# jopohl/urh

Measured on AMD Instinct MI355X. Metric: Msamples/s IQ->bits (1 GiB complex64 2-FSK per GPU, qad materialised, compact outputs copied to the host), higher is better.
Workload: dtype f32

## Files before the change

include/urhgpu.h:

```cpp
#ifndef URHGPU_H
#define URHGPU_H

#include <stdint.h>

#ifdef __cplusplus
extern "C" {
#endif

#define URHGPU_VERSION 100

#define URHGPU_OK 0
#define URHGPU_ERR_HIP (-1)
#define URHGPU_ERR_DTYPE (-2)
#define URHGPU_ERR_ARG (-3)
#define URHGPU_ERR_CAPACITY (-4)
#define URHGPU_ERR_UNSUPPORTED (-5)
#define URHGPU_ERR_NO_DEVICE (-6)

#define URHGPU_DT_I8 0
#define URHGPU_DT_U8 1
#define URHGPU_DT_I16 2
#define URHGPU_DT_U16 3
#define URHGPU_DT_F32 4

// ... 190 lines not shown

int urhgpu_segment_runs_dev(urhgpu_ctx *ctx, const void *d_iq, int dtype, int64_t n, float noise_threshold,
                            int64_t *d_rows, int64_t cap_rows, int64_t *d_n_rows);
int urhgpu_message_ranges_dev(urhgpu_ctx *ctx, const void *d_iq, int dtype, int64_t n, float noise_threshold, int64_t *seg_out, int64_t cap_seg_out,
                              int64_t *n_seg_out, int64_t *merged_out, int64_t cap_merged_out, int64_t *n_merged_out, int *merge_ambiguous);
int urhgpu_message_ranges_demod_dev(urhgpu_ctx *ctx, const void *d_iq, int dtype, int64_t n, float noise_threshold, int64_t *seg_out,
                                    int64_t cap_seg_out, int64_t *n_seg_out, int64_t *merged_out, int64_t cap_merged_out,
                                    int64_t *n_merged_out, int *merge_ambiguous, float *d_qad_ask);
int urhgpu_compact_gt_dev(urhgpu_ctx *ctx, const float *d_x, int64_t n, float thr, float *d_out, int64_t *d_count);
int urhgpu_edges_le_dev(urhgpu_ctx *ctx, const float *d_x, int64_t n, float center, int64_t *d_idx, int64_t cap, int64_t *d_count);
int urhgpu_minmax_f32_dev(urhgpu_ctx *ctx, const float *d_x, int64_t n, float *d_out2);
int urhgpu_pairwise_sum_f32_dev(urhgpu_ctx *ctx, const float *d_x, int64_t n, int mode, float mean, float *sum_out);
int urhgpu_histogram_f32_dev(urhgpu_ctx *ctx, const float *d_x, int64_t n, const double *d_edges, int64_t n_edges, int64_t *d_counts);

int urhgpu_msg_center_stats(urhgpu_ctx *ctx, const float *d_x, int64_t n, const int64_t *ranges, int n_msgs, int64_t max_bins,
                            double *out_stats, int64_t *out_hist, double *out_center, int32_t *out_flag);
int urhgpu_msg_plateaus(urhgpu_ctx *ctx, const float *d_x, int64_t n, const int64_t *ranges, const double *centers, int n_msgs,
                        int percentage, int64_t extra_window, int64_t *out_off, uint64_t *out_len, int64_t cap_total);

int urhgpu_merge_plateaus(const uint64_t *plateaus, int64_t n, uint64_t tolerance, uint64_t max_count, uint64_t *out, int64_t *n_out);

int urhgpu_detect_modulation_dev(urhgpu_ctx *ctx, const float *d_iq, int64_t n, const int64_t *ranges, int n_msgs, int wavelet_scale,
                                 int median_filter_order, int *labels_out, double *vars_out);

int urhgpu_msg_bit_lengths(const uint64_t *lens, const int64_t *off, int n_msgs, int64_t *tol_out, int64_t *bitlen_out);
int urhgpu_msg_plateau_decisions(urhgpu_ctx *ctx, const float *d_x, int64_t n, const int64_t *ranges, const double *centers, int n_msgs,
                                 int percentage, int64_t extra_window, int64_t *tol_out, int64_t *bitlen_out);
int urhgpu_msg_estimate(urhgpu_ctx *ctx, const float *d_x, int64_t n, const int64_t *ranges, int n_msgs, int64_t max_bins, int percentage,
                        int64_t extra_window, double *out_stats, double *out_center, int32_t *out_flag, int64_t *tol_out, int64_t *bitlen_out);
int urhgpu_test_bit_length_from_counts(const uint64_t *lens, int64_t n, int64_t *tol_out, int64_t *bitlen_out);
int urhgpu_msg_divisor_histogram(const uint64_t *lens, int64_t n, uint64_t *hist_out, int64_t cap, int64_t *hist_len, int64_t *tol_out);
int urhgpu_bit_length_from_order(const uint64_t *hist, const int64_t *order_desc, int64_t len, int64_t *bitlen_out);

int urhgpu_minmax(urhgpu_ctx *ctx, const void *arr, int dtype, int64_t n, void *out2);
int urhgpu_segment_messages(urhgpu_ctx *ctx, const void *magnitudes, int is_f64, int64_t n, float noise_threshold, int64_t *seg_out,
                            int64_t cap_seg, int64_t *n_seg);
int urhgpu_get_plateau_lengths(urhgpu_ctx *ctx, const float *rect_data, int64_t n, float center, int percentage, uint64_t *out, int64_t cap,
                               int64_t *n_out);
int urhgpu_threshold_divisor_histogram(const uint64_t *lens, int64_t n, float threshold, uint64_t *hist_out, int64_t cap, int64_t *hist_len);
int urhgpu_median_filter(urhgpu_ctx *ctx, const double *data, int64_t n, unsigned int k, float *out);

int urhgpu_test_fast_division_dev(urhgpu_ctx *ctx, uint64_t seed, int reps, uint64_t *n_mismatch);
int urhgpu_test_sincosf_fast_dev(urhgpu_ctx *ctx, uint64_t *n_mismatch);
int urhgpu_test_force_merge_ambiguous(int on);

int urhgpu_modulate_dev(urhgpu_ctx *ctx, const uint8_t *bits, const int64_t *bit_off, const uint32_t *pause, const uint32_t *start,
                        int n_msgs, uint32_t samples_per_symbol, int mod, const float *parameters, int bits_per_symbol,
                        float carrier_amplitude, float carrier_frequency, float carrier_phase, float sample_rate, int dtype,
                        void *d_out, int64_t cap_samples, int64_t *total_samples);
int urhgpu_modulate(urhgpu_ctx *ctx, const uint8_t *bits, int64_t num_bits, uint32_t samples_per_symbol, int mod,
                    const float *parameters, int bits_per_symbol, float carrier_amplitude, float carrier_frequency,
                    float carrier_phase, float sample_rate, uint32_t pause, uint32_t start, int dtype, void *out);

int urhgpu_modulate_gfsk_dev(urhgpu_ctx *ctx, const uint8_t *bits, const int64_t *bit_off, const uint32_t *pause, const uint32_t *start,
                             int n_msgs, uint32_t samples_per_symbol, const float *parameters, int bits_per_symbol,
                             float carrier_amplitude, float carrier_phase, float sample_rate, int dtype, const float *gauss_fir,
                             int n_taps, const float *frequencies, void *d_out, int64_t cap_samples, int64_t *total_samples);
int urhgpu_modulate_gfsk(urhgpu_ctx *ctx, const uint8_t *bits, int64_t num_bits, uint32_t samples_per_symbol, const float *parameters,
                         int bits_per_symbol, float carrier_amplitude, float carrier_phase, float sample_rate, uint32_t pause,
                         uint32_t start, int dtype, const float *gauss_fir, int n_taps, const float *frequencies, void *out);

int urhgpu_convert_dev(urhgpu_ctx *ctx, const void *d_src, int src_dtype, void *d_dst, int dst_dtype, int64_t n);
int urhgpu_pcm_to_iq_dev(urhgpu_ctx *ctx, const void *d_raw, int64_t n_frames, int channels, int sample_width, float *d_out);
int urhgpu_fft_peak_dev(urhgpu_ctx *ctx, const float *d_x, int64_t n, int64_t *peak_index);
int urhgpu_sub_encode_runs(const uint8_t *values, int64_t n, int64_t stride, int64_t *runs_out, int64_t cap, int64_t *n_runs);
int urhgpu_astype_dev(urhgpu_ctx *ctx, const void *d_src, int src_dtype, void *d_dst, int dst_dtype, int64_t n);

int urhgpu_path_minmax_dev(urhgpu_ctx *ctx, const void *d_samples, int dtype, int64_t start, int64_t end,
                           int64_t samples_per_pixel, void *d_values);
int urhgpu_path_minmax(urhgpu_ctx *ctx, const void *samples, int dtype, int64_t n, int64_t start, int64_t end,
                       int64_t samples_per_pixel, void *values);

int urhgpu_spectrogram_dev(urhgpu_ctx *ctx, const float *d_x, int64_t n, int window_size, int64_t hop, int64_t frames,
                           const double *d_window, const double *d_twiddles, double *d_stft, float *d_db);
int urhgpu_bgra_lookup_dev(urhgpu_ctx *ctx, const float *d_db, int64_t frames, int window_size, const uint32_t *d_colormap,
                           int n_colors, float data_min, float data_max, uint32_t *d_image);

int urhgpu_bench_copy_ceiling_dev(urhgpu_ctx *ctx, const float *d_in, float *d_out, int64_t n_samples, int shape, int reps, float *ms_per_copy);
int urhgpu_test_hot_probe(urhgpu_ctx *ctx, const void *d_iq, int64_t n, const urhgpu_params *p, float *d_qad, int stream_kind, int event_mode,
                          int graded, int launches, int keep, void *d_chunks_out, int64_t *n_chunks_out, float *dur_ms, float *gap_ms, int bubble_us,
                          int load_kind);
int urhgpu_test_hot_stamps(int on);
int urhgpu_test_tail_skip(int mask);
int urhgpu_test_fetch_chunk_tables(urhgpu_ctx *ctx, void *host_dst, int64_t n_chunks);
int urhgpu_memcpy_to_host(urhgpu_ctx *ctx, const void *d_src, void *host_dst, int64_t bytes);
int urhgpu_memcpy_dtod(urhgpu_ctx *ctx, void *d_dst, const void *d_src, int64_t bytes);

int urhgpu_test_force_state_bytes(int on);

int urhgpu_test_force_generic_tail(int on);

int urhgpu_test_force_tiles_per_chunk(int tiles);

int64_t urhgpu_test_wide_int_launches(void);

int64_t urhgpu_test_costas_host_syncs(void);
int64_t urhgpu_test_center_host_syncs(void);
int urhgpu_test_costas_scratch(int64_t n, int loop_order, int64_t *out3);

int urhgpu_test_atan2f_dev(urhgpu_ctx *ctx, const float *d_y, const float *d_x, int64_t n, float *d_out);

int urhgpu_chunk_power_stats_dev(urhgpu_ctx *ctx, const void *d_src, int dtype, int64_t n_rows, void *d_dst, int64_t n_store, double *sum_out,
                                 double *max_out);
int urhgpu_chunk_stats_launches(urhgpu_ctx *ctx, int64_t *n_launches);

int urhgpu_magnitude_chunk_partials_dev(urhgpu_ctx *ctx, const void *d_iq, int dtype, int64_t n_local, int64_t pos_base, int64_t n_total,
                                        int64_t chunk, int64_t n_chunks, double *d_sum, double *d_max);
#define URHGPU_PW_REC_HEAD 8
#define URHGPU_PW_REC_FIRST 136
#define URHGPU_PW_REC_LAST 264
#define URHGPU_PW_REC_TAIL 392
#define URHGPU_PW_REC_PIECES 520
int urhgpu_pairwise_partial_f32_dev(urhgpu_ctx *ctx, const float *d_x, int64_t m_local, int64_t g_off, int64_t m_total, int mode, float mean,
                                    float *d_out, int64_t cap, int64_t *n_out);

typedef struct urhgpu_noise_result {
    double noise;
    float noise_f32;
    float noise_sqrd;
    int64_t flag;
    int64_t chunk, n_chunks;
    int64_t n_candidates;
    double min_mean, max_mean;
} urhgpu_noise_result;
double urhgpu_noise_max_magnitude(int dtype);
int urhgpu_detect_noise_level_dev(urhgpu_ctx *ctx, const void *d_iq, int dtype, int64_t n, void *d_result);
int urhgpu_iq_to_bits_auto_dev(urhgpu_ctx *ctx, const void *d_iq, int64_t n, const urhgpu_params *p, int auto_noise, int auto_center,
                               int64_t center_max_size, const urhgpu_outputs *out, void *d_noise_result, void *h_noise_result,
                               void *d_center_result, void *h_center_result, int64_t hist_cap);
int urhgpu_stream_set_auto_noise(urhgpu_stream *st, int enable);
int urhgpu_stream_noise(urhgpu_stream *st, int64_t seq, double *noise, int64_t *flag);
int64_t urhgpu_test_noise_host_syncs(void);

typedef struct urhgpu_msg_record {
    double rssi;
    int64_t first_pos;
    int64_t mid_pos;
    int32_t n_pad;
    int32_t flag;
} urhgpu_msg_record;
int urhgpu_msg_records_dev(urhgpu_ctx *ctx, const void *d_iq, int64_t n, const urhgpu_params *p, const urhgpu_outputs *out,
                           int64_t message_length_divisor, void *d_rec, int64_t cap_msg, void *h_rec);
int urhgpu_stream_set_msg_records(urhgpu_stream *st, int enable, int64_t message_length_divisor);
int urhgpu_stream_msg_records(urhgpu_stream *st, int64_t seq, const urhgpu_msg_record **rec, int64_t *n_msg);
int64_t urhgpu_test_records_host_syncs(void);

int urhgpu_dc_correct_dev(urhgpu_ctx *ctx, const void *d_in, int64_t n, int dtype, void *d_out, void *d_mean);
int urhgpu_dc_correct(urhgpu_ctx *ctx, const void *h_in, int64_t n, int dtype, void *h_out, void *h_mean);
int64_t urhgpu_test_dc_host_syncs(void);
int urhgpu_test_dc_stats(urhgpu_ctx *ctx, int64_t *stats);

int urhgpu_shard_dc_sums_dev(urhgpu_ctx *ctx, const void *d_in, int64_t n, int dtype, void *d_words);
#define URHGPU_DC_RECORD_BYTES 64
int urhgpu_shard_dc_spec_dev(urhgpu_ctx *ctx, const void *d_in, int64_t n, const double *base, void *d_records);
int urhgpu_shard_dc_resolve_dev(urhgpu_ctx *ctx, const void *d_in, int64_t n, const uint32_t *entry, void *d_exit);
int urhgpu_shard_dc_apply_dev(urhgpu_ctx *ctx, const void *d_in, int64_t n, int dtype, const void *mean, void *d_out);
int urhgpu_shard_dc_stats(urhgpu_ctx *ctx, int64_t *stats);

#define URHGPU_SHARD_REC_SUMMARY_WORDS 10
#define URHGPU_SHARD_REC_FIRST_WORDS 8
int urhgpu_shard_records_summary_dev(urhgpu_ctx *ctx, int64_t n_local, int64_t pos_base, const urhgpu_outputs *out, void *d_words);
int urhgpu_shard_records_lookup_dev(urhgpu_ctx *ctx, const urhgpu_outputs *out, const void *d_index, int64_t n, void *d_values);
int urhgpu_shard_msg_records_dev(urhgpu_ctx *ctx, const void *d_iq, int64_t n_local, int64_t pos_base, int64_t n_total, const urhgpu_params *p,
                                 const urhgpu_outputs *out, int64_t message_length_divisor, const int64_t *first, const void *d_window,
                                 int64_t window_len, void *d_rec, int64_t cap_msg, void *h_rec);

// ... 87 lines not shown
```

urh_amd/_lib.py:

```python
import ctypes as C
import os
import threading

HERE = os.path.dirname(os.path.abspath(__file__))
LIB_PATH = os.path.join(HERE, "liburhgpu.so")

OK = 0
ERR_HIP, ERR_DTYPE, ERR_ARG, ERR_CAPACITY, ERR_UNSUPPORTED, ERR_NO_DEVICE = -1, -2, -3, -4, -5, -6
BLOB_LEN16 = 2
BLOB_ROW16 = 4

DT_I8, DT_U8, DT_I16, DT_U16, DT_F32 = 0, 1, 2, 3, 4
MOD_ASK, MOD_FSK, MOD_PSK, MOD_OTHER = 0, 1, 2, 3
ROW_ABSORBED = -(1 << 62)
BLOB_MAGIC = 0x55524842424C4F42
BLOB_HEADER_BYTES = 128


class UrhGpuError(RuntimeError):
    def __init__(self, status, msg):
        super().__init__(msg)
        self.status = status


# ... 80 lines not shown
                                    C.POINTER(_i64)]),
    "urhgpu_ppseq_to_bits": (_i, [_vp, _vp, _i64, _i64, _i, _i, _i64, _vp, _i64, _vp, _vp, _i64, _vp, _i64, _vp, _vp]),
    "urhgpu_fir_filter": (_i, [_vp, _vp, _i64, _vp, _i64, _vp]),
    "urhgpu_fir_filter_dev": (_i, [_vp, _vp, _i64, _vp, _i64, _vp, _vp]),
    "urhgpu_fir_filter_stats_dev": (_i, [_vp, _vp, _i64, _vp, _i64, _vp, _vp, _i64, _i64, _vp, _vp]),
    "urhgpu_bandpass": (_i, [_vp, _vp, _i64, _vp, _i64, _i64, _i64, _vp]),
    "urhgpu_bandpass_dev": (_i, [_vp, _vp, _i64, _vp, _i64, _i64, _i64, _vp, _i64, _vp, _i64, _vp, _i]),
    "urhgpu_iir_filter": (_i, [_vp, _vp, _i64, _vp, _i64, _vp, _i64, _vp]),
    "urhgpu_afp_demod_dev": (_i, [_vp, _vp, _i64, C.POINTER(Params), _vp]),
    "urhgpu_grab_pulse_lens_dev": (_i, [_vp, _vp, _i64, C.POINTER(Params), _vp, _i64, _vp]),
    "urhgpu_ppseq_to_bits_dev": (_i, [_vp, _vp, _vp, _i64, C.POINTER(Params), C.POINTER(Outputs)]),
    "urhgpu_iq_to_bits_dev": (_i, [_vp, _vp, _i64, C.POINTER(Params), C.POINTER(Outputs)]),
    "urhgpu_detect_center_dev": (_i, [_vp, _vp, _i64, _i64, _vp, _i64]),
    "urhgpu_iq_to_bits_auto_center_dev": (_i, [_vp, _vp, _i64, C.POINTER(Params), _i64, C.POINTER(Outputs), _vp, _vp, _i64]),
    "urhgpu_center_hist_cap": (_i64, [_vp]),
    "urhgpu_stream_set_auto_center": (_i, [_vp, _i, _i64]),
    "urhgpu_stream_center": (_i, [_vp, _i64, C.POINTER(C.c_double), C.POINTER(_i64), C.POINTER(_vp), C.POINTER(_i64), C.POINTER(C.c_double),
                                  C.POINTER(C.c_double)]),
    "urhgpu_test_center_host_syncs": (_i64, []),
    "urhgpu_noise_max_magnitude": (C.c_double, [_i]),
    "urhgpu_detect_noise_level_dev": (_i, [_vp, _vp, _i, _i64, _vp]),
    "urhgpu_iq_to_bits_auto_dev": (_i, [_vp, _vp, _i64, C.POINTER(Params), _i, _i, _i64, C.POINTER(Outputs), _vp, _vp, _vp, _vp, _i64]),
    "urhgpu_stream_set_auto_noise": (_i, [_vp, _i]),
    "urhgpu_stream_noise": (_i, [_vp, _i64, C.POINTER(C.c_double), C.POINTER(_i64)]),
    "urhgpu_test_noise_host_syncs": (_i64, []),
    "urhgpu_msg_records_dev": (_i, [_vp, _vp, _i64, C.POINTER(Params), C.POINTER(Outputs), _i64, _vp, _i64, _vp]),
    "urhgpu_stream_set_msg_records": (_i, [_vp, _i, _i64]),
    "urhgpu_stream_msg_records": (_i, [_vp, _i64, C.POINTER(_vp), C.POINTER(_i64)]),
    "urhgpu_test_records_host_syncs": (_i64, []),
    "urhgpu_shard_records_summary_dev": (_i, [_vp, _i64, _i64, C.POINTER(Outputs), _vp]),
    "urhgpu_shard_records_lookup_dev": (_i, [_vp, C.POINTER(Outputs), _vp, _i64, _vp]),
    "urhgpu_shard_msg_records_dev": (_i, [_vp, _vp, _i64, _i64, _i64, C.POINTER(Params), C.POINTER(Outputs), _i64, C.POINTER(_i64), _vp, _i64, _vp, _i64,
                                          _vp]),
    "urhgpu_blob_capacity": (_i64, [_i64, _i64, _i64, _i64, _i]),
    "urhgpu_outputs_to_host": (_i, [_vp, C.POINTER(Outputs), _i, _vp, _i64, C.POINTER(_i64)]),
    "urhgpu_host_libm_check": (_i, [C.POINTER(_i64)]),
    "urhgpu_stream_capacities": (_i, [_i64, C.POINTER(Params), C.POINTER(_i64), C.POINTER(_i64), C.POINTER(_i64), C.POINTER(_i64)]),
    "urhgpu_stream_create": (_i, [_vp, _i64, C.POINTER(Params), _i, _i, _i64, C.POINTER(_vp)]),
    "urhgpu_stream_destroy": (_i, [_vp]),
    "urhgpu_stream_push": (_i, [_vp, _vp, _i64, C.POINTER(HostResult)]),
    "urhgpu_stream_push_upload": (_i, [_vp, _vp, _vp, _i64, C.POINTER(HostResult)]),
    "urhgpu_stream_flush": (_i, [_vp, C.POINTER(HostResult), C.POINTER(_i)]),
    "urhgpu_stream_stats": (_i, [_vp, C.POINTER(_i64)]),
    "urhgpu_stream_wide_passes": (_i, [_vp, C.POINTER(_i64)]),
    "urhgpu_stream_costas_stats": (_i, [_vp, C.POINTER(_i64)]),
    "urhgpu_shard_runs_dev": (_i, [_vp, _vp, _i64, _i64, _i64, _i, _i, _vp, C.POINTER(Params), C.POINTER(Outputs), _vp]),
    "urhgpu_shard_prelaunch_dev": (_i, [_vp, _vp, _i64, _i64, _i64, _i, _i, C.POINTER(Params), C.POINTER(Outputs)]),
    "urhgpu_shard_launch_dev": (_i, [_vp, _vp, _i64, _i64, _i64, _i, _i, _vp, C.POINTER(Params), C.POINTER(Outputs)]),
    "urhgpu_shard_rows_dev": (_i, [_vp, _vp, _vp]),
    "urhgpu_shard_bits_prepare_dev": (_i, [_vp, _vp, _vp]),
    "urhgpu_shard_bits_finish_dev": (_i, [_vp, _vp]),
    "urhgpu_costas_halo_samples": (_i64, [C.POINTER(Params)]),
    "urhgpu_shard_costas_spec_dev": (_i, [_vp, _vp, _i64, _i64, _i64, _i, _i, _vp, _i64, C.POINTER(Params), C.POINTER(Outputs), _vp]),
    "urhgpu_shard_costas_resolve_dev": (_i, [_vp, C.POINTER(C.c_uint32), _vp]),
    "urhgpu_shard_demod_dev": (_i, [_vp, _vp, _i64, _i64, _i64, _i, _i, _vp, C.POINTER(Params), C.POINTER(Outputs)]),
    "urhgpu_shard_seam_value": (_i, [_vp, C.POINTER(C.c_float)]),
    "urhgpu_magnitude_chunk_stats_dev": (_i, [_vp, _vp, _i, _i64, _i64, _i64, _vp, _vp]),
    "urhgpu_segment_runs_dev": (_i, [_vp, _vp, _i, _i64, _f, _vp, _i64, _vp]),
    "urhgpu_message_ranges_dev": (_i, [_vp, _vp, _i, _i64, _f, _vp, _i64, C.POINTER(_i64), _vp, _i64, C.POINTER(_i64), C.POINTER(_i)]),
    "urhgpu_message_ranges_demod_dev": (_i, [_vp, _vp, _i, _i64, _f, _vp, _i64, C.POINTER(_i64), _vp, _i64, C.POINTER(_i64), C.POINTER(_i), _vp]),
    "urhgpu_compact_gt_dev": (_i, [_vp, _vp, _i64, _f, _vp, _vp]),
    "urhgpu_edges_le_dev": (_i, [_vp, _vp, _i64, _f, _vp, _i64, _vp]),
    "urhgpu_minmax_f32_dev": (_i, [_vp, _vp, _i64, _vp]),
    "urhgpu_pairwise_sum_f32_dev": (_i, [_vp, _vp, _i64, _i, _f, C.POINTER(_f)]),
    "urhgpu_histogram_f32_dev": (_i, [_vp, _vp, _i64, _vp, _i64, _vp]),
    "urhgpu_msg_center_stats": (_i, [_vp, _vp, _i64, _vp, _i, _i64, _vp, _vp, _vp, _vp]),
    "urhgpu_msg_plateaus": (_i, [_vp, _vp, _i64, _vp, _vp, _i, _i, _i64, _vp, _vp, _i64]),
    "urhgpu_detect_modulation_dev": (_i, [_vp, _vp, _i64, _vp, _i, _i, _i, _vp, _vp]),
    "urhgpu_msg_bit_lengths": (_i, [_vp, _vp, _i, _vp, _vp]),
    "urhgpu_msg_plateau_decisions": (_i, [_vp, _vp, _i64, _vp, _vp, _i, _i, _i64, _vp, _vp]),
    "urhgpu_msg_estimate": (_i, [_vp, _vp, _i64, _vp, _i, _i64, _i, _i64, _vp, _vp, _vp, _vp, _vp]),
    "urhgpu_test_bit_length_from_counts": (_i, [_vp, _i64, C.POINTER(_i64), C.POINTER(_i64)]),
    "urhgpu_msg_divisor_histogram": (_i, [_vp, _i64, _vp, _i64, C.POINTER(_i64), C.POINTER(_i64)]),
    "urhgpu_bit_length_from_order": (_i, [_vp, _vp, _i64, C.POINTER(_i64)]),
    "urhgpu_merge_plateaus": (_i, [_vp, _i64, C.c_uint64, C.c_uint64, _vp, C.POINTER(_i64)]),
    "urhgpu_minmax": (_i, [_vp, _vp, _i, _i64, _vp]),
    "urhgpu_segment_messages": (_i, [_vp, _vp, _i, _i64, _f, _vp, _i64, C.POINTER(_i64)]),
    "urhgpu_get_plateau_lengths": (_i, [_vp, _vp, _i64, _f, _i, _vp, _i64, C.POINTER(_i64)]),
    "urhgpu_threshold_divisor_histogram": (_i, [_vp, _i64, _f, _vp, _i64, C.POINTER(_i64)]),
    "urhgpu_median_filter": (_i, [_vp, _vp, _i64, C.c_uint, _vp]),
    "urhgpu_test_hot_probe": (_i, [_vp, _vp, _i64, C.POINTER(Params), _vp, _i, _i, _i, _i, _i, _vp, C.POINTER(_i64), _vp, _vp, _i, _i]),
    "urhgpu_test_hot_stamps": (_i, [_i]),
    "urhgpu_test_tail_skip": (_i, [_i]),
    "urhgpu_test_fetch_chunk_tables": (_i, [_vp, _vp, _i64]),
    "urhgpu_test_fast_division_dev": (_i, [_vp, C.c_uint64, _i, C.POINTER(C.c_uint64)]),
    "urhgpu_test_sincosf_fast_dev": (_i, [_vp, C.POINTER(C.c_uint64)]),
    "urhgpu_test_force_merge_ambiguous": (_i, [_i]),
    "urhgpu_modulate_dev": (_i, [_vp, _vp, _vp, _vp, _vp, _i, C.c_uint32, _i, _vp, _i, _f, _f, _f, _f, _i, _vp, _i64, C.POINTER(_i64)]),
    "urhgpu_modulate": (_i, [_vp, _vp, _i64, C.c_uint32, _i, _vp, _i, _f, _f, _f, _f, C.c_uint32, C.c_uint32, _i, _vp]),
    "urhgpu_modulate_gfsk_dev": (_i, [_vp, _vp, _vp, _vp, _vp, _i, C.c_uint32, _vp, _i, _f, _f, _f, _i, _vp, _i, _vp, _vp, _i64, C.POINTER(_i64)]),
    "urhgpu_modulate_gfsk": (_i, [_vp, _vp, _i64, C.c_uint32, _vp, _i, _f, _f, _f, C.c_uint32, C.c_uint32, _i, _vp, _i, _vp, _vp]),
    "urhgpu_spectrogram_dev": (_i, [_vp, _vp, _i64, _i, _i64, _i64, _vp, _vp, _vp, _vp]),
    "urhgpu_bgra_lookup_dev": (_i, [_vp, _vp, _i64, _i, _vp, _i, _f, _f, _vp]),
    "urhgpu_convert_dev": (_i, [_vp, _vp, _i, _vp, _i, _i64]),
    "urhgpu_pcm_to_iq_dev": (_i, [_vp, _vp, _i64, _i, _i, _vp]),
    "urhgpu_sub_encode_runs": (_i, [_vp, _i64, _i64, _vp, _i64, _vp]),
    "urhgpu_fft_peak_dev": (_i, [_vp, _vp, _i64, _vp]),
    "urhgpu_astype_dev": (_i, [_vp, _vp, _i, _vp, _i, _i64]),
    "urhgpu_path_minmax_dev": (_i, [_vp, _vp, _i, _i64, _i64, _i64, _vp]),
    "urhgpu_path_minmax": (_i, [_vp, _vp, _i, _i64, _i64, _i64, _i64, _vp]),
    "urhgpu_bench_copy_ceiling_dev": (_i, [_vp, _vp, _vp, _i64, _i, _i, C.POINTER(_f)]),
    "urhgpu_memcpy_to_host": (_i, [_vp, _vp, _vp, _i64]),
    "urhgpu_memcpy_dtod": (_i, [_vp, _vp, _vp, _i64]),
    "urhgpu_test_force_state_bytes": (_i, [_i]),
    "urhgpu_test_force_tiles_per_chunk": (_i, [_i]),
    "urhgpu_test_wide_int_launches": (_i64, []),
    "urhgpu_test_costas_host_syncs": (_i64, []),
    "urhgpu_test_costas_scratch": (_i, [_i64, _i, C.POINTER(_i64)]),
    "urhgpu_test_force_generic_tail": (_i, [_i]),
    "urhgpu_test_atan2f_dev": (_i, [_vp, _vp, _vp, _i64, _vp]),
    "urhgpu_chunk_power_stats_dev": (_i, [_vp, _vp, _i, _i64, _vp, _i64, C.POINTER(C.c_double), C.POINTER(C.c_double)]),
    "urhgpu_chunk_stats_launches": (_i, [_vp, C.POINTER(_i64)]),
    "urhgpu_magnitude_chunk_partials_dev": (_i, [_vp, _vp, _i, _i64, _i64, _i64, _i64, _i64, _vp, _vp]),
    "urhgpu_pairwise_partial_f32_dev": (_i, [_vp, _vp, _i64, _i64, _i64, _i, _f, _vp, _i64, C.POINTER(_i64)]),
    "urhgpu_dc_correct_dev": (_i, [_vp, _vp, _i64, _i, _vp, _vp]),
    "urhgpu_dc_correct": (_i, [_vp, _vp, _i64, _i, _vp, _vp]),
    "urhgpu_test_dc_host_syncs": (_i64, []),
    "urhgpu_test_dc_stats": (_i, [_vp, C.POINTER(_i64)]),
    "urhgpu_shard_dc_sums_dev": (_i, [_vp, _vp, _i64, _i, _vp]),
    "urhgpu_shard_dc_spec_dev": (_i, [_vp, _vp, _i64, C.POINTER(C.c_double), _vp]),
    "urhgpu_shard_dc_resolve_dev": (_i, [_vp, _vp, _i64, C.POINTER(C.c_uint32), _vp]),
    "urhgpu_shard_dc_apply_dev": (_i, [_vp, _vp, _i64, _i, _vp, _vp]),
    "urhgpu_shard_dc_stats": (_i, [_vp, C.POINTER(_i64)]),
    "urhgpu_batch_step": (_i, []),
    "urhgpu_batch_plan": (_i, [_vp, _i64, C.POINTER(Params), _i, _i64, _vp, C.POINTER(_i64), C.POINTER(_i64)]),
    "urhgpu_iq_to_bits_batch_dev": (_i, [_vp, _vp, _i64, _vp, _vp, _i64, C.POINTER(Params), _vp, _vp, _i64, _vp, _vp, _vp, _i64]),
    "urhgpu_batch_fetch": (_i, [_vp, _vp, _i64, _vp, _vp, _vp, _i64, C.POINTER(_i64)]),
    "urhgpu_batch_launches": (_i, [_vp, C.POINTER(_i64)]),
    "urhgpu_batch_noise_dev": (_i, [_vp, _vp, _i64, _vp, _vp, _i64, C.POINTER(Params), _vp]),
    "urhgpu_iq_to_bits_batch_auto_dev": (_i, [_vp, _vp, _i64, _vp, _vp, _i64, C.POINTER(Params), _vp, _vp, _i64, _vp, _vp, _vp, _i64, _vp]),
    "urhgpu_batch_noise_fetch": (_i, [_vp, _vp, _i64, _vp]),
    "urhgpu_batch_center_plan": (_i, [_vp, _i64, _i64, _i64, C.POINTER(_i64), C.POINTER(_i64), C.POINTER(_i64)]),
    "urhgpu_batch_center_dev": (_i, [_vp, _vp, _i64, _vp, _i64, C.POINTER(Params), _i64, _vp, _vp, _i64, _vp, _i64, _vp, _i64, _vp, _i64]),
    "urhgpu_qad_to_bits_batch_dev": (_i, [_vp, _vp, _i64, _vp, _vp, _i64, C.POINTER(Params), _vp, _i64, _vp, _vp, _i64, _vp, _vp, _vp, _i64]),
    "urhgpu_iq_to_bits_batch_center_dev": (_i, [_vp, _vp, _i64, _vp, _vp, _i64, C.POINTER(Params), _i, _i64, _vp, _vp, _i64, _vp, _vp, _vp, _i64, _vp,
                                                _vp, _i64, _vp, _i64, _vp, _i64, _vp, _i64]),
    "urhgpu_batch_center_fetch": (_i, [_vp, _vp, _i64, _vp, _i64, _vp, _vp, _i64, C.POINTER(_i64)]),
    "urhgpu_batch_msg_records_dev": (_i, [_vp, _vp, _i64, _vp, _i64, _vp, _vp, _i64, C.POINTER(Params), _vp, _i64, _vp, _i64, _vp, _vp, _vp, _i64, _vp]),
    "urhgpu_batch_records_fetch": (_i, [_vp, _vp, _i64, _i64, _vp]),
    "urhgpu_batch_segments_capacity": (_i64, [_i64]),
    "urhgpu_batch_segments_dev": (_i, [_vp, _vp, _i, _i64, _vp, _vp, _i64, _vp, _vp, _vp, _i64, _vp, _vp, _vp, _i64]),
    "urhgpu_batch_segments_fetch": (_i, [_vp, _vp, _i64, _vp, _vp, _vp, _i64, C.POINTER(_i64)]),
    "urhgpu_batch_demod_dev": (_i, [_vp, _vp, _i64, _vp, _vp, _i64, C.POINTER(Params), _vp, _vp]),
    "urhgpu_batch_costas_dev": (_i, [_vp, _vp, _i64, _vp, _vp, _i64, C.POINTER(Params), _vp, _vp]),
    "urhgpu_iq_to_bits_batch_psk_dev": (_i, [_vp, _vp, _i64, _vp, _vp, _i64, C.POINTER(Params), _i, _i, _i64, _vp, _vp, _i64, _vp, _vp, _vp, _i64, _vp,
                                             _vp, _i64, _vp, _i64, _vp, _i64, _vp, _i64]),
    "urhgpu_batch_dc_correct_dev": (_i, [_vp, _vp, _i64, _i, _vp, _vp, _i64, _vp, _vp]),
    "urhgpu_batch_plan_each": (_i, [_vp, _i64, _vp, _i, _i64, _vp, C.POINTER(_i64), C.POINTER(_i64)]),
    "urhgpu_iq_to_bits_batch_each_dev": (_i, [_vp, _vp, _i64, _i, _vp, _vp, _i64, _vp, _vp, _i64, _i64, _i, _vp, _vp, _i64, _vp, _vp, _vp, _i64, _vp]),
    "urhgpu_batch_msg_records_each_dev": (_i, [_vp, _vp, _i64, _i, _vp, _vp, _i64, _vp, _i64, _vp, _i64, _vp, _vp, _vp, _i64, _vp]),
}

_lib = None
_lock = threading.Lock()


def _share_torch_hip_runtime():
    import importlib.util
    try:
        spec = importlib.util.find_spec("torch")
    except (ImportError, ValueError):
        spec = None
    if spec is None or not spec.origin:
        return
    cand = os.path.join(os.path.dirname(spec.origin), "lib", "libamdhip64.so")
    if os.path.exists(cand):
# ... 139 lines not shown
```

urh_amd/csrc/common.hpp:

```cpp
#pragma once
#include <hip/hip_runtime.h>
#include <stdint.h>
#include <stdio.h>
#include <string.h>

#include <atomic>
#include <vector>

#include "../../include/urhgpu.h"

#ifndef URH_TAIL_PRIO_LEVEL
#define URH_TAIL_PRIO_LEVEL 3
#endif
#ifndef URH_TAIL_PAD
#define URH_TAIL_PAD 0
#endif
#if URH_TAIL_PAD
#define URH_TAIL_PRIO() do { __builtin_amdgcn_s_setprio(URH_TAIL_PRIO_LEVEL); __asm__ volatile("v_mov_b32 v95, 0" ::: "v95"); } while (0)
#else
#define URH_TAIL_PRIO() __builtin_amdgcn_s_setprio(URH_TAIL_PRIO_LEVEL)
#endif

namespace urh {

// ... 25 lines not shown
    void *take(size_t bytes) {
        size_t off = (used + 255) & ~size_t(255);
        if (off + bytes > cap) return nullptr;
        used = off + bytes;
        return (char *)base + off;
    }
    void release();
};
inline size_t align256(size_t x) { return (x + 255) & ~size_t(255); }

extern std::atomic<long long> g_center_host_syncs;
extern thread_local int g_center_scope;
extern std::atomic<long long> g_noise_host_syncs;
extern thread_local int g_noise_scope;
extern std::atomic<long long> g_records_host_syncs;
extern thread_local int g_records_scope;
inline void center_note_wait() {
    if (g_center_scope > 0) ++g_center_host_syncs;
    if (g_noise_scope > 0) ++g_noise_host_syncs;
    if (g_records_scope > 0) ++g_records_host_syncs;
}
struct CenterScope { CenterScope() { ++g_center_scope; } ~CenterScope() { --g_center_scope; } };
struct NoiseScope { bool on; explicit NoiseScope(bool enable = true) : on(enable) { if (on) ++g_noise_scope; } ~NoiseScope() { if (on) --g_noise_scope; } };
struct RecordsScope { bool on; explicit RecordsScope(bool enable = true) : on(enable) { if (on) ++g_records_scope; } ~RecordsScope() { if (on) --g_records_scope; } };

}

constexpr size_t kSmallPinned = size_t(1) << 20;
constexpr int kNoiseMaxChunks = 199;
constexpr size_t kNoiseWorkBytes = 128 * 1024;
struct urhgpu_ctx {
    int device = 0;
    hipStream_t own_stream = nullptr;
    hipStream_t stream = nullptr;
    hipDeviceProp_t prop;
    urh::Arena arena;
    urh::Arena staging;
    urh::Arena aux;
    urh::Arena fir_work;
    hipEvent_t ev_fir = nullptr;
    hipStream_t fir_stream = nullptr;
    int64_t *d_counts = nullptr;
    int64_t *h_counts = nullptr;
    bool tune_spin_wait = true;
    bool tune_wide_int = false;
    bool tune_shard_summary_generic = false;
    int tune_costas_dev_rounds = -1;
    int32_t *costas_stats_next = nullptr;
    hipStream_t last_tail = nullptr;
    int wide_int_next = 0;
    char *h_small = nullptr;
    int32_t *d_tickets = nullptr;
    void *d_desc = nullptr;
    size_t desc_cap = 0;
    void *d_rdesc = nullptr;
    size_t rdesc_cap = 0;
    unsigned long long scan_epoch = 0x0ACE0FBA5E000000ull;
    std::vector<hipEvent_t> prof_events;
    std::vector<bool> prof_dispatch;
    int prof_used = 0;
    bool prof_on = false;
    bool prof_bracket = false;
    void *shard = nullptr;
    bool pipelined = false;
    int hot_lds_pad_sharded = 33 * 1024;
    int tune_hot_cus_removed = 4;
    hipStream_t hot_masked = nullptr;
    hipEvent_t ev_in = nullptr;
    int hot_lds_pad = 0;
    hipStream_t tail_stream = nullptr;
    bool own_tail_stream = false;
    urh::Arena arena_alt, arena_alt2;
    hipEvent_t ev_hot = nullptr;
    hipEvent_t ev_tail[3] = {nullptr, nullptr, nullptr};
    int flip = 0;
    bool tail_pending = false;
    int tile_parity = 0;
    void *d_seg = nullptr;
    bool seg_dirty[3] = {false, false, false};
    int tune_stream_segments = 7;
    int tune_stream_policy = 5;
    long long passes_begun = 0;
    bool tune_stream_latency = false;
    bool tune_stream_pos_direct = true;
    int tune_upload_pieces = 4;
    hipEvent_t ev_piece[16] = {};
    hipEvent_t ev_hot_done[3] = {nullptr, nullptr, nullptr};
    hipStream_t bits_stream = nullptr;
    hipEvent_t ev_rows[3][16] = {};
    hipEvent_t ev_bits[3] = {nullptr, nullptr, nullptr};
    urh::Arena chunk_work;
    double *h_chunk = nullptr;
    long long chunk_launches = 0;
    long long batch_launches = 0, batch_copies = 0;
    urh::Arena center_work;
    int tune_center_max_bins = 4096;
    hipEvent_t ev_center = nullptr;
    void *d_noise_work = nullptr;
    int wide_int_auto = 0;
    urh::Arena dc_work;
    hipEvent_t ev_dc = nullptr;
    hipStream_t dc_stream = nullptr;
    const void *dc_shard_in = nullptr;
    int64_t dc_shard_n = -1;
    urh::Arena batch_dc_mean;
};
constexpr size_t kSegBlockBytes = 4096;

namespace urh {
int iq_to_bits_streamed(urhgpu_ctx *ctx, const void *d_iq, int64_t n, const urhgpu_params *p, const urhgpu_outputs *out, void *host_blob,
                        int64_t cap_host, hipEvent_t ev_ready, bool *streamed, const void *h_iq, void *stage_blob = nullptr, bool *staged = nullptr,
                        hipEvent_t ev_rows = nullptr, int len16 = 0);
hipError_t wait_stream(const urhgpu_ctx *ctx, hipStream_t s);
int reserve_psk_pass(urhgpu_ctx *ctx, int64_t n_max, int tolerance, bool want_qad);
int join_tail(urhgpu_ctx *ctx);
inline int stage_in(urhgpu_ctx *ctx, const void *host, size_t bytes, void **dev) {
    void *d = ctx->staging.take(bytes ? bytes : 16);
    if (!d) return URHGPU_ERR_ARG;
    if (bytes) URH_HIP(hipMemcpyAsync(d, host, bytes, hipMemcpyHostToDevice, ctx->stream));
    *dev = d;
    return URHGPU_OK;
}
inline int fetch_out(urhgpu_ctx *ctx, void *host, const void *dev, size_t bytes) {
    URH_HIP(hipMemcpyAsync(host, dev, bytes, hipMemcpyDeviceToHost, ctx->stream));
    URH_HIP(hipStreamSynchronize(ctx->stream));
    return URHGPU_OK;
}
}
```

urh_amd/csrc/ctx.hip:

```cpp
#include <chrono>

#include "pass.hpp"
#include "fdlibm_atan2f.h"
#include "glibc_sincosf.h"

namespace urh {

thread_local char g_hip_err[256] = "";
std::atomic<long long> g_center_host_syncs{0};
thread_local int g_center_scope = 0;
std::atomic<long long> g_noise_host_syncs{0};
thread_local int g_noise_scope = 0;
std::atomic<long long> g_records_host_syncs{0};
thread_local int g_records_scope = 0;

int Arena::reserve(size_t bytes) {
    if (bytes <= cap) return URHGPU_OK;
    if (base) { center_note_wait(); URH_HIP(hipFree(base)); base = nullptr; cap = 0; }
    const size_t want = (bytes + (size_t(1) << 20)) & ~((size_t(1) << 20) - 1);
    URH_HIP(hipMalloc(&base, want));
    cap = want;
    used = 0;
    return URHGPU_OK;
}
// ... 118 lines not shown
            if (ctx->ev_bits[k]) (void)hipEventDestroy(ctx->ev_bits[k]);
            for (hipEvent_t e : ctx->ev_rows[k]) if (e) (void)hipEventDestroy(e);
        }
    }
    if (ctx->ev_hot) { (void)hipEventDestroy(ctx->ev_hot); (void)hipEventDestroy(ctx->ev_tail[0]); (void)hipEventDestroy(ctx->ev_tail[1]); (void)hipEventDestroy(ctx->ev_tail[2]); }
    free_shard_session(ctx);
    for (hipEvent_t e : ctx->prof_events) (void)hipEventDestroy(e);
    if (ctx->d_counts) (void)hipFree(ctx->d_counts);
    if (ctx->d_tickets) (void)hipFree(ctx->d_tickets);
    if (ctx->d_noise_work) (void)hipFree(ctx->d_noise_work);
    if (ctx->d_desc) (void)hipFree(ctx->d_desc);
    if (ctx->d_rdesc) (void)hipFree(ctx->d_rdesc);
    if (ctx->h_counts) (void)hipHostFree(ctx->h_counts);
    if (ctx->h_small) (void)hipHostFree(ctx->h_small);
    if (ctx->own_stream) (void)hipStreamDestroy(ctx->own_stream);
    delete ctx;
    return URHGPU_OK;
}

int urhgpu_ctx_set_stream(urhgpu_ctx *ctx, void *hip_stream) {
    if (!ctx) return URHGPU_ERR_ARG;
    ctx->stream = (hipStream_t)hip_stream;
    return URHGPU_OK;
}

int urhgpu_ctx_use_private_stream(urhgpu_ctx *ctx) {
    if (!ctx) return URHGPU_ERR_ARG;
    ctx->stream = ctx->own_stream;
    return URHGPU_OK;
}

int urhgpu_ctx_sync(urhgpu_ctx *ctx) {
    if (!ctx) return URHGPU_ERR_ARG;
    if (ctx->hot_masked) URH_HIP(hipStreamSynchronize(ctx->hot_masked));
    if (ctx->bits_stream) URH_HIP(hipStreamSynchronize(ctx->bits_stream));
    if (ctx->tail_stream) URH_HIP(hipStreamSynchronize(ctx->tail_stream));
    URH_HIP(hipStreamSynchronize(ctx->stream));
    ctx->tail_pending = false;
    return URHGPU_OK;
}

int urhgpu_ctx_set_pipelined(urhgpu_ctx *ctx, int enable, void *tail_stream) {
    if (!ctx) return URHGPU_ERR_ARG;
    URH_HIP(hipSetDevice(ctx->device));
    URH_TRY(urhgpu_ctx_sync(ctx));
    if (ctx->own_tail_stream && ctx->tail_stream) { (void)hipStreamDestroy(ctx->tail_stream); }
    ctx->tail_stream = nullptr; ctx->own_tail_stream = false; ctx->pipelined = false;
    if (ctx->hot_masked) { (void)hipStreamSynchronize(ctx->hot_masked); (void)hipStreamDestroy(ctx->hot_masked); ctx->hot_masked = nullptr; }
    if (!enable) return URHGPU_OK;
    if (tail_stream) ctx->tail_stream = (hipStream_t)tail_stream;
    else {
        URH_HIP(hipStreamCreateWithFlags(&ctx->tail_stream, hipStreamNonBlocking));
        ctx->own_tail_stream = true;
    }
    if (!ctx->ev_hot) {
        URH_HIP(hipEventCreateWithFlags(&ctx->ev_hot, hipEventDisableTiming));
        for (hipEvent_t &e : ctx->ev_tail) URH_HIP(hipEventCreateWithFlags(&e, hipEventDisableTiming));
    }
    if (ctx->tune_hot_cus_removed > 0 && ctx->prop.multiProcessorCount == 256) {
        const int words = 8;
        uint32_t mask[8];
        hot_cu_mask(ctx->tune_hot_cus_removed, mask);
        if (hipExtStreamCreateWithCUMask(&ctx->hot_masked, (uint32_t)words, mask) != hipSuccess) { (void)hipGetLastError(); ctx->hot_masked = nullptr; }
        if (ctx->hot_masked && !ctx->ev_in && hipEventCreateWithFlags(&ctx->ev_in, hipEventDisableTiming) != hipSuccess) {
            (void)hipGetLastError();
            (void)hipStreamDestroy(ctx->hot_masked);
            ctx->hot_masked = nullptr;
        }
    }
    ctx->pipelined = true;
    return URHGPU_OK;
}

int urhgpu_ctx_set_tuning(urhgpu_ctx *ctx, const char *key, int value) {
    if (!ctx || !key) return URHGPU_ERR_ARG;
    if (!strcmp(key, "hot_lds_kb")) { if (value < 0 || value > 150) return URHGPU_ERR_ARG; ctx->hot_lds_pad = value * 1024; }
    else if (!strcmp(key, "hot_lds_kb_sharded")) { if (value < 0 || value > 150) return URHGPU_ERR_ARG; ctx->hot_lds_pad_sharded = value * 1024; }
    else if (!strcmp(key, "profile_bracket")) ctx->prof_bracket = value != 0;
    else if (!strcmp(key, "hot_cus_removed_per_xcd")) { if (value < 0 || value > 16) return URHGPU_ERR_ARG; ctx->tune_hot_cus_removed = value; }
    else if (!strcmp(key, "stream_segments")) { if (value < 1 || value > kMaxSegments) return URHGPU_ERR_ARG; ctx->tune_stream_segments = value; }
    else if (!strcmp(key, "stream_policy")) { if (value < 0 || value > 6) return URHGPU_ERR_ARG; ctx->tune_stream_policy = value; }
    else if (!strcmp(key, "stream_latency")) { ctx->tune_stream_latency = value != 0; }
    else if (!strcmp(key, "stream_pos_direct")) { ctx->tune_stream_pos_direct = value != 0; }
    else if (!strcmp(key, "spin_wait")) { ctx->tune_spin_wait = value != 0; }
    else if (!strcmp(key, "shard_summary_generic")) { ctx->tune_shard_summary_generic = value != 0; }
    else if (!strcmp(key, "wide_int")) { ctx->tune_wide_int = value != 0; }
    else if (!strcmp(key, "costas_dev_rounds")) { if (value < -1 || value > 24) return URHGPU_ERR_ARG; ctx->tune_costas_dev_rounds = value; }
    else if (!strcmp(key, "upload_pieces")) { if (value < 2 || value > kMaxSegments) return URHGPU_ERR_ARG; ctx->tune_upload_pieces = value; }
    else if (!strcmp(key, "auto_center_max_bins")) { if (value < 1 || value > (1 << 20)) return URHGPU_ERR_ARG; ctx->tune_center_max_bins = value; }
    else return URHGPU_ERR_ARG;
    return URHGPU_OK;
}

int urhgpu_ctx_join(urhgpu_ctx *ctx) {
    if (!ctx) return URHGPU_ERR_ARG;
    URH_HIP(hipSetDevice(ctx->device));
    return join_tail(ctx);
}

int urhgpu_host_libm_check(int64_t *out4) {
    if (!out4) return URHGPU_ERR_ARG;
    static const uint32_t kDiscriminating[17] = {0x418a3adbu, 0x418a3adcu, 0x418a3addu, 0x418a3adeu, 0x41bc76d9u, 0x4202eb4bu, 0x4255b0a9u, 0x4280ce28u,
                                                 0x42687a55u, 0x42a35c07u, 0x42a35d44u, 0x42870e40u, 0x42a97360u, 0x42c55faau, 0x42d8d23eu, 0x42e87a55u,
                                                 0x42cf5854u};
    int64_t n_sc = 0, bad_sc = 0, n_at = 0, bad_at = 0;
    auto same = [](float a, float b) { uint32_t x, y; memcpy(&x, &a, 4); memcpy(&y, &b, 4); return x == y || (a != a && b != b); };
    auto check_sc = [&](float x) {
        volatile float vx = x;
        n_sc += 2;
        if (!same(sinf(vx), urh_sinf(x))) ++bad_sc;
        if (!same(cosf(vx), urh_cosf(x))) ++bad_sc;
    };
    for (uint32_t u : kDiscriminating) {
        float x; memcpy(&x, &u, 4);
        check_sc(x); check_sc(-x);
    }
    uint64_t s = 0x243f6a8885a308d3ull;
    auto next = [&]() { s += 0x9e3779b97f4a7c15ull; uint64_t z = s; z = (z ^ (z >> 30)) * 0xbf58476d1ce4e5b9ull; z = (z ^ (z >> 27)) * 0x94d049bb133111ebull; return z ^ (z >> 31); };
    for (int i = 0; i < 4096; ++i) {
        const uint64_t z = next();
        check_sc((float)((double)(int64_t)(z >> 11) * (1.0 / 9007199254740992.0) * 240.0 - 120.0));
        const uint32_t a = (uint32_t)z, b = (uint32_t)(z >> 32);
        float y, x;
        const uint32_t uy = (a & 0x807fffffu) | (((a >> 23) % 41u + 107u) << 23), ux = (b & 0x807fffffu) | (((b >> 23) % 41u + 107u) << 23);
        memcpy(&y, &uy, 4); memcpy(&x, &ux, 4);
        volatile float vy = y, vx = x;
        ++n_at;
        if (!same(atan2f(vy, vx), urh_atan2f(y, x))) ++bad_at;
    }
    out4[0] = n_sc; out4[1] = bad_sc; out4[2] = n_at; out4[3] = bad_at;
    return URHGPU_OK;
}

int urhgpu_ctx_info(urhgpu_ctx *ctx, int *compute_units, int *wavefront, int64_t *hbm_bytes, char *name, int name_cap) {
    if (!ctx) return URHGPU_ERR_ARG;
    if (compute_units) *compute_units = ctx->prop.multiProcessorCount;
    if (wavefront) *wavefront = ctx->prop.warpSize;
    if (hbm_bytes) *hbm_bytes = (int64_t)ctx->prop.totalGlobalMem;
    if (name && name_cap > 0) { strncpy(name, ctx->prop.name, (size_t)name_cap - 1); name[name_cap - 1] = 0; }
    return URHGPU_OK;
}

int urhgpu_ctx_reserve(urhgpu_ctx *ctx, int64_t n_samples, int tolerance) {
    if (!ctx || n_samples < 0 || tolerance < 0) return URHGPU_ERR_ARG;
    URH_HIP(hipSetDevice(ctx->device));
    const Plan pl = make_plan(ctx, n_samples, tolerance);
    const int64_t cap_rows = n_samples / ((int64_t)tolerance + 1) + 2;
    URH_TRY(ctx->arena.reserve(digitize_scratch_bytes(pl, cap_rows, true, true)));
    if (ctx->pipelined) {
        URH_TRY(ctx->arena_alt.reserve(digitize_scratch_bytes(pl, cap_rows, true, true)));
        URH_TRY(ctx->arena_alt2.reserve(digitize_scratch_bytes(pl, cap_rows, true, true)));
    }
    return URHGPU_OK;
}

int urhgpu_ctx_profile_begin(urhgpu_ctx *ctx, int max_records) {
    if (!ctx || max_records < 0) return URHGPU_ERR_ARG;
    URH_HIP(hipSetDevice(ctx->device));
    while ((int)ctx->prof_events.size() < 4 * max_records) {
        hipEvent_t e;
        URH_HIP(hipEventCreate(&e));
        ctx->prof_events.push_back(e);
    }
    ctx->prof_used = 0;
    ctx->prof_on = max_records > 0;
    return URHGPU_OK;
// ... 53 lines not shown
```

urh_amd/csrc/launchers.hpp:

```cpp
#pragma once
#include <atomic>
#include <hip/hip_runtime.h>
#include <stdint.h>

#include "common.hpp"
#include "runs.hpp"

namespace urh {

struct RunArgs {
    const void *in;
    float *qad;
    const void *left_halo;
    int64_t n;
    int64_t range_begin;
    int64_t range_end;
    int64_t chunk_base;
    int64_t pos_base;
    int64_t chunk_len;
    uint64_t *slab;
    int64_t slab_stride;
    ChunkInfo *chunks;
    float noise_sqrd;
    float noise_val;
// ... 155 lines not shown
size_t merge_scratch_bytes(int64_t cap);
int launch_merge_rows_ask(const int64_t *rows_in, const int64_t *d_n_in, int64_t cap, int64_t *rows_out,
                          int64_t cap_out, int64_t *d_n_out, void *scratch, int32_t *tickets, hipStream_t s);
size_t bits_scratch_bytes(int64_t cap_rows);
struct ScanState {
    int32_t *tickets;
    void *desc;
    size_t desc_bytes;
    unsigned long long *epoch;
};
size_t bits_desc_bytes(int64_t cap_rows);
int launch_ppseq_to_bits(const int64_t *rows, const int64_t *d_n_rows, int64_t cap_rows, const BitsParams &bp,
                         const BitsOut &o, void *scratch, const ScanState &ss, hipStream_t s);
int launch_bits_prepare(const int64_t *rows, const int64_t *d_n_rows, int64_t cap_rows, const BitsParams &bp,
                        void *scratch, int64_t *d_flags, const ScanState &ss, hipStream_t s);
int launch_bits_finish(const int64_t *rows, const int64_t *d_n_rows, int64_t cap_rows, const BitsParams &bp,
                       const BitsOut &o, void *scratch, const ScanState &ss, hipStream_t s);
struct SegState {
    int64_t rows_at[kMaxSegments];
    int64_t rows_needed;
    int64_t n_acc;
    int64_t n_groups;
    int64_t n_groups_local;
    int64_t end_bits, end_pos, end_msgs;
    int64_t err;
    struct In {
        int64_t g0;
        int64_t carry[3];
        int64_t ship_bits, ship_pos, ship_msgs, pad;
    } in[2];
};
static_assert(sizeof(SegState) == 128 + 64 + 128, "SegState");
constexpr int64_t kSegAlign = 256;
struct SegGate {
    const uint32_t *progress;
    int k;
    uint32_t target;
    int init;
    SegState *seg;
    long long max_ticks;
    int fused;
};
struct RowsSegment {
    int index;
    int final;
    int64_t c0, c1;
    SegGate gate;
    int8_t *h_state;
    int32_t *h_len;
    int fuse_gate;
    int len16;
    int64_t *esc;
    int64_t esc_cap;
};
struct BitsSegment {
    int index;
    int final;
    int64_t c0, c1;
    int rows_index;
    SegState *state;
    int64_t scan_b0;
};
struct SegPackDst {
    void *host;
    int64_t cap_host;
    uint32_t *progress_reset;
    int blocks;
    int pos_direct;
    int split;
    void *host_head;
    const int64_t *esc;
    int64_t esc_cap;
    int64_t row16_esc_off;
};

struct TileTailMem {
    void *mem;
    int64_t n_chunks;
    int32_t *huge_count;
    int parity;
    void *rdesc;
    unsigned long long epoch;
    int64_t *d_row_base = nullptr;
};
size_t tile_rdesc_bytes(int64_t n_chunks);
size_t tile_tail_bytes(int64_t n_chunks);
int64_t tile_desc_cap(int64_t cap_rows, int64_t n_chunks);
int64_t tile_scan_blocks(int64_t c0, int64_t c1, int final);
int launch_tile_rows(const ResolveArgs &r, const EmitArgs &e, const TileTailMem &m, const BitsParams *bp, hipStream_t s);
int launch_tile_bits(const TileTailMem &m, const int64_t *rows, const int64_t *d_n_rows, int64_t cap_rows, const BitsParams &bp,
                     const BitsOut &o, void *scratch, const ScanState &ss, hipStream_t s);
int launch_tile_bits_prepare(const TileTailMem &m, const int64_t *rows, const int64_t *d_n_rows, int64_t cap_rows, const BitsParams &bp,
                             void *scratch, int64_t *d_flags, const ScanState &ss, hipStream_t s);
int launch_tile_bits_finish(const TileTailMem &m, const int64_t *rows, const int64_t *d_n_rows, int64_t cap_rows, const BitsParams &bp,
                            const BitsOut &o, void *scratch, const ScanState &ss, hipStream_t s);
int launch_rows_segment(const ResolveArgs &r, const EmitArgs &e, const TileTailMem &m, const BitsParams &bp, SegState *state, const RowsSegment &sg,
                        hipStream_t s);
int launch_bits_segment(const TileTailMem &m, const BitsParams &bp, const BitsOut &o, void *scratch, const ScanState &ss, int64_t *rows,
                        int64_t cap_rows, const BitsSegment &sg, const SegPackDst *dst, hipStream_t s);
void launch_merge_summary(const int64_t *rows, const int64_t *d_n_rows, int64_t *d_out5, hipStream_t s);
void launch_merge_fix(int64_t *rows, const int64_t *d_n_rows, const int64_t *d_all, int rank, int world,
                      int64_t *d_absorbed, hipStream_t s);
void launch_bits_extra(const int64_t *d_all, int rank, int world, int32_t *d_extra, hipStream_t s);

size_t fir_stats_scratch_bytes(int64_t n);
size_t fir_work_bytes(int64_t n, int m);
int launch_fir(const float2 *x, int64_t n, const float2 *taps, int m, const float2 *halo, float2 *out, hipStream_t s, void *work = nullptr,
               int64_t chunk = 0, int64_t n_chunks = 0, double *d_sum = nullptr, double *d_max = nullptr, void *tile_scratch = nullptr);
int launch_iir(const double *a, int64_t M, const double *b, int64_t N, const float2 *x, int64_t n, float2 *y, hipStream_t s);
int launch_magnitudes(const void *iq, int dtype, int64_t n, double *out, hipStream_t s);
size_t mag_chunk_scratch_bytes(int64_t n_chunks);
int launch_mag_chunk_stats(const void *iq, int dtype, int64_t n, int64_t chunk, int64_t n_chunks, double *d_sum, double *d_max,
                           void *scratch, hipStream_t s);
int launch_noise_chain(const void *iq, int dtype, int64_t n, double max_mag, float cfg_noise, int use_cfg, void *work, void *d_result, void *h_result,
                       hipStream_t s);
size_t compact_scratch_bytes(int64_t n);
int launch_compact_gt(const float *x, int64_t n, const int64_t *d_n, float thr, float *out, int64_t *d_count, void *scratch,
                      int32_t *tickets, hipStream_t s);
int launch_compact_edges(const float *x, int64_t n, const int64_t *d_n, float center, int64_t *out, int64_t cap, int64_t *d_count,
                         void *scratch, int32_t *tickets, hipStream_t s);
size_t minmax_scratch_bytes();
int launch_minmax(const float *x, int64_t n, float *d_out2, void *scratch, hipStream_t s);
int launch_minmax_any(const void *x, int dtype, int64_t n, void *d_out2, void *scratch, hipStream_t s);
int launch_above_flags(const void *mag, int is_f64, int64_t n, float thr, float *flags, hipStream_t s);
int launch_median_filter(const double *data, int64_t n, int k, float *out, hipStream_t s);
constexpr int kDtAboveFlags = 100;
int pairwise_sum_f32(urhgpu_ctx *ctx, const float *d_x, int64_t n, int mode, float mean, float *out);
int launch_hist_edges(const float *x, int64_t n, const double *d_edges, int n_edges, int64_t *d_counts, hipStream_t s);
size_t sp_mag_scratch_bytes(int64_t n_chunks);
int launch_mag_chunk_partials(const void *iq, int dtype, int64_t n_local, int64_t pos_base, int64_t n_total, int64_t chunk, int64_t n_chunks,
                              double *d_sum, double *d_max, void *scratch, hipStream_t s);
int64_t pairwise_partial_words(int64_t m_local, int64_t g_off, int64_t m_total);
size_t pairwise_partial_scratch_bytes(int64_t m_local);
int launch_pairwise_partial(const float *x, int64_t m_local, int64_t g_off, int64_t m_total, int mode, float mean, float *rec, void *scratch,
                            hipStream_t s);
size_t chunk_stats_scratch_bytes(int dtype, int64_t n_rows);
int launch_chunk_stats(const void *d_src, int dtype, int64_t n_rows, void *d_dst, int64_t store_rows, void *scratch, double *h_out, hipStream_t s);
struct SegCtl;
extern bool g_force_merge_ambiguous;
int launch_message_ranges(const int64_t *d_rows, const int64_t *d_n_rows, int64_t cap_rows, const void *d_iq, int dtype, int64_t n, float thr,
                          int ook_merge, int64_t *d_seg, int64_t *d_msgs, int64_t cap, SegCtl *d_ctl, void *scratch, hipStream_t s);
size_t seg_scratch_bytes(int64_t cap_rows, int64_t cap);
size_t seg_ctl_bytes();
void seg_ctl_read(const void *host_copy, int64_t *n_seg, int64_t *n_msgs, int *ambiguous);
int launch_pack_blob(const urhgpu_outputs *o, int write_pos, hipStream_t s);
void launch_copy_shape(const float *in, float *out, int64_t n_samples, int shape, hipStream_t s);
int launch_msg_records(const void *d_iq, int64_t n, const urhgpu_params *p, const urhgpu_outputs *out, int64_t divisor, void *d_rec, int64_t cap_rec,
                       void *h_rec, hipStream_t s);
size_t costas_scratch_bytes(int64_t n);
int launch_costas(urhgpu_ctx *ctx, const void *d_iq, int64_t n, const urhgpu_params *p, float *d_qad, void *scratch, const float *d_noise = nullptr);
extern std::atomic<long long> g_costas_host_syncs;
void costas_scratch_layout(int64_t n, int K, int64_t out3[3]);
constexpr int kCostasSummaryBytes = 160;
struct CostasShard {
    const void *iq;
    const void *halo_end;
    float *out;
    int64_t n, origin, lo, start1;
    urhgpu_params p;
    void *scratch;
};
int64_t costas_halo_samples(const urhgpu_params *p);
int launch_costas_shard_spec(urhgpu_ctx *ctx, const CostasShard &cs, void *d_summary);
int launch_costas_shard_resolve(urhgpu_ctx *ctx, const CostasShard &cs, uint32_t freq_bits, uint32_t phase_bits, void *d_end);

}
```

urh_amd/csrc/probes.hip:

```cpp
#include "pass.hpp"

using namespace urh;

#define URH_PROBE_WPB 4

namespace urh {
bool g_tile_tail = true;
int g_force_tiles_per_chunk = 0;
}

extern "C" {

int urhgpu_test_fast_division_dev(urhgpu_ctx *ctx, uint64_t seed, int reps, uint64_t *n_mismatch) {
    if (!ctx || !n_mismatch || reps < 0) return URHGPU_ERR_ARG;
    URH_HIP(hipSetDevice(ctx->device));
    URH_HIP(hipMemsetAsync(ctx->d_counts, 0, 8, ctx->stream));
    launch_test_div(seed, reps, (unsigned long long *)ctx->d_counts, ctx->stream);
    URH_HIP(hipGetLastError());
    URH_TRY(fetch_out(ctx, ctx->h_counts, ctx->d_counts, 8));
    *n_mismatch = (uint64_t)ctx->h_counts[0];
    return URHGPU_OK;
}

int urhgpu_test_force_merge_ambiguous(int on) {
    const int was = urh::g_force_merge_ambiguous ? 1 : 0;
    urh::g_force_merge_ambiguous = on != 0;
    return was;
}

int urhgpu_test_sincosf_fast_dev(urhgpu_ctx *ctx, uint64_t *n_mismatch) {
    if (!ctx || !n_mismatch) return URHGPU_ERR_ARG;
    URH_HIP(hipSetDevice(ctx->device));
    URH_HIP(hipMemsetAsync(ctx->d_counts, 0, 8, ctx->stream));
    launch_test_sincosf_fast((unsigned long long *)ctx->d_counts, ctx->stream);
    URH_HIP(hipGetLastError());
    URH_TRY(fetch_out(ctx, ctx->h_counts, ctx->d_counts, 8));
    *n_mismatch = (uint64_t)ctx->h_counts[0];
    return URHGPU_OK;
}

int urhgpu_bench_copy_ceiling_dev(urhgpu_ctx *ctx, const float *d_in, float *d_out, int64_t n_samples, int shape, int reps, float *ms_per_copy) {
    if (!ctx || !d_in || !d_out || !ms_per_copy || n_samples < 8192 || n_samples % 8192 || reps < 1 || shape < 0 || shape > 2) return URHGPU_ERR_ARG;
    if (((uintptr_t)d_in & 15) || ((uintptr_t)d_out & 15)) return URHGPU_ERR_ARG;
    URH_HIP(hipSetDevice(ctx->device));
    URH_TRY(urhgpu_ctx_sync(ctx));
    hipStream_t cs = ctx->stream;
    if (shape == 2) {
        if (!ctx->hot_masked) return URHGPU_ERR_UNSUPPORTED;
        cs = ctx->hot_masked; shape = 0;
    }
    hipEvent_t e0, e1;
    URH_HIP(hipEventCreate(&e0));
    URH_HIP(hipEventCreate(&e1));
    for (int k = 0; k < 3; ++k) launch_copy_shape(d_in, d_out, n_samples, shape, cs);
    URH_HIP(hipEventRecord(e0, cs));
    for (int k = 0; k < reps; ++k) launch_copy_shape(d_in, d_out, n_samples, shape, cs);
    URH_HIP(hipEventRecord(e1, cs));
    URH_HIP(hipEventSynchronize(e1));
    float ms = 0.f;
    URH_HIP(hipEventElapsedTime(&ms, e0, e1));
    (void)hipEventDestroy(e0); (void)hipEventDestroy(e1);
    *ms_per_copy = ms / (float)reps;
    return URHGPU_OK;
}

__global__ void k_probe_valu(long long ticks, int prio, float *sink) {
    if (prio) __builtin_amdgcn_s_setprio(3);
    const long long t0 = (long long)wall_clock64();
    float x = (float)threadIdx.x, y = 1.0f;
    unsigned long long z = threadIdx.x;
    do {
#pragma unroll
        for (int k = 0; k < 64; ++k) { x = x * 1.0001f + y; y = y * 0.9999f + x; z = z * 6364136223846793005ull + 1442695040888963407ull; }
    } while ((long long)wall_clock64() - t0 < ticks);
    if (x == 12345.678f && z == 42) *sink = y;
}
__global__ void k_probe_latency(long long ticks, const unsigned long long *mem, unsigned long long lines, unsigned long long *sink) {
    const long long t0 = (long long)wall_clock64();
    unsigned long long at = (blockIdx.x * 256ull + threadIdx.x) * 0x9e3779b97f4a7c15ull, acc = 0;
    do {
#pragma unroll 1
        for (int k = 0; k < 8; ++k) { const unsigned long long v = mem[(at % lines) * 8]; acc += v; at = at * 6364136223846793005ull + v + 1442695040888963407ull; }
    } while ((long long)wall_clock64() - t0 < ticks);
    if (acc == 0x1234567ull) *sink = acc;
}

__global__ void k_probe_spin(long long ticks) {
    const long long t0 = (long long)wall_clock64();
    while ((long long)wall_clock64() - t0 < ticks) __builtin_amdgcn_s_sleep(16);
}

int urhgpu_test_hot_stamps(int on) { urh::g_stamp_probe = (on != 0); return URHGPU_OK; }
int urhgpu_test_tail_skip(int mask) { urh::g_tail_skip = mask; return URHGPU_OK; }

int urhgpu_test_fetch_chunk_tables(urhgpu_ctx *ctx, void *host_dst, int64_t n_chunks) {
    if (!ctx || !host_dst || n_chunks < 1) return URHGPU_ERR_ARG;
    URH_HIP(hipSetDevice(ctx->device));
    URH_TRY(urhgpu_ctx_sync(ctx));
    const size_t bytes = (size_t)n_chunks * sizeof(ChunkInfo);
    const urh::Arena *order[3] = {&ctx->arena, &ctx->arena_alt2, &ctx->arena_alt};
    for (int k = 0; k < 3; ++k) {
        if (!order[k]->base || order[k]->cap < bytes) { memset((char *)host_dst + k * bytes, 0, bytes); continue; }
        URH_HIP(hipMemcpy((char *)host_dst + k * bytes, order[k]->base, bytes, hipMemcpyDeviceToHost));
    }
    return URHGPU_OK;
}

int urhgpu_test_hot_probe(urhgpu_ctx *ctx, const void *d_iq, int64_t n, const urhgpu_params *p, float *d_qad, int stream_kind, int event_mode,
                          int graded, int launches, int keep, void *d_chunks_out, int64_t *n_chunks_out, float *dur_ms, float *gap_ms, int bubble_us,
                          int load_kind) {
    if (!ctx || !d_iq || !p || !d_qad || !d_chunks_out || !n_chunks_out || launches < 1 || keep < 1 || keep > launches || n < kTile || n % kTile) return URHGPU_ERR_ARG;
    if (p->dtype != URHGPU_DT_F32 || p->mod != URHGPU_MOD_FSK || p->bits_per_symbol != 1) return URHGPU_ERR_UNSUPPORTED;
    URH_HIP(hipSetDevice(ctx->device));
    URH_TRY(join_tail(ctx));
    URH_TRY(urhgpu_ctx_sync(ctx));
    const Plan pl = make_plan(ctx, n, p->tolerance);
    const int64_t g = std::min<int64_t>(std::max(graded, 0), pl.n_chunks);
    const int64_t short_len = pl.chunk_len / 4;
    if (g > 0 && ((short_len % (URH_PROBE_WPB * kRowSamples)) != 0 || n % pl.chunk_len != 0)) return URHGPU_ERR_UNSUPPORTED;
    const int64_t n_launch = pl.n_chunks + 3 * g;
    URH_TRY(ctx->arena.reserve((size_t)n_launch * sizeof(ChunkInfo) + (size_t)n_launch * pl.slab_stride * 8 + 4096));
    ctx->arena.reset();
    ChunkInfo *chunks = (ChunkInfo *)ctx->arena.take((size_t)n_launch * sizeof(ChunkInfo));
    uint64_t *slab = (uint64_t *)ctx->arena.take((size_t)n_launch * pl.slab_stride * 8);
    if (!chunks || !slab) return URHGPU_ERR_ARG;
    RunArgs a;
    URH_TRY(hot_run_args(ctx, p, pl, n, 0, true, &a));
    a.in = d_iq; a.qad = d_qad; a.wide_int = 0;
    a.chunks = chunks; a.slab = slab; a.stamp_probe = 1;
    if (g > 0) { a.graded_from = pl.n_chunks - g; a.graded_len = short_len; }
    hipStream_t s = ctx->stream;
    if (stream_kind == 1) { if (!ctx->hot_masked) return URHGPU_ERR_UNSUPPORTED; s = ctx->hot_masked; }
    std::vector<hipEvent_t> ev((size_t)launches * 2, nullptr);
    if (event_mode != 0) {
        const unsigned fl = event_mode == 1 ? hipEventDisableTiming : event_mode == 2 ? (hipEventDisableTiming | hipEventDisableSystemFence | hipEventReleaseToDevice) : hipEventDefault;
        for (auto &e : ev) URH_HIP(hipEventCreateWithFlags(&e, fl));
    }
    hipStream_t s2 = nullptr;
    void *load_mem = nullptr;
    if (load_kind != 0) {
        if (event_mode == 0 || event_mode == 3) return URHGPU_ERR_ARG;
        if (load_kind == 3 || load_kind == 5) URH_HIP(hipStreamCreateWithFlags(&s2, hipStreamNonBlocking));
        else {
            uint32_t m[8], inv[8];
            hot_cu_mask(ctx->tune_hot_cus_removed, m);
            for (int w = 0; w < 8; ++w) inv[w] = ~m[w];
            URH_HIP(hipExtStreamCreateWithCUMask(&s2, 8, inv));
        }
        URH_HIP(hipMalloc(&load_mem, size_t(256) << 20));
        URH_HIP(hipMemset(load_mem, 1, size_t(256) << 20));
        URH_HIP(hipDeviceSynchronize());
    }
    for (int j = 0; j < launches; ++j) {
        a.chunks = (j >= launches - keep) ? (ChunkInfo *)d_chunks_out + (size_t)(j - (launches - keep)) * n_launch : chunks;
        HotEvents he;
        if (event_mode != 0) { he.start = event_mode == 3 ? ev[2 * j] : nullptr; he.stop = ev[2 * j + 1]; }
        URH_TRY(launch_demod_runs_iq(a, p->dtype, p->mod, true, s, &he));
        if (bubble_us > 0) hipLaunchKernelGGL(k_probe_spin, dim3(1), dim3(64), 0, s, (long long)bubble_us * 100);
        if (load_kind != 0) {
            URH_HIP(hipStreamWaitEvent(s2, ev[2 * j + 1], 0));
            if (load_kind == 1 || load_kind == 2) hipLaunchKernelGGL(k_probe_valu, dim3(64), dim3(256), 0, s2, 20000ll, load_kind == 2 ? 1 : 0, (float *)load_mem);
            else if (load_kind == 3) hipLaunchKernelGGL(k_probe_valu, dim3(4096), dim3(256), 0, s2, 400ll, 1, (float *)load_mem);
            else if (load_kind == 4) hipLaunchKernelGGL(k_probe_latency, dim3(64), dim3(256), 0, s2, 20000ll, (const unsigned long long *)load_mem, (unsigned long long)((size_t(256) << 20) / 64), (unsigned long long *)load_mem);
            else for (int k = 0; k < 6; ++k) hipLaunchKernelGGL(k_probe_spin, dim3(1), dim3(64), 0, s2, 100ll);
        }
    }
    URH_HIP(hipStreamSynchronize(s));
    if (s2) { URH_HIP(hipStreamSynchronize(s2)); (void)hipStreamDestroy(s2); (void)hipFree(load_mem); }
    if (event_mode == 3 && dur_ms && gap_ms) {
        for (int j = 0; j < launches; ++j) {
            URH_HIP(hipEventElapsedTime(&dur_ms[j], ev[2 * j], ev[2 * j + 1]));
            if (j + 1 < launches) URH_HIP(hipEventElapsedTime(&gap_ms[j], ev[2 * j + 1], ev[2 * j + 2]));
        }
    }
    for (auto e : ev) if (e) (void)hipEventDestroy(e);
    *n_chunks_out = n_launch;
// ... 29 lines not shown
```

urh_amd/csrc/pulse_table.hip:

```cpp
#include <hip/hip_runtime.h>

#include <algorithm>

#include "common.hpp"
#include "compact.hpp"
#include "launchers.hpp"
#include "runs.hpp"
#include "scan.hpp"

namespace urh {

#ifndef URH_RESOLVE_BLOCK
#define URH_RESOLVE_BLOCK 256
#endif
#ifndef URH_RESOLVE_ITEMS
#define URH_RESOLVE_ITEMS 4
#endif
constexpr int kResolveBlock = URH_RESOLVE_BLOCK;

__host__ __device__ static inline int64_t resolve_blocks(int64_t n_chunks) { return (n_chunks + kResolveBlock - 1) / kResolveBlock; }

size_t resolve_scratch_bytes(int64_t n_chunks) {
    return (size_t)n_chunks * (4 * 4 + 2 * 8) + (size_t)(resolve_blocks(n_chunks) + 1) * (4 + 4 + 8) + 10 * 256;
}
// ... 568 lines not shown
    __device__ __forceinline__ bool has() const { return (meta >> 48) & 1; }
    __device__ __forceinline__ bool la_valid() const { return (meta >> 49) & 1; }
    __device__ __forceinline__ uint32_t first_state() const { return (uint32_t)(meta & 0xFFFF); }
    __device__ __forceinline__ uint32_t last_state() const { return (uint32_t)((meta >> 16) & 0xFFFF); }
    __device__ __forceinline__ uint32_t la_state() const { return (uint32_t)((meta >> 32) & 0xFFFF); }
};
__device__ __forceinline__ ResElem res_identity() { ResElem e; e.cnt = 0; e.first_pos = -1; e.la_pos = -1; e.meta = 0; return e; }
__device__ __forceinline__ ResElem res_make(uint32_t first_state, int64_t first_pos, uint32_t last_state, int64_t cnt, bool la_valid,
                                            int64_t la_pos, uint32_t la_state) {
    ResElem e;
    e.cnt = cnt; e.first_pos = first_pos; e.la_pos = la_pos;
    e.meta = (uint64_t)(first_state & 0xFFFF) | ((uint64_t)(last_state & 0xFFFF) << 16) | ((uint64_t)(la_state & 0xFFFF) << 32) |
             (1ull << 48) | ((uint64_t)(la_valid ? 1 : 0) << 49);
    return e;
}
__device__ __forceinline__ ResElem res_combine(const ResElem &a, const ResElem &b) {
    const bool ah = a.has(), bh = b.has();
    const bool acc = b.first_state() != a.last_state();
    const bool blv = b.la_valid();
    const int64_t both_cnt = a.cnt + b.cnt + (acc ? 1 : 0);
    const int64_t both_la_pos = blv ? b.la_pos : (acc ? b.first_pos : a.la_pos);
    const uint64_t both_la_state = blv ? b.la_state() : (acc ? b.first_state() : a.la_state());
    const uint64_t both_lav = (blv || acc || a.la_valid()) ? 1 : 0;
    const uint64_t both_meta = (uint64_t)a.first_state() | ((uint64_t)b.last_state() << 16) | (both_la_state << 32) | (1ull << 48) | (both_lav << 49);
    ResElem r;
    r.cnt = !ah ? b.cnt : (!bh ? a.cnt : both_cnt);
    r.first_pos = !ah ? b.first_pos : a.first_pos;
    r.la_pos = !ah ? b.la_pos : (!bh ? a.la_pos : both_la_pos);
    r.meta = !ah ? b.meta : (!bh ? a.meta : both_meta);
    return r;
}
__device__ __forceinline__ ResElem res_shfl_up(const ResElem &x, int o) {
    ResElem r;
    r.cnt = __shfl_up(x.cnt, o); r.first_pos = __shfl_up(x.first_pos, o); r.la_pos = __shfl_up(x.la_pos, o);
    r.meta = (uint64_t)__shfl_up((long long)x.meta, o);
    return r;
}
__device__ __forceinline__ ResElem res_shfl_down(const ResElem &x, int o) {
    ResElem r;
    r.cnt = __shfl_down(x.cnt, o); r.first_pos = __shfl_down(x.first_pos, o); r.la_pos = __shfl_down(x.la_pos, o);
    r.meta = (uint64_t)__shfl_down((long long)x.meta, o);
    return r;
}
__device__ __forceinline__ ResElem res_shfl(const ResElem &x, int src) {
    ResElem r;
    r.cnt = __shfl(x.cnt, src); r.first_pos = __shfl(x.first_pos, src); r.la_pos = __shfl(x.la_pos, src);
    r.meta = (uint64_t)__shfl((long long)x.meta, src);
    return r;
}
__device__ __forceinline__ ResElem res_wave_incl_scan(ResElem x, int lane) {
#pragma unroll
    for (int o = 1; o < 64; o <<= 1) {
        const ResElem u = res_shfl_up(x, o);
        if (lane >= o) x = res_combine(u, x);
    }
    return x;
}
__device__ __forceinline__ ResElem res_of_chunk(int cnt, uint32_t c_first_state, uint32_t c_last_state, uint32_t c_pend_state, int64_t c_last_pos,
                                                int64_t c_pend_pos, int pend_stable) {
    const bool pend_in = pend_stable && (cnt == 0 || c_pend_state != c_last_state);
    const int k = cnt + (pend_in ? 1 : 0);
    if (k == 0) return res_identity();
    const uint32_t first_state = cnt > 0 ? c_first_state : c_pend_state;
    const int64_t last_pos = pend_in ? c_pend_pos : c_last_pos;
    const uint32_t last_state = pend_in ? c_pend_state : c_last_state;
    return res_make(first_state, k == 1 ? last_pos : -1, last_state, k - 1, k >= 2, last_pos, last_state);
}

struct TileTail {
    ResElem *ploc;
    ResElem *btot;
    VecK<4> *agg;
    VecK<4> *excl;
    int64_t *tile_off;
    int32_t *tile_cnt;
    int64_t *d_n_tiles;
    int32_t *huge_count;
    int parity;
    int want_bits;
    GranDesc *rdesc;
    unsigned long long epoch;
    int64_t *d_row_base;
    int64_t *esc;
};

__global__ __launch_bounds__(kResolveBlock) void k_resolve_one(const ResolveArgs a, const TileTail ft, const int64_t blk0, const SegGate gate) {
    URH_TAIL_PRIO();
    __shared__ ResElem s_w[kResolveBlock / 64];
    const int64_t blk = blk0 + blockIdx.x;
    const int64_t c = blk * kResolveBlock + threadIdx.x;
    const int t = threadIdx.x, lane = t & 63, wave = t >> 6;
    if (gate.fused) {
        if (t == 0) {
            const uint32_t *ctr = gate.progress + gate.k * kProgressStride;
            const long long t0 = (long long)wall_clock64();
            while (__hip_atomic_load(ctr, __ATOMIC_RELAXED, __HIP_MEMORY_SCOPE_AGENT) < gate.target) {
                __builtin_amdgcn_s_sleep(8);
                if ((long long)wall_clock64() - t0 > gate.max_ticks) { gate.seg->err = 1 + gate.k; break; }
            }
        }
        __syncthreads();
        __builtin_amdgcn_fence(__ATOMIC_ACQUIRE, "agent");
    }
    if (gate.seg && gate.init && blockIdx.x == 0 && t == 0) {
        if (!gate.progress) gate.seg->err = 0;
        int64_t *w = (int64_t *)&gate.seg->in[0];
        for (int i = 0; i < (int)(2 * sizeof(SegState::In) / 8); ++i) w[i] = 0;
    }
    if (blockIdx.x == 0 && t == 0 && ft.want_bits) ft.huge_count[ft.parity] = 0;
    if (blockIdx.x == 0 && t == 0 && ft.esc) ft.esc[0] = 0;
    ResElem e = res_identity();
    if (c < a.n_chunks) {
        ChunkInfo *ch = a.chunks + c;
        const int64_t pend_pos = ch->pend_pos, start = ch->start, len = ch->len, last_pos = ch->last_pos;
        const int cnt = ch->cnt;
        const uint32_t first_state = ch->first_state, last_state = ch->last_state, pend_state = ch->pend_state;
        const bool has_next = c + 1 < a.n_chunks;
        int64_t lead = has_next ? ch[1].lead : 0, nlen = has_next ? ch[1].len : 1;
        int ps = 0;
        if (pend_pos >= 0) {
            int64_t run = start + len - pend_pos;
            for (int64_t u = c + 1; run <= a.tol && u < a.n_chunks; ++u) {
                if (u > c + 1) { lead = a.chunks[u].lead; nlen = a.chunks[u].len; }
                run += lead;
                if (lead < nlen) break;
            }
            ps = run > a.tol;
        }
        ch->pend_stable = ps;
        e = res_of_chunk(cnt, first_state, last_state, pend_state, last_pos, pend_pos, ps);
    }
    const ResElem incl = res_wave_incl_scan(e, lane);
    if (lane == 63) s_w[wave] = incl;
    __syncthreads();
    ResElem base = res_identity(), tot = res_identity();
#pragma unroll
    for (int w = 0; w < kResolveBlock / 64; ++w) {
        if (w < wave) base = res_combine(base, s_w[w]);
        tot = res_combine(tot, s_w[w]);
    }
    ResElem ex = res_shfl_up(incl, 1);
    if (lane == 0) ex = res_identity();
    ex = res_combine(base, ex);
    if (c < a.n_chunks) ft.ploc[c] = ex;
    if (t == 0) ft.btot[blk] = tot;
}

__device__ __forceinline__ ResElem res_fold_blocks(const ResElem *btot, int64_t count, int lane, ResElem first) {
    ResElem carry = res_identity();
    for (int64_t u0 = 0; u0 < count; u0 += 64) {
        ResElem x = first;
        if (u0 > 0) { x = res_identity(); if (u0 + lane < count) x = btot[u0 + lane]; }
        x = res_wave_incl_scan(x, lane);
        carry = res_combine(carry, res_shfl(x, 63));
    }
    return carry;
}

__device__ __forceinline__ ResElem res_before_entry(const TileTail &ft, const ResElem &init, int64_t c, int64_t n_chunks, int lane) {
    const int64_t nb = (c >= n_chunks) ? resolve_blocks(n_chunks) : c / kResolveBlock;
    ResElem first = res_identity();
    if (lane < nb) first = ft.btot[lane];
    ResElem pre = res_combine(init, res_fold_blocks(ft.btot, nb, lane, first));
    if (c < n_chunks) pre = res_combine(pre, ft.ploc[c]);
    return pre;
}

struct ShardPart { ResElem tot; int32_t first_nonlead, open_chunk; };
__global__ __launch_bounds__(kResolveBlock) void k_shard_summary(const ResolveArgs a, ShardPart *part, int32_t *ticket) {
    URH_TAIL_PRIO();
    __shared__ ResElem s_w[kResolveBlock / 64];
    __shared__ int32_t s_fn[kResolveBlock / 64], s_oc[kResolveBlock / 64];
    __shared__ bool s_last;
    const int64_t c = (int64_t)blockIdx.x * kResolveBlock + threadIdx.x;
    const int t = threadIdx.x, lane = t & 63, wave = t >> 6;
    ResElem e = res_identity();
    int32_t fn = kAuxNone, oc = kAuxNone;
    if (c < a.n_chunks) {
        const ChunkInfo *ch = a.chunks + c;
        const int64_t pend_pos = ch->pend_pos, start = ch->start, len = ch->len, last_pos = ch->last_pos, own_lead = ch->lead;
        const int cnt = ch->cnt;
        const uint32_t first_state = ch->first_state, last_state = ch->last_state, pend_state = ch->pend_state;
        const bool has_next = c + 1 < a.n_chunks;
        int64_t lead = has_next ? ch[1].lead : 0, nlen = has_next ? ch[1].len : 1;
        int ps = 0;
        if (pend_pos >= 0) {
            int64_t run = start + len - pend_pos;
            bool hit = false;
            for (int64_t u = c + 1; run <= a.tol && u < a.n_chunks; ++u) {
                if (u > c + 1) { lead = a.chunks[u].lead; nlen = a.chunks[u].len; }
                run += lead;
                if (lead < nlen) { hit = true; break; }
            }
// ... 86 lines not shown
constexpr int kEmitWaves = 4;
#ifndef URH_TAIL_CPW
#define URH_TAIL_CPW 4
#endif
constexpr int kTailCPW = URH_TAIL_CPW;
#ifndef URH_TILE_CHUNKS
#define URH_TILE_CHUNKS URH_TAIL_CPW
#endif
constexpr int kTileChunks = URH_TILE_CHUNKS;
static_assert(kTileChunks >= 1 && kTailCPW % kTileChunks == 0, "a wavefront's chunks are a whole number of tiles");
#ifndef URH_EXPAND_PREFETCH
#define URH_EXPAND_PREFETCH 1
#endif
#ifndef URH_PACK_WORDS
#define URH_PACK_WORDS 1
#endif
#ifndef URH_EXPAND_EARLY_EXIT
#define URH_EXPAND_EARLY_EXIT 1
#endif
#ifdef URH_TAIL_CAP80
#define URH_TAIL_OCC __attribute__((amdgpu_waves_per_eu(URH_TAIL_CAP80)))
#else
#define URH_TAIL_OCC
#endif
#ifdef URH_OCC_EMIT
#define URH_EMIT_OCC __attribute__((amdgpu_waves_per_eu(URH_OCC_EMIT)))
#else
#define URH_EMIT_OCC
#endif
#ifdef URH_OCC_EXPAND
#define URH_EXPAND_OCC __attribute__((amdgpu_waves_per_eu(URH_OCC_EXPAND)))
#else
#define URH_EXPAND_OCC URH_TAIL_OCC
#endif
static_assert(kResolveBlock % kTailCPW == 0 && kTailCPW <= 64, "the chunks of one wavefront share their resolve workgroup");

__device__ __forceinline__ int64_t lane_bcast(int64_t v, int src) {
    const int lo = __builtin_amdgcn_readlane((int)(uint32_t)(uint64_t)v, src), hi = __builtin_amdgcn_readlane((int)(uint32_t)((uint64_t)v >> 32), src);
    return (int64_t)(((uint64_t)(uint32_t)hi << 32) | (uint32_t)lo);
}
__device__ __forceinline__ int lane_bcast(int v, int src) { return __builtin_amdgcn_readlane(v, src); }

struct EmitTileArgs {
    EmitArgs e;
    ResolveArgs r;
    TileTail ft;
    BitsParams bp;
    HugeRef *huge;
    int32_t huge_cap;
    int64_t w0, w_end;
    int final_seg;
    SegState *seg;
    int seg_k;
    int8_t *h_state;
    int32_t *h_len;
    int len16;
    int64_t *esc;
    int64_t esc_cap;
};

__host__ __device__ static inline int64_t tail_waves(int64_t n_items) { return (n_items + kTailCPW - 1) / kTailCPW; }
__host__ __device__ static inline int64_t chunk_tiles(int64_t n_chunks, int tc) { return (n_chunks + tc - 1) / tc; }

__device__ __forceinline__ void ship_row(const EmitTileArgs &g, int64_t idx, int64_t state, int64_t len) {
    if (g.len16 == 2) {
        const bool fits = len >= 0 && len < 0x1FFF;
        ((uint16_t *)g.h_len)[idx] = (uint16_t)((((uint32_t)(state + 1) & 7u) << 13) | (fits ? (uint32_t)len : 0x1FFFu));
        if (!fits) {
            const unsigned long long slot = atomicAdd((unsigned long long *)g.esc, 1ull);
            if ((int64_t)slot < g.esc_cap) g.esc[1 + slot] = (int64_t)(((uint64_t)(uint32_t)(int32_t)len << 32) | (uint64_t)(uint32_t)idx);
        }
        return;
    }
    g.h_state[idx] = (int8_t)state;
    if (!g.len16) { g.h_len[idx] = (int32_t)len; return; }
    const bool fits = len >= 0 && len < 0xFFFF;
    ((uint16_t *)g.h_len)[idx] = fits ? (uint16_t)len : (uint16_t)0xFFFF;
    if (!fits) {
        const unsigned long long slot = atomicAdd((unsigned long long *)g.esc, 1ull);
        if ((int64_t)slot < g.esc_cap) g.esc[1 + slot] = (int64_t)(((uint64_t)(uint32_t)(int32_t)len << 32) | (uint64_t)(uint32_t)idx);
    }
}

template <int TC>
__global__ __launch_bounds__(64 * kEmitWaves) URH_EMIT_OCC void k_emit_rows_tiles(const EmitTileArgs g) {
    URH_TAIL_PRIO();
    const EmitArgs &a = g.e;
    const ResolveArgs &r = g.r;
    const int lane = threadIdx.x & 63;
    const int64_t w = g.w0 + (int64_t)blockIdx.x * kEmitWaves + __builtin_amdgcn_readfirstlane((int)(threadIdx.x >> 6));
    const int64_t n_cw = g.w_end;
    if (w > n_cw) return;
    const bool totals = (w == n_cw);
    const bool table = (r.n_local != r.n_chunks);
    const int64_t lc0 = a.chunk_first, lc1 = a.chunk_first + r.n_local;
    const int64_t c0 = totals ? (g.final_seg ? r.n_chunks : n_cw * kTailCPW) : w * kTailCPW;
    const int64_t n_before = (totals && g.final_seg) ? resolve_blocks(r.n_chunks) : c0 / kResolveBlock;
    const uint32_t init_state = a.chunks[0].init_state;
    ResElem first = res_identity();
    if (lane < n_before) first = g.ft.btot[lane];
    const int n_mine = totals ? 0 : (int)((r.n_chunks - c0 < kTailCPW) ? r.n_chunks - c0 : kTailCPW);
    ResElem pl_l = res_identity();
    int cnt_l = 0, fl_l = 0, pp_l = 0;
    int64_t pend_pos_l = -1, last_pos_l = 0;
    if (lane < n_mine) {
        pl_l = g.ft.ploc[c0 + lane];
        const ChunkInfo *ch = a.chunks + c0 + lane;
        cnt_l = ch->cnt; pend_pos_l = ch->pend_pos;
        if (table) last_pos_l = ch->last_pos;
        fl_l = (int)((uint32_t)ch->first_state | ((uint32_t)ch->last_state << 16));
        pp_l = (int)((uint32_t)ch->pend_state | ((uint32_t)(ch->pend_stable ? 1 : 0) << 16));
    }
    uint64_t rec = 0;
    if (n_mine > 0 && c0 >= lc0 && c0 < lc1 && lane < a.slab_stride)
        rec = (a.slab + (c0 - lc0) * a.slab_stride)[lane];
    const ResElem init = res_make(init_state, -1, init_state, 0, false, -1, 0);
    const ResElem base = res_combine(init, res_fold_blocks(g.ft.btot, n_before, lane, first));
    int64_t row_base = 0;
    if (table) row_base = res_before_entry(g.ft, init, lc0, r.n_chunks, lane).cnt;
    if (totals) {
        const ResElem pre = base;
        if (!g.final_seg) {
            if (lane == 0) g.seg->rows_at[g.seg_k] = (r.rows != nullptr && pre.cnt > r.cap_rows) ? r.cap_rows : pre.cnt;
            return;
        }
        const int64_t c = chunk_tiles(r.n_chunks, TC);
        int64_t row_end = pre.cnt;
        if (table && lc1 < r.n_chunks) row_end = res_before_entry(g.ft, init, lc1, r.n_chunks, lane).cnt;
        if (lane == 0) {
            const int64_t P = pre.cnt;
            *r.d_n_acc = P;
            int64_t n_rows = row_end - row_base;
            int64_t o = n_rows;
            VecK<4> v; v.zero();
            int32_t tcnt = 0;
            if (P < r.n_total && r.write_last_row) {
                o = P - row_base;
                n_rows = o + 1;
                tcnt = 1;
                const int64_t fpos = pre.la_valid() ? pre.la_pos : -1;
                const uint32_t fstate = pre.la_valid() ? pre.la_state() : init_state;
                const int64_t len = (P == 0) ? (r.n_total - r.tol) : (r.n_total - 1 - fpos - r.tol);
                if (r.rows != nullptr && o < r.cap_rows) {
                    r.rows[2 * o] = (int64_t)fstate - 1; r.rows[2 * o + 1] = len;
                    if (g.h_state) ship_row(g, o, (int64_t)fstate - 1, len);
                }
                if (g.ft.want_bits) {
                    v = row_value((int64_t)fstate - 1, len, P == 0, g.bp);
                    if (v.v[0] > kHugeBits) {
                        const int slot = atomicAdd(g.ft.huge_count + g.ft.parity, 1);
                        if (slot < g.huge_cap) { g.huge[slot].tile = c; g.huge[slot].row = o; }
                    }
                }
            }
            *r.d_n_rows_needed = n_rows;
            *r.d_n_rows = (r.rows != nullptr && n_rows > r.cap_rows) ? r.cap_rows : n_rows;
            if (g.ft.d_row_base) *g.ft.d_row_base = row_base;
            g.ft.agg[c] = v; g.ft.tile_off[c] = o; g.ft.tile_cnt[c] = tcnt;
        }
        return;
    }
    int64_t acc_bits = 0;
    uint64_t acc_ld = 0;
    int64_t my_last_pos = 0;
    int64_t t_samples = 0, t_off = 0, t_total = 0;
    for (int jc = 0; jc < n_mine; ++jc) {
        const int64_t c = c0 + jc;
        const bool local = (TC > 1) || (c >= lc0 && c < lc1);
        const uint64_t *slab = a.slab + (c - lc0) * a.slab_stride;
        uint64_t rec_next = 0;
        if (jc + 1 < n_mine && c + 1 >= lc0 && c + 1 < lc1 && lane < a.slab_stride) rec_next = (a.slab + (c + 1 - lc0) * a.slab_stride)[lane];
        ResElem pl;
        pl.cnt = lane_bcast(pl_l.cnt, jc); pl.first_pos = lane_bcast(pl_l.first_pos, jc); pl.la_pos = lane_bcast(pl_l.la_pos, jc);
        pl.meta = (uint64_t)lane_bcast((int64_t)pl_l.meta, jc);
        const int cnt = lane_bcast(cnt_l, jc);
        const uint32_t fl = (uint32_t)lane_bcast(fl_l, jc), pp = (uint32_t)lane_bcast(pp_l, jc);
        const int64_t pend_pos = lane_bcast(pend_pos_l, jc);
        const uint32_t c_first = fl & 0xFFFFu, c_last = fl >> 16, c_pend = pp & 0xFFFFu;
        const int pend_stable = (int)(pp >> 16);
        const ResElem pre = res_combine(base, pl);
        const uint32_t prev_state = pre.last_state();
        const int first_acc = (cnt > 0) && (c_first != prev_state);
        const uint32_t before_pend = (cnt > 0) ? c_last : prev_state;
        const int pend_acc = pend_stable && (c_pend != before_pend);
        const int skip = (cnt > 0 && !first_acc) ? 1 : 0;
        const int64_t from_slab = (cnt > 0) ? cnt - skip : 0;
        const int64_t total = from_slab + pend_acc;
        const int64_t out_off = pre.cnt;
        const int64_t prev_pos = pre.la_valid() ? pre.la_pos : -1;
        const uint32_t prev_st = pre.la_valid() ? pre.la_state() : init_state;
        if (!local) {
            VecK<4> acc; acc.zero();
            if (g.ft.want_bits && total > 0) acc.v[2] = (pend_acc ? pend_pos : lane_bcast(last_pos_l, jc)) - prev_pos;
            if (lane == 0) { g.ft.agg[c] = acc; g.ft.tile_off[c] = 0; g.ft.tile_cnt[c] = 0; }
            rec = rec_next;
            continue;
        }
        if (jc % TC == 0) { acc_bits = 0; acc_ld = 0; t_samples = 0; t_total = 0; t_off = out_off - row_base; }
        const bool in_regs = cnt <= 64;
        const uint64_t rec_j = skip ? (uint64_t)__shfl_down((long long)rec, 1) : rec;
        const uint64_t rec_p = (uint64_t)__shfl_up((long long)rec_j, 1);
        for (int64_t j = lane; j < total; j += 64) {
            int64_t pos, ppos; uint32_t pst;
            if (in_regs && j < 64) {
                pos = (j < from_slab) ? rec_pos(rec_j) : pend_pos;
                if (j == 0) { ppos = prev_pos; pst = prev_st; }
                else { ppos = rec_pos(rec_p); pst = rec_state(rec_p); }
            } else {
                pos = (j < from_slab) ? rec_pos(slab[j + skip]) : pend_pos;
                if (j == 0) { ppos = prev_pos; pst = prev_st; }
                else { const uint64_t rr = slab[j - 1 + skip]; ppos = rec_pos(rr); pst = rec_state(rr); }
            }
            my_last_pos = pos;
            const int64_t gi = out_off + j;
            const int64_t len = (gi == 0) ? pos + 1 : pos - ppos;
            const int64_t state = (int64_t)pst - 1;
            if (gi - row_base < a.cap_rows) {
                if (a.rows) *(longlong2 *)(a.rows + 2 * (gi - row_base)) = longlong2{(long long)state, (long long)len};
                if (g.h_state) ship_row(g, gi - row_base, state, len);
            }
            if (g.ft.want_bits) {
                const VecK<4> v = row_value(state, len, gi == 0, g.bp);
                acc_bits += v.v[0];
                acc_ld += (uint64_t)v.v[1] | ((uint64_t)v.v[3] << 32);
                if (v.v[0] > kHugeBits) {
                    const int slot = atomicAdd(g.ft.huge_count + g.ft.parity, 1);
                    if (slot < g.huge_cap) { g.huge[slot].tile = c / TC; g.huge[slot].row = gi - row_base; }
                }
            }
        }
        if (g.ft.want_bits && total > 0) t_samples += lane_bcast(my_last_pos, (int)((total - 1) & 63)) - prev_pos;
        t_total += total;
        if (jc % TC == TC - 1 || jc == n_mine - 1) {
            VecK<4> acc; acc.zero();
            if (g.ft.want_bits && t_total > 0) {
#pragma unroll
                for (int o = 32; o > 0; o >>= 1) { acc_bits += __shfl_xor(acc_bits, o); acc_ld += (uint64_t)__shfl_xor((long long)acc_ld, o); }
                acc.v[0] = acc_bits; acc.v[1] = (int64_t)(acc_ld & 0xFFFFFFFFull); acc.v[3] = (int64_t)(acc_ld >> 32);
                acc.v[2] = t_samples;
            }
            if (lane == 0) { g.ft.agg[c / TC] = acc; g.ft.tile_off[c / TC] = t_off; g.ft.tile_cnt[c / TC] = (int32_t)t_total; }
        }
        rec = rec_next;
    }
}

struct TileScanArgs {
    const int64_t *rows;
    const int64_t *d_n_rows;
    const VecK<4> *agg;
    const int64_t *tile_off;
    const int32_t *tile_cnt;
    VecK<4> *excl;
    GroupInfo *groups;
    int64_t cap_groups;
    int64_t *d_n_groups;
    int64_t n_tiles;
    BitsParams bp;
    GranDesc *desc;
    unsigned long long epoch;
    int64_t b0, t_base;
    SegState *seg;
    int seg_parity;
};
__global__ __launch_bounds__(kScanBlock) URH_TAIL_OCC void k_tile_scan(const TileScanArgs a) {
    URH_TAIL_PRIO();
    __shared__ VecK<4> s_wave[kScanBlock / 64];
    __shared__ VecK<4> s_prefix;
    __shared__ VecK<4> s_ex[kScanBlock];
    __shared__ int64_t s_off[kScanBlock], s_end[kScanBlock];
    __shared__ int s_count;
    const int64_t b = a.b0 + blockIdx.x, nb = a.b0 + gridDim.x;
    const int64_t t = a.t_base + (int64_t)blockIdx.x * kScanBlock + threadIdx.x;
    const int lane = threadIdx.x & 63, wave = threadIdx.x >> 6;
    const int64_t n = *a.d_n_rows;
    const bool row0g = !a.bp.d_row_base || *a.bp.d_row_base == 0;
    VecK<4> mine; mine.zero();
    int64_t off = 0; int32_t cnt = 0;
    if (t < a.n_tiles) { mine = a.agg[t]; off = a.tile_off[t]; cnt = a.tile_cnt[t]; }
    if (threadIdx.x == 0) s_count = 0;
    VecK<4> total;
    VecK<4> ex = block_excl_scan_vec<4>(mine, total, s_wave);
    if (threadIdx.x < 64) {
        const uint32_t tag = (uint32_t)a.epoch;
        if (threadIdx.x == 0) gran_store(a.desc[b].agg, total, tag);
        VecK<4> zero; zero.zero();
        bool ok;
        const VecK<4> prefix = gran_look_back<VecK<4>>(a.desc, b, tag, zero,
                                                         [](const VecK<4> &l, const VecK<4> &r) { VecK<4> x = l; x.add(r); return x; },
                                                         [](const VecK<4> &x, int o) { VecK<4> r; for (int k = 0; k < 4; ++k) r.v[k] = __shfl_down(x.v[k], o); return r; },
                                                         [](const VecK<4> &x) { VecK<4> r; for (int k = 0; k < 4; ++k) r.v[k] = __shfl(x.v[k], 0); return r; },
                                                         lane, ok);
        if (threadIdx.x == 0) {
            VecK<4> incl = prefix; incl.add(total);
            gran_store(a.desc[b].incl, incl, tag);
            s_prefix = prefix;
            if (b == nb - 1) {
                int64_t g = (n > 0) ? incl.v[1] + 1 : 0;
                if (g > a.cap_groups) g = a.cap_groups;
                *a.d_n_groups = g;
                if (a.seg) {
                    const int64_t g0 = a.seg->in[a.seg_parity].g0;
                    a.seg->n_groups_local = (g > g0) ? g - g0 : 0;
                }
            }
        }
    }
    __syncthreads();
    ex.add(s_prefix);
    int64_t end = off + cnt;
    if (end > n) end = n;
    if (t < a.n_tiles) {
        a.excl[t] = ex;
        if (end > off && (mine.v[1] > 0 || end == n)) {
            const int slot = atomicAdd(&s_count, 1);
            s_ex[slot] = ex; s_off[slot] = off; s_end[slot] = end;
        }
    }
    __syncthreads();
    const int n_list = s_count;
    for (int w = wave; w < n_list; w += kScanBlock / 64) {
        const int64_t o = s_off[w], e = s_end[w];
        VecK<4> run = s_ex[w];
        for (int64_t i0 = o; i0 < e; i0 += 64) {
            const int64_t i = i0 + lane;
            VecK<4> v; v.zero();
            int64_t type = 0, len = 0;
            if (i < e) {
                const longlong2 row = *(const longlong2 *)(a.rows + 2 * i);
                type = row.x; len = row.y;
                v = row_value(type, len, i == 0 && row0g, a.bp);
            }
            const VecK<4> incl = wave_incl_scan_vec<4>(v, lane);
            VecK<4> before = run;
#pragma unroll
            for (int k = 0; k < 4; ++k) before.v[k] += incl.v[k] - v.v[k];
            if (i < e && v.v[1] && before.v[1] < a.cap_groups) {
                GroupInfo gi;
                gi.bits_end = before.v[0]; gi.data_end = before.v[3]; gi.ts_close = before.v[2]; gi.pause = len; gi.closed = 1; gi.pad = 0;
                a.groups[before.v[1]] = gi;
            }
            if (i < e && i + 1 == n && before.v[1] + v.v[1] < a.cap_groups) {
                GroupInfo gi;
                gi.bits_end = before.v[0] + v.v[0]; gi.data_end = before.v[3] + v.v[3]; gi.ts_close = before.v[2] + v.v[2];
                gi.pause = (type == -1) ? len : 0;
                gi.closed = 0; gi.pad = 0;
                a.groups[before.v[1] + v.v[1]] = gi;
            }
#pragma unroll
            for (int k = 0; k < 4; ++k) run.v[k] += __shfl(incl.v[k], 63);
        }
    }
}

struct ExpandTileArgs {
    const int64_t *rows;
    const int64_t *d_n_rows;
    const VecK<4> *agg;
    const VecK<4> *excl;
    const int64_t *tile_off;
    const int32_t *tile_cnt;
    const GroupOut *gout;
    const int64_t *d_n_groups;
    uint8_t *bits; int64_t cap_bits;
    int64_t *pos; int64_t cap_pos;
    BitsParams bp;
    const HugeRef *huge;
    int32_t *huge_count;
    int32_t huge_cap;
    int parity;
    int64_t n_tiles;
    int64_t t_base;
    uint32_t *h_pos;
};
constexpr unsigned kHugeBlocksX = 16, kHugeBlocksY = 16;

__host__ __device__ static inline int64_t expand_tile_blocks(int64_t n_tiles, int tc) {
    const int64_t tpw = kTailCPW / tc;
    return ((n_tiles + tpw - 1) / tpw + kEmitWaves - 1) / kEmitWaves;
}

template <int TC>
__global__ __launch_bounds__(64 * kEmitWaves) URH_EXPAND_OCC void k_expand_tiles(const ExpandTileArgs a) {
    constexpr int kTPW = kTailCPW / TC;
    URH_TAIL_PRIO();
    const int lane = threadIdx.x & 63, wave = __builtin_amdgcn_readfirstlane((int)(threadIdx.x >> 6));
    const int bps = (int)a.bp.bps;
    const int64_t tile_blocks = expand_tile_blocks(a.n_tiles - a.t_base, TC);
    if ((int64_t)blockIdx.x >= tile_blocks) {
        const int64_t n = *a.d_n_rows;
        const bool row0g = !a.bp.d_row_base || *a.bp.d_row_base == 0;
        const int64_t hb = (int64_t)blockIdx.x - tile_blocks;
        const int hx = (int)(hb % kHugeBlocksX), hy = (int)(hb / kHugeBlocksX);
        if (hb == 0 && threadIdx.x == 0) a.huge_count[a.parity ^ 1] = 0;
        int cnt = a.huge_count[a.parity];
        if (cnt > a.huge_cap) cnt = 0;
        __shared__ int64_t s_h[5];
        for (int w = hy; w < cnt; w += kHugeBlocksY) {
            const HugeRef h = a.huge[w];
            __syncthreads();
            if (h.tile < a.t_base || h.tile >= a.n_tiles || h.row < a.tile_off[h.tile] || h.row >= a.tile_off[h.tile] + a.tile_cnt[h.tile]) continue;
            if (wave == 0) {
                VecK<4> run = a.excl[h.tile];
                const int64_t off = a.tile_off[h.tile];
                for (int64_t i0 = off; i0 <= h.row; i0 += 64) {
                    const int64_t i = i0 + lane;
                    VecK<4> v; v.zero();
                    if (i < h.row && i < n) v = row_value(a.rows[2 * i], a.rows[2 * i + 1], i == 0 && row0g, a.bp);
                    run.add(wave_sum_vec<4>(v));
                }
                if (lane == 0) {
                    int64_t kb = 0, ob = 0, op = 0, ty = 0;
                    if (h.row < n && run.v[1] < *a.d_n_groups) {
                        const GroupOut go = a.gout[run.v[1]];
                        if (go.is_msg) {
                            ty = a.rows[2 * h.row];
                            kb = row_value(ty, a.rows[2 * h.row + 1], h.row == 0 && row0g, a.bp).v[0];
                            ob = go.out_bits + (run.v[0] - go.bits_start);
                            op = go.out_pos + (run.v[0] - go.bits_start);
                        }
                    }
                    s_h[0] = kb; s_h[1] = ob; s_h[2] = op; s_h[3] = run.v[2]; s_h[4] = ty;
                }
            }
            __syncthreads();
            const int64_t kb = s_h[0], ob = s_h[1], op = s_h[2], ts = s_h[3], ty = s_h[4];
            for (int64_t k = (int64_t)hx * blockDim.x + threadIdx.x; k < kb; k += (int64_t)kHugeBlocksX * blockDim.x) {
                const int sh = (bps == 1) ? 0 : bps - 1 - (int)(k % bps);
                const uint8_t b = (ty < 0) ? 0 : (uint8_t)((ty >> sh) & 1);
                if (ob + k < a.cap_bits) a.bits[ob + k] = b;
                if (a.bp.write_pos && op + k < a.cap_pos) {
                    a.pos[op + k] = ts + k * a.bp.samples_per_bit;
                    if (a.h_pos) a.h_pos[op + k] = (uint32_t)(ts + k * a.bp.samples_per_bit);
                }
            }
        }
        return;
    }
    const int64_t t0 = a.t_base + ((int64_t)blockIdx.x * kEmitWaves + wave) * kTPW;
    if (t0 >= a.n_tiles) return;
    const int n_mine = (int)((a.n_tiles - t0 < kTPW) ? a.n_tiles - t0 : kTPW);
    const int64_t n = *a.d_n_rows;
    const int64_t n_groups = *a.d_n_groups;
    const bool row0g = !a.bp.d_row_base || *a.bp.d_row_base == 0;
    const int hc = a.huge_count[a.parity];
    int64_t off_l = 0; int32_t tcnt_l = 0;
    VecK<4> run_l; run_l.zero();
    int narrow_l = 0;
    if (lane < n_mine) {
        off_l = a.tile_off[t0 + lane]; tcnt_l = a.tile_cnt[t0 + lane]; run_l = a.excl[t0 + lane];
        const int64_t tb = a.agg[t0 + lane].v[0], tsm = a.agg[t0 + lane].v[2];
        narrow_l = (tb >= 0 && tb < (int64_t(1) << 31) && tsm >= 0 && tsm < (int64_t(1) << 31)) ? 1 : 0;
    }
    const int64_t own_limit = (hc > a.huge_cap) ? INT64_MAX : kHugeBits;
    GroupOut go_l; go_l.bits_start = 0; go_l.out_bits = 0; go_l.out_pos = 0; go_l.is_msg = 0; go_l.pad = 0;
    if (lane < n_mine && run_l.v[1] < n_groups) go_l = a.gout[run_l.v[1]];
    const int64_t off_first = lane_bcast(off_l, 0);
    int64_t end_first = off_first + lane_bcast((int)tcnt_l, 0);
    if (end_first > n) end_first = n;
    longlong2 row0 = longlong2{0, 0};
    if (off_first + lane < end_first) row0 = *(const longlong2 *)(a.rows + 2 * (off_first + lane));
    for (int jt = 0; jt < n_mine; ++jt) {
        const int64_t off = lane_bcast(off_l, jt);
        const int32_t tcnt = lane_bcast((int)tcnt_l, jt);
        const bool narrow = lane_bcast(narrow_l, jt) != 0;
        VecK<4> run;
        run.v[0] = lane_bcast(run_l.v[0], jt); run.v[1] = lane_bcast(run_l.v[1], jt); run.v[2] = lane_bcast(run_l.v[2], jt); run.v[3] = 0;
        GroupOut go0;
        go0.bits_start = lane_bcast(go_l.bits_start, jt); go0.out_bits = lane_bcast(go_l.out_bits, jt); go0.out_pos = lane_bcast(go_l.out_pos, jt);
        go0.is_msg = lane_bcast((int)go_l.is_msg, jt); go0.pad = 0;
        int64_t end = off + tcnt;
        if (end > n) end = n;
        longlong2 row_next = longlong2{0, 0};
        if (jt + 1 < n_mine) {
            const int64_t off_n = lane_bcast(off_l, jt + 1);
            int64_t end_n = off_n + lane_bcast((int)tcnt_l, jt + 1);
            if (end_n > n) end_n = n;
            if (off_n + lane < end_n) row_next = *(const longlong2 *)(a.rows + 2 * (off_n + lane));
        }
        const int64_t g0 = run.v[1];
        longlong2 row_cur = row0;
        for (int64_t i0 = off; i0 < end; i0 += 64) {
            const int64_t i = i0 + lane;
            VecK<4> v; v.zero();
            int64_t type = 0;
#if URH_EXPAND_PREFETCH
            longlong2 row_pf = longlong2{0, 0};
            if (i + 64 < end) row_pf = *(const longlong2 *)(a.rows + 2 * (i + 64));
            if (i < end) {
                type = row_cur.x;
                v = row_value(type, row_cur.y, i == 0 && row0g, a.bp);
            }
            row_cur = row_pf;
#else
            if (i < end) {
                const longlong2 row = (i0 == off) ? row0 : *(const longlong2 *)(a.rows + 2 * i);
                type = row.x;
                v = row_value(type, row.y, i == 0 && row0g, a.bp);
            }
#endif
            int64_t in_bits = v.v[0], in_ts = v.v[2];
            int in_l = (int)v.v[1];
#if URH_DPP_SCAN
            in_bits = wave_incl_sum_dpp(in_bits); in_ts = wave_incl_sum_dpp(in_ts); in_l = wave_incl_sum_dpp(in_l);
#else
            if (narrow) {
                uint32_t b32 = (uint32_t)v.v[0], t32 = (uint32_t)v.v[2];
#pragma unroll
                for (int o = 1; o < 64; o <<= 1) {
                    const uint32_t ub = (uint32_t)__shfl_up((int)b32, o), ut = (uint32_t)__shfl_up((int)t32, o);
                    const int ul = __shfl_up(in_l, o);
                    if (lane >= o) { b32 += ub; t32 += ut; in_l += ul; }
                }
                in_bits = (int64_t)b32; in_ts = (int64_t)t32;
            } else {
#pragma unroll
                for (int o = 1; o < 64; o <<= 1) {
                    const int64_t ub = __shfl_up(in_bits, o), ut = __shfl_up(in_ts, o);
                    const int ul = __shfl_up(in_l, o);
                    if (lane >= o) { in_bits += ub; in_ts += ut; in_l += ul; }
                }
            }
#endif
            int64_t kb = 0, ob = 0, op = 0, ts = 0;
            if (i < end && v.v[0] > 0 && v.v[0] <= own_limit) {
                const int64_t grp = run.v[1] + in_l - v.v[1];
                if (grp < n_groups) {
                    GroupOut go = go0;
                    if (grp != g0) go = a.gout[grp];
                    if (go.is_msg) {
                        const int64_t bit_prefix = run.v[0] + in_bits - v.v[0];
                        kb = v.v[0];
                        ob = go.out_bits + (bit_prefix - go.bits_start);
                        op = go.out_pos + (bit_prefix - go.bits_start);
                        ts = run.v[2] + in_ts - v.v[2];
                    }
                }
            }
            constexpr int kShort = 16;
#if URH_EXPAND_EARLY_EXIT
            {
                const int kbs = (kb > 0 && kb <= kShort) ? (int)kb : 0;
                const int nb = (ob + kbs <= a.cap_bits) ? kbs : (int)((a.cap_bits > ob) ? a.cap_bits - ob : 0);
                const int np = !a.bp.write_pos ? 0 : ((op + kbs <= a.cap_pos) ? kbs : (int)((a.cap_pos > op) ? a.cap_pos - op : 0));
                uint8_t *bp8 = a.bits + ob;
                int64_t *pp = a.pos + op;
                uint32_t *hp = a.h_pos ? a.h_pos + op : nullptr;
                int64_t tsk = ts;
                int sh = bps - 1;
#pragma unroll 1
                for (int k = 0; k < kShort; ++k) {
                    if (__ballot(k < kbs) == 0ull) break;
                    const uint8_t b = (type < 0) ? 0 : (uint8_t)((type >> sh) & 1);
                    sh = (sh == 0) ? bps - 1 : sh - 1;
                    if (k < nb) bp8[k] = b;
                    if (k < np) { pp[k] = tsk; if (hp) hp[k] = (uint32_t)tsk; }
                    tsk += a.bp.samples_per_bit;
                }
            }
#else
            if (kb > 0 && kb <= kShort) {
                const int nb = (ob + kb <= a.cap_bits) ? (int)kb : (int)((a.cap_bits > ob) ? a.cap_bits - ob : 0);
                const int np = !a.bp.write_pos ? 0 : ((op + kb <= a.cap_pos) ? (int)kb : (int)((a.cap_pos > op) ? a.cap_pos - op : 0));
                uint8_t *bp8 = a.bits + ob;
                int64_t *pp = a.pos + op;
                uint32_t *hp = a.h_pos ? a.h_pos + op : nullptr;
                int64_t tsk = ts;
                int sh = bps - 1;
                for (int k = 0; k < (int)kb; ++k) {
                    const uint8_t b = (type < 0) ? 0 : (uint8_t)((type >> sh) & 1);
                    sh = (sh == 0) ? bps - 1 : sh - 1;
                    if (k < nb) bp8[k] = b;
                    if (k < np) { pp[k] = tsk; if (hp) hp[k] = (uint32_t)tsk; }
                    tsk += a.bp.samples_per_bit;
                }
            }
#endif
            unsigned long long big = __ballot(kb > kShort);
            while (big) {
                const int src = __builtin_ctzll(big);
                big &= big - 1;
                const int64_t kb_s = __shfl(kb, src), ob_s = __shfl(ob, src), op_s = __shfl(op, src), ts_s = __shfl(ts, src),
                              ty_s = __shfl(type, src);
                for (int64_t k = lane; k < kb_s; k += 64) {
                    const uint8_t b = symbol_bit(ty_s, k, bps);
                    if (ob_s + k < a.cap_bits) a.bits[ob_s + k] = b;
                    if (a.bp.write_pos && op_s + k < a.cap_pos) {
                        a.pos[op_s + k] = ts_s + k * a.bp.samples_per_bit;
                        if (a.h_pos) a.h_pos[op_s + k] = (uint32_t)(ts_s + k * a.bp.samples_per_bit);
                    }
                }
            }
            run.v[0] += lane_bcast(in_bits, 63); run.v[1] += lane_bcast(in_l, 63); run.v[2] += lane_bcast(in_ts, 63);
        }
        row0 = row_next;
    }
}

int launch_resolve(const ResolveArgs &a, int32_t *tickets, hipStream_t s) {
    if (a.n_chunks <= 0) return URHGPU_ERR_ARG;
    const unsigned g = (unsigned)((a.n_chunks + kResolveBlock - 1) / kResolveBlock);
    (void)tickets;
    hipLaunchKernelGGL(k_resolve_a, dim3(g), dim3(kResolveBlock), 0, s, a);
    hipLaunchKernelGGL(k_resolve_b, dim3(g), dim3(kResolveBlock), 0, s, a);
    hipLaunchKernelGGL(k_resolve_c, dim3(g), dim3(kResolveBlock), 0, s, a);
    return URHGPU_OK;
}

int launch_shard_summary(const ResolveArgs &a, int32_t *ticket, hipStream_t s) {
    if (a.n_chunks <= 0 || !a.local_pass || !a.summary_out || a.n_chunks >= kAuxNone) return URHGPU_ERR_ARG;
    static_assert(sizeof(ShardPart) <= 256 && sizeof(ShardPart) <= (size_t)kResolveBlock * 8, "one partial per kResolveBlock chunks fits the out_cnt section (8 bytes per chunk, 256-byte granules)");
    const unsigned g = (unsigned)resolve_blocks(a.n_chunks);
    hipLaunchKernelGGL(k_shard_summary, dim3(g), dim3(kResolveBlock), 0, s, a, (ShardPart *)a.sc.out_cnt, ticket);
    return URHGPU_OK;
}

int launch_resolve_emit_single(const ResolveArgs &r, const EmitArgs &e, hipStream_t s) {
    if (r.n_chunks <= 0 || r.local_pass || r.chunk_first != 0 || r.n_local != r.n_chunks || e.chunk_first != 0) return URHGPU_ERR_ARG;
    const unsigned g = (unsigned)((r.n_chunks + kResolveBlock - 1) / kResolveBlock);
    hipLaunchKernelGGL(k_resolve_a, dim3(g), dim3(kResolveBlock), 0, s, r);
    hipLaunchKernelGGL(k_resolve_b, dim3(g), dim3(kResolveBlock), 0, s, r);
    hipLaunchKernelGGL(k_emit_rows_fused, dim3((unsigned)r.n_chunks), dim3(64), 0, s, e, r);
    return URHGPU_OK;
}

int launch_emit_rows(const EmitArgs &a, int64_t n_local_chunks, hipStream_t s) {
    if (n_local_chunks > 0) hipLaunchKernelGGL(k_emit_rows, dim3((unsigned)n_local_chunks), dim3(64), 0, s, a);
    return URHGPU_OK;
}

static inline int64_t scan_blocks(int64_t cap) { return (cap + kScanTile - 1) / kScanTile; }
constexpr int kGroupItems = 1;
static inline int64_t group_scan_blocks(int64_t cap) { return (cap + kScanBlock * kGroupItems - 1) / (kScanBlock * kGroupItems); }

size_t merge_scratch_bytes(int64_t cap) {
    return (size_t)(scan_blocks(cap) + 1) * sizeof(VecK<2>) + 256 + (size_t)cap * 16 + 512;
}

int launch_merge_rows_ask(const int64_t *rows_in, const int64_t *d_n_in, int64_t cap, int64_t *rows_out,
                          int64_t cap_out, int64_t *d_n_out, void *scratch, int32_t *tickets, hipStream_t s) {
    if (cap <= 0) return URHGPU_OK;
    const int64_t nb = scan_blocks(cap);
    char *p = (char *)scratch;
    VecK<2> *partials = (VecK<2> *)p; p += ((size_t)(nb + 1) * sizeof(VecK<2>) + 255) & ~size_t(255);
    int64_t *grp_state = (int64_t *)p; p += (size_t)cap * 8;
    int64_t *grp_end = (int64_t *)p;
    MergeLoad ld{rows_in};
    MergeStore st{rows_in, d_n_in, grp_state, grp_end};
    (void)tickets;
    hipLaunchKernelGGL((k_scan_reduce<2, MergeLoad>), dim3(scan_grid(nb)), dim3(kScanBlock), 0, s, d_n_in, ld, partials, nb);
    hipLaunchKernelGGL((k_scan_apply<2, MergeLoad, MergeStore>), dim3(scan_grid(nb)), dim3(kScanBlock), 0, s, d_n_in, ld, partials, nb, st,
                       kScanAlwaysDirect);
    hipLaunchKernelGGL((k_scan_finish<2, NoFinal>), dim3(1), dim3(kScanBlock), 0, s, d_n_in, partials, nb, NoFinal(), kScanAlwaysDirect);
    int64_t fin_blocks = (cap + 255) / 256; if (fin_blocks > 4096) fin_blocks = 4096;
    hipLaunchKernelGGL(k_merge_finish, dim3((unsigned)fin_blocks), dim3(256), 0, s, partials + nb, grp_state, grp_end,
                       rows_out, cap_out, d_n_out);
    return URHGPU_OK;
}

size_t bits_scratch_bytes(int64_t cap_rows) {
    const int64_t nb = scan_blocks(cap_rows);
    const int64_t cap_groups = cap_rows + 1;
    const int64_t nbg = group_scan_blocks(cap_groups);
    return (size_t)(nb + 1) * sizeof(VecK<4>) + (size_t)(nbg + 1) * sizeof(VecK<3>) + (size_t)cap_rows * sizeof(RowInfo) +
           (size_t)cap_groups * (sizeof(GroupInfo) + sizeof(GroupOut)) + 64 + 8 * 256 + 64 + 256 +
           (size_t)kHugeCap * sizeof(HugeRow) + 256;
}

namespace {
struct BitsScratch {
    VecK<4> *part4; VecK<3> *part3; RowInfo *info; GroupInfo *groups; GroupOut *gout; int64_t *d_n_groups;
    HugeRow *huge; int32_t *huge_count;
    int64_t nb, nbg;
};
BitsScratch carve_bits(void *scratch, int64_t cap_rows) {
    BitsScratch b;
    b.nb = scan_blocks(cap_rows);
    const int64_t cap_groups = cap_rows + 1;
// ... 21 lines not shown
        const int64_t n = *d_n_rows;
        const int64_t n_l = (n > 0) ? grand.v[1] : 0;
        *d_n_groups = (n > 0) ? n_l + 1 : 0;
        if (d_flags) {
            d_flags[0] = n_l > 0;
            d_flags[1] = (n > 0) && groups[0].data_end > 0;
            d_flags[2] = (n > 0) && (groups[n_l].data_end - (n_l ? groups[n_l - 1].data_end : 0) > 0);
        }
    }
};

size_t bits_desc_bytes(int64_t cap_rows) {
    if (cap_rows <= 0) cap_rows = 1;
    return (((size_t)(scan_blocks(cap_rows) + 1) * sizeof(ScanDesc<4>) + 255) & ~size_t(255)) + (size_t)(group_scan_blocks(cap_rows + 1) + 1) * sizeof(ScanDesc<3>) + 512;
}

int launch_bits_prepare(const int64_t *rows, const int64_t *d_n_rows, int64_t cap_rows, const BitsParams &bp,
                        void *scratch, int64_t *d_flags, const ScanState &ss, hipStream_t s) {
    if (cap_rows <= 0) cap_rows = 1;
    if (ss.desc_bytes < bits_desc_bytes(cap_rows)) return URHGPU_ERR_ARG;
    const BitsScratch b = carve_bits(scratch, cap_rows);
    const bool single = (d_flags == nullptr);
    BitsLoad ld{rows, d_n_rows, bp, single ? b.d_n_groups : nullptr};
    BitsStore st{rows, d_n_rows, b.info, b.groups, bp.d_ts_carry, bp.d_absorbed, single ? b.d_n_groups : nullptr};
    GroupCountFinal fin{d_n_rows, b.groups, b.d_n_groups, d_flags};
    hipLaunchKernelGGL((k_scan_reduce<4, BitsLoad>), dim3(scan_grid(b.nb)), dim3(kScanBlock), 0, s, d_n_rows, ld, b.part4, b.nb);
    hipLaunchKernelGGL((k_scan_apply<4, BitsLoad, BitsStore>), dim3(scan_grid(b.nb)), dim3(kScanBlock), 0, s, d_n_rows, ld, b.part4, b.nb, st,
                       kScanAlwaysDirect);
    if (!single)
        hipLaunchKernelGGL((k_scan_finish<4, GroupCountFinal>), dim3(1), dim3(kScanBlock), 0, s, d_n_rows, b.part4, b.nb, fin, kScanAlwaysDirect);
    return URHGPU_OK;
}

int launch_bits_finish(const int64_t *rows, const int64_t *d_n_rows, int64_t cap_rows, const BitsParams &bp,
                       const BitsOut &o, void *scratch, const ScanState &ss, hipStream_t s) {
    if (cap_rows <= 0) cap_rows = 1;
    if (ss.desc_bytes < bits_desc_bytes(cap_rows)) return URHGPU_ERR_ARG;
    const BitsScratch b = carve_bits(scratch, cap_rows);
    ScanDesc<3> *desc3 = (ScanDesc<3> *)((char *)ss.desc + (((size_t)(b.nb + 1) * sizeof(ScanDesc<4>) + 255) & ~size_t(255)));
    GroupLoad gl{b.groups, b.d_n_groups, bp.d_extra, bp.is_last_rank, bp.write_pos};
    GroupStore gs{gl, b.gout, o.msg_off, o.pauses, o.pos_off, o.pos, o.cap_msg, o.cap_pos};
    BitsCountsFinal fin{d_n_rows, o.msg_off, o.pos_off, o.counts, b.huge_count, bp.d_rows_needed, o.h_counts};
    if (!(g_tail_skip & 8))
        hipLaunchKernelGGL((k_scan_lookback<3, GroupLoad, GroupStore, BitsCountsFinal, kGroupItems>), dim3(scan_grid(b.nbg)), dim3(kScanBlock), 0, s,
                           b.d_n_groups, gl, desc3, b.nbg, gs, fin, ++*ss.epoch, ss.tickets + 2, 0);
    ExpandArgs ea{rows, d_n_rows, b.info, b.gout, o.bits, o.cap_bits, o.pos, o.cap_pos, bp, b.huge, b.huge_count, kHugeCap};
    const int64_t eb = std::min<int64_t>((cap_rows + 255) / 256, kExpandMaxBlocks);
    hipLaunchKernelGGL(k_expand_bits, dim3((unsigned)eb), dim3(256), 0, s, ea);
    hipLaunchKernelGGL(k_expand_huge, dim3(kHugeGridX, kHugeGridY), dim3(256), 0, s, ea);
    return URHGPU_OK;
}

int launch_ppseq_to_bits(const int64_t *rows, const int64_t *d_n_rows, int64_t cap_rows, const BitsParams &bp,
                         const BitsOut &o, void *scratch, const ScanState &ss, hipStream_t s) {
    URH_TRY(launch_bits_prepare(rows, d_n_rows, cap_rows, bp, scratch, nullptr, ss, s));
    return launch_bits_finish(rows, d_n_rows, cap_rows, bp, o, scratch, ss, s);
}


int g_tail_skip = 0;
namespace {
constexpr int kTileHugeCap = 8192;
struct TileCarve { TileTail ft; HugeRef *huge; };
TileCarve carve_tile(const TileTailMem &m) {
    TileCarve tc;
    char *p = (char *)m.mem;
    auto take = [&](size_t bytes) { char *r = p; p += (bytes + 255) & ~size_t(255); return r; };
    const int64_t nt = m.n_chunks + 1;
    tc.ft.ploc = (ResElem *)take((size_t)m.n_chunks * sizeof(ResElem));
    tc.ft.btot = (ResElem *)take((size_t)(resolve_blocks(m.n_chunks) + 1) * sizeof(ResElem));
    tc.ft.agg = (VecK<4> *)take((size_t)nt * sizeof(VecK<4>));
    tc.ft.excl = (VecK<4> *)take((size_t)nt * sizeof(VecK<4>));
    tc.ft.tile_off = (int64_t *)take((size_t)nt * 8);
    tc.ft.tile_cnt = (int32_t *)take((size_t)nt * 4);
    tc.ft.d_n_tiles = (int64_t *)take(64);
    tc.huge = (HugeRef *)take((size_t)kTileHugeCap * sizeof(HugeRef));
    tc.ft.huge_count = m.huge_count;
    tc.ft.parity = m.parity;
    tc.ft.want_bits = 0;
    tc.ft.rdesc = (GranDesc *)m.rdesc;
    tc.ft.epoch = m.epoch;
    tc.ft.d_row_base = m.d_row_base;
    tc.ft.esc = nullptr;
    return tc;
}
}

static inline int tile_chunks_of(const TileTailMem &m) { return m.d_row_base ? 1 : kTileChunks; }

int64_t tile_desc_cap(int64_t cap_rows, int64_t n_chunks) { return std::max<int64_t>(cap_rows, 8 * (n_chunks + 2) + kScanTile); }

static inline int64_t tile_scan_blocks_tc(int64_t c0, int64_t c1, int final, int tc) {
    const int64_t t1 = final ? chunk_tiles(c1, tc) + 1 : c1 / tc;
    return (t1 - c0 / tc + kScanBlock - 1) / kScanBlock;
}
int64_t tile_scan_blocks(int64_t c0, int64_t c1, int final) { return tile_scan_blocks_tc(c0, c1, final, kTileChunks); }

size_t tile_rdesc_bytes(int64_t n_chunks) {
    return (size_t)(resolve_blocks(n_chunks) + 2 + (n_chunks + 1 + kScanBlock - 1) / kScanBlock + kMaxSegments + 2) * sizeof(GranDesc);
}

size_t tile_tail_bytes(int64_t n_chunks) {
    const int64_t nt = n_chunks + 1;
    return (size_t)n_chunks * sizeof(ResElem) + (size_t)(resolve_blocks(n_chunks) + 1) * sizeof(ResElem) + (size_t)nt * (2 * sizeof(VecK<4>) + 12) +
           64 + (size_t)kTileHugeCap * sizeof(HugeRef) + 10 * 256;
}

int launch_tile_rows(const ResolveArgs &r, const EmitArgs &e, const TileTailMem &m, const BitsParams *bp, hipStream_t s) {
    if (r.n_chunks <= 0 || r.local_pass || r.chunk_first != e.chunk_first || r.chunk_first < 0 || r.chunk_first + r.n_local > r.n_chunks ||
        m.n_chunks != r.n_chunks || e.is_ask)
        return URHGPU_ERR_ARG;
    if ((r.n_local != r.n_chunks) != (m.d_row_base != nullptr)) return URHGPU_ERR_ARG;
    TileCarve tc = carve_tile(m);
    EmitTileArgs g;
    g.e = e; g.r = r; g.ft = tc.ft; g.huge = tc.huge; g.huge_cap = kTileHugeCap;
    memset(&g.bp, 0, sizeof(g.bp));
    if (bp) { g.bp = *bp; g.ft.want_bits = 1; }
    const unsigned gb = (unsigned)resolve_blocks(r.n_chunks);
    g.w0 = 0; g.w_end = tail_waves(r.n_chunks); g.final_seg = 1; g.seg = nullptr; g.seg_k = 0; g.h_state = nullptr; g.h_len = nullptr; g.len16 = 0; g.esc = nullptr; g.esc_cap = 0; g.ft.esc = nullptr;
    SegGate no_gate;
    memset(&no_gate, 0, sizeof(no_gate));
    if (!(g_tail_skip & 1)) hipLaunchKernelGGL(k_resolve_one, dim3(gb), dim3(kResolveBlock), 0, s, r, g.ft, (int64_t)0, no_gate);
    const dim3 grid((unsigned)((tail_waves(r.n_chunks) + 1 + kEmitWaves - 1) / kEmitWaves));
    if (!(g_tail_skip & 2)) {
        if (tile_chunks_of(m) == 1) hipLaunchKernelGGL(k_emit_rows_tiles<1>, grid, dim3(64 * kEmitWaves), 0, s, g);
        else hipLaunchKernelGGL(k_emit_rows_tiles<kTileChunks>, grid, dim3(64 * kEmitWaves), 0, s, g);
    }
    return URHGPU_OK;
}

namespace {
__global__ void k_tile_flags(const int64_t *d_n_rows, const GroupInfo *groups, const int64_t *d_n_groups, int64_t *d_flags) {
    const int64_t n = *d_n_rows, ng = *d_n_groups;
    const int64_t n_l = (n > 0 && ng > 0) ? ng - 1 : 0;
    d_flags[0] = n_l > 0;
    d_flags[1] = (n > 0) && groups[0].data_end > 0;
    d_flags[2] = (n > 0) && (groups[n_l].data_end - (n_l ? groups[n_l - 1].data_end : 0) > 0);
}
}

int launch_tile_bits_prepare(const TileTailMem &m, const int64_t *rows, const int64_t *d_n_rows, int64_t cap_rows, const BitsParams &bp,
                             void *scratch, int64_t *d_flags, const ScanState &ss, hipStream_t s) {
    if (cap_rows <= 0) cap_rows = 1;
    const int64_t nt = chunk_tiles(m.n_chunks, tile_chunks_of(m)) + 1;
    const int64_t cap_desc = tile_desc_cap(cap_rows, m.n_chunks);
    if (ss.desc_bytes < bits_desc_bytes(cap_desc)) return URHGPU_ERR_ARG;
    const TileCarve tc = carve_tile(m);
    const BitsScratch b = carve_bits(scratch, cap_rows);
    const int64_t cap_groups = cap_rows + 1;
    GranDesc *tdesc = (GranDesc *)m.rdesc + resolve_blocks(m.n_chunks) + 2;
    TileScanArgs ta{rows, d_n_rows, tc.ft.agg, tc.ft.tile_off, tc.ft.tile_cnt, tc.ft.excl, b.groups, cap_groups, b.d_n_groups, nt, bp, tdesc,
                    m.epoch, 0, 0, nullptr, 0};
    const unsigned nb_ts = (unsigned)((nt + kScanBlock - 1) / kScanBlock);
    if (!(g_tail_skip & 4)) hipLaunchKernelGGL(k_tile_scan, dim3(nb_ts), dim3(kScanBlock), 0, s, ta);
    if (d_flags) hipLaunchKernelGGL(k_tile_flags, dim3(1), dim3(1), 0, s, d_n_rows, b.groups, b.d_n_groups, d_flags);
    return URHGPU_OK;
}

int launch_tile_bits_finish(const TileTailMem &m, const int64_t *rows, const int64_t *d_n_rows, int64_t cap_rows, const BitsParams &bp,
                            const BitsOut &o, void *scratch, const ScanState &ss, hipStream_t s) {
    if (cap_rows <= 0) cap_rows = 1;
    const int tch = tile_chunks_of(m);
    const int64_t nt = chunk_tiles(m.n_chunks, tch) + 1;
    const int64_t cap_desc = tile_desc_cap(cap_rows, m.n_chunks);
    if (ss.desc_bytes < bits_desc_bytes(cap_desc)) return URHGPU_ERR_ARG;
    const TileCarve tc = carve_tile(m);
    const BitsScratch b = carve_bits(scratch, cap_rows);
    ScanDesc<3> *desc3 = (ScanDesc<3> *)((char *)ss.desc + (((size_t)(scan_blocks(cap_desc) + 1) * sizeof(ScanDesc<4>) + 255) & ~size_t(255)));
    GroupLoad gl{b.groups, b.d_n_groups, bp.d_extra, bp.is_last_rank, bp.write_pos};
    GroupStore gs{gl, b.gout, o.msg_off, o.pauses, o.pos_off, o.pos, o.cap_msg, o.cap_pos};
    BitsCountsFinal fin{d_n_rows, o.msg_off, o.pos_off, o.counts, b.huge_count, bp.d_rows_needed, o.h_counts};
    if (!(g_tail_skip & 8))
        hipLaunchKernelGGL((k_scan_lookback<3, GroupLoad, GroupStore, BitsCountsFinal, kGroupItems>), dim3(scan_grid(b.nbg)), dim3(kScanBlock), 0, s,
                           b.d_n_groups, gl, desc3, b.nbg, gs, fin, ++*ss.epoch, ss.tickets + 2, 0);
    ExpandTileArgs ea{rows, d_n_rows, tc.ft.agg, tc.ft.excl, tc.ft.tile_off, tc.ft.tile_cnt, b.gout, b.d_n_groups, o.bits, o.cap_bits, o.pos, o.cap_pos,
                      bp, tc.huge, m.huge_count, kTileHugeCap, m.parity, nt, 0, nullptr};
    const dim3 grid((unsigned)expand_tile_blocks(nt, tch) + kHugeBlocksX * kHugeBlocksY);
    if (!(g_tail_skip & 16)) {
        if (tch == 1) hipLaunchKernelGGL(k_expand_tiles<1>, grid, dim3(64 * kEmitWaves), 0, s, ea);
        else hipLaunchKernelGGL(k_expand_tiles<kTileChunks>, grid, dim3(64 * kEmitWaves), 0, s, ea);
    }
    return URHGPU_OK;
}

int launch_tile_bits(const TileTailMem &m, const int64_t *rows, const int64_t *d_n_rows, int64_t cap_rows, const BitsParams &bp,
                     const BitsOut &o, void *scratch, const ScanState &ss, hipStream_t s) {
    URH_TRY(launch_tile_bits_prepare(m, rows, d_n_rows, cap_rows, bp, scratch, nullptr, ss, s));
    return launch_tile_bits_finish(m, rows, d_n_rows, cap_rows, bp, o, scratch, ss, s);
}

__global__ void k_seg_gate(const SegGate gate) {
    if (threadIdx.x != 0) return;
    if (gate.init) gate.seg->err = 0;
    if (!gate.progress) return;
    const uint32_t *ctr = gate.progress + gate.k * kProgressStride;
    const long long t0 = (long long)wall_clock64();
    while (__hip_atomic_load(ctr, __ATOMIC_RELAXED, __HIP_MEMORY_SCOPE_AGENT) < gate.target) {
        __builtin_amdgcn_s_sleep(16);
        if ((long long)wall_clock64() - t0 > gate.max_ticks) { gate.seg->err = 1 + gate.k; break; }
    }
}

struct SegGroupLoad {
    GroupLoad ld;
    const SegState *seg;
    int parity;
    __device__ VecK<3> operator()(int64_t i) const { return ld(seg->in[parity].g0 + i); }
};
struct SegGroupStore {
// ... 62 lines not shown
    uint32_t *progress;
    int pos_shipped;
    int split;
    char *head;
    const int64_t *esc;
    int64_t esc_cap;
    int64_t row16_esc_off;
};
__global__ __launch_bounds__(256) void k_pack_seg(const SegPack a) {
    URH_TAIL_PRIO();
    const int64_t gtid = blockIdx.x * 256ll + threadIdx.x, stride = (int64_t)gridDim.x * 256;
    const SegState::In in = a.seg->in[a.parity];
    auto lim = [](int64_t x, int64_t cap) { return x < cap ? (x < 0 ? 0 : x) : cap; };
    const int64_t nbits = lim(a.seg->end_bits, a.cap_bits);
    const int64_t j0 = lim(in.ship_bits, a.cap_bits) / 8, j1 = a.final ? (nbits + 7) / 8 : nbits / 8;
    const int64_t p0 = a.has_pos ? lim(in.ship_pos, a.cap_pos) : 0, p1 = a.has_pos ? lim(a.seg->end_pos, a.cap_pos) : 0;
    const int64_t m0 = lim(in.ship_msgs, a.cap_msg), m1 = lim(a.seg->end_msgs, a.cap_msg);
    BlobLayout L = a.L;
    if (a.split) {
        const int64_t c5[5] = {0, m1, nbits, 0, 0};
        const BlobLayout T = blob_layout(c5, a.cap_rows, a.cap_bits, a.cap_msg, a.cap_pos, 0);
        L.off_pauses = T.off_pauses; L.off_msg_off = T.off_msg_off; L.off_pos_off = T.off_pos_off; L.off_bits = T.off_bits;
    }
    {
        uint8_t *out = (uint8_t *)(a.head + L.off_bits);
        const unsigned long long *in8 = (const unsigned long long *)a.bits;
        auto pack8 = [&](int64_t j) -> unsigned long long {
            unsigned long long w;
            if (8 * j + 8 <= nbits) w = in8[j];
            else { w = 0; for (int k = 0; k < 8 && 8 * j + k < nbits; ++k) w |= (unsigned long long)a.bits[8 * j + k] << (8 * k); }
            return ((w & 0x0101010101010101ull) * 0x8040201008040201ull) >> 56;
        };
#if URH_PACK_WORDS
        int64_t ja = j0 + (int64_t)((8 - ((uintptr_t)(out + j0) & 7)) & 7);
        if (ja > j1) ja = j1;
        int64_t nw = (j1 - ja) / 8;
        const int64_t full = nbits / 8;
        if (ja + 8 * nw > full) nw = full > ja ? (full - ja) / 8 : 0;
        for (int64_t k = gtid; k < nw; k += stride) {
            const int64_t j = ja + 8 * k;
            unsigned long long r = 0;
#pragma unroll
            for (int b = 0; b < 8; ++b) r |= (((in8[j + b] & 0x0101010101010101ull) * 0x8040201008040201ull) >> 56) << (8 * b);
            *(unsigned long long *)(out + j) = r;
        }
        for (int64_t j = j0 + gtid; j < ja; j += stride) out[j] = (uint8_t)pack8(j);
        for (int64_t j = ja + 8 * nw + gtid; j < j1; j += stride) out[j] = (uint8_t)pack8(j);
#else
        for (int64_t j = j0 + gtid; j < j1; j += stride) out[j] = (uint8_t)pack8(j);
#endif
    }
    if (a.has_pos && !a.pos_shipped) {
        uint32_t *p32 = (uint32_t *)(a.host + L.off_pos32);
        for (int64_t i = p0 + gtid; i < p1; i += stride) p32[i] = (uint32_t)a.pos[i];
    }
    {
        int64_t *pa = (int64_t *)(a.head + L.off_pauses), *mo = (int64_t *)(a.head + L.off_msg_off), *po = (int64_t *)(a.head + L.off_pos_off);
        if (gtid == 0 && m0 == 0) { mo[0] = 0; po[0] = 0; }
        for (int64_t i = m0 + gtid; i < m1; i += stride) { pa[i] = a.pauses[i]; mo[i + 1] = a.msg_off[i + 1]; po[i + 1] = a.pos_off[i + 1]; }
    }
    int64_t n_esc = 0;
    if (a.esc && a.final) {
        n_esc = a.esc[0];
        const bool over = n_esc > a.esc_cap;
        if (over) n_esc = a.esc_cap;
        int64_t *dst = (int64_t *)(a.head + (a.row16_esc_off > 0 ? a.row16_esc_off : ((L.off_bits + (nbits + 7) / 8 + 15) & ~int64_t(15))));
        if (gtid == 0) dst[0] = over ? -n_esc : n_esc;
        for (int64_t i = gtid; i < n_esc; i += stride) dst[1 + i] = a.esc[1 + i];
    }
    if (a.final && gtid == 0) {
        int64_t *hdr = (int64_t *)a.head;
        const int64_t *c = a.counts;
        const int64_t n_rows = lim(*a.d_n_rows, a.cap_rows);
        hdr[1] = n_rows; hdr[2] = m1; hdr[3] = nbits; hdr[4] = p1; hdr[5] = c[4];
        const bool row16 = a.esc && a.row16_esc_off > 0;
        hdr[6] = URHGPU_BLOB_HEADER_BYTES + n_rows * (row16 ? 2 : (a.esc ? 3 : 5)) + (a.esc ? 8 + n_esc * 8 : 0) + (nbits + 7) / 8 + p1 * 4 + m1 * 24 + 16;
        hdr[7] = a.has_pos | (row16 ? URHGPU_BLOB_ROW16 : (a.esc ? URHGPU_BLOB_LEN16 : 0));
        hdr[8] = L.off_pauses; hdr[9] = L.off_msg_off; hdr[10] = L.off_pos_off; hdr[11] = row16 ? a.row16_esc_off : L.off_row_state; hdr[12] = L.off_bits;
        hdr[13] = L.off_row_len; hdr[14] = L.off_pos32;
        hdr[15] = ((c[1] > a.cap_msg || c[2] > a.cap_bits || (a.has_pos && c[3] > a.cap_pos) || c[4] > a.cap_rows) ? 1 : 0) | (a.seg->err ? 2 : 0);
        hdr[0] = URHGPU_BLOB_MAGIC;
    }
    if (a.final && a.progress && gtid < kMaxSegments) a.progress[gtid * kProgressStride] = 0;
}

int launch_rows_segment(const ResolveArgs &r, const EmitArgs &e, const TileTailMem &m, const BitsParams &bp, SegState *state, const RowsSegment &sg,
                        hipStream_t s) {
    if (r.n_chunks <= 0 || r.local_pass || r.chunk_first != 0 || e.chunk_first != 0 || r.n_local != r.n_chunks || m.n_chunks != r.n_chunks ||
        e.is_ask || m.d_row_base != nullptr || !state || sg.index < 0 || sg.index >= kMaxSegments)
        return URHGPU_ERR_ARG;
    if (sg.c0 < 0 || sg.c0 % kSegAlign || sg.c1 <= sg.c0 || sg.c1 > r.n_chunks || (sg.final ? sg.c1 != r.n_chunks : (sg.c1 % kSegAlign != 0 || sg.c1 >= r.n_chunks)))
        return URHGPU_ERR_ARG;
    static_assert(kSegAlign % kResolveBlock == 0 && kSegAlign % kScanBlock == 0 && kSegAlign % (kTailCPW * kEmitWaves) == 0, "segment alignment");
    if (sg.final && (r.d_n_rows != &state->rows_at[sg.index] || r.d_n_rows_needed != &state->rows_needed)) return URHGPU_ERR_ARG;
    if ((sg.h_state == nullptr) != (sg.h_len == nullptr) || sg.gate.seg != state) return URHGPU_ERR_ARG;
    const TileCarve tc = carve_tile(m);
    EmitTileArgs g;
    g.e = e; g.r = r; g.ft = tc.ft; g.huge = tc.huge; g.huge_cap = kTileHugeCap;
    g.bp = bp; g.ft.want_bits = 1;
    g.w0 = sg.c0 / kTailCPW; g.w_end = sg.final ? tail_waves(r.n_chunks) : sg.c1 / kTailCPW; g.final_seg = sg.final; g.seg = state; g.seg_k = sg.index;
    g.h_state = sg.h_state; g.h_len = sg.h_len;
    g.len16 = (sg.len16 && sg.esc && sg.h_len) ? sg.len16 : 0; g.esc = g.len16 ? sg.esc : nullptr; g.esc_cap = sg.esc_cap;
    g.ft.esc = (g.len16 && sg.index == 0) ? sg.esc : nullptr;
    if (g_tail_skip & 64) { g.h_state = nullptr; g.h_len = nullptr; }
    if (g_tail_skip & 128) g.e.rows = nullptr;
    TileTail ft_resolve = g.ft;
    if (sg.index != 0) ft_resolve.want_bits = 0;
    SegGate gate = sg.gate;
    gate.fused = (sg.fuse_gate && gate.progress && !gate.init && resolve_blocks(sg.c1 - sg.c0) == 1) ? 1 : 0;
    if (!gate.fused && gate.progress) hipLaunchKernelGGL(k_seg_gate, dim3(1), dim3(64), 0, s, gate);
    if (!(g_tail_skip & 1)) hipLaunchKernelGGL(k_resolve_one, dim3((unsigned)resolve_blocks(sg.c1 - sg.c0)), dim3(kResolveBlock), 0, s, r, ft_resolve, sg.c0 / kResolveBlock, gate);
    if (!(g_tail_skip & 2)) hipLaunchKernelGGL(k_emit_rows_tiles<kTileChunks>, dim3((unsigned)((g.w_end - g.w0 + 1 + kEmitWaves - 1) / kEmitWaves)), dim3(64 * kEmitWaves), 0, s, g);
    return URHGPU_OK;
}

int launch_bits_segment(const TileTailMem &m, const BitsParams &bp, const BitsOut &o, void *scratch, const ScanState &ss, int64_t *rows,
                        int64_t cap_rows, const BitsSegment &sg, const SegPackDst *dst, hipStream_t s) {
    if (m.n_chunks <= 0 || m.d_row_base != nullptr || !sg.state || sg.rows_index < 0 || sg.rows_index >= kMaxSegments) return URHGPU_ERR_ARG;
    if (sg.c0 < 0 || sg.c0 % kSegAlign || sg.c1 <= sg.c0 || sg.c1 > m.n_chunks || (sg.final ? sg.c1 != m.n_chunks : (sg.c1 % kSegAlign != 0 || sg.c1 >= m.n_chunks)))
        return URHGPU_ERR_ARG;
    if (cap_rows <= 0) cap_rows = 1;
    const int64_t cap_desc = tile_desc_cap(cap_rows, m.n_chunks);
    if (ss.desc_bytes < bits_desc_bytes(cap_desc)) return URHGPU_ERR_ARG;
    const TileCarve tc = carve_tile(m);
    const BitsScratch b = carve_bits(scratch, cap_rows);
    SegState *st = sg.state;
    const int64_t *d_n_rows = &st->rows_at[sg.rows_index];
    const int parity = sg.index & 1;
    if (sg.scan_b0 < 0 || sg.scan_b0 + tile_scan_blocks(sg.c0, sg.c1, sg.final) > (m.n_chunks + 1 + kScanBlock - 1) / kScanBlock + kMaxSegments) return URHGPU_ERR_ARG;
    const int64_t t0 = sg.c0 / kTileChunks, t1 = sg.final ? chunk_tiles(m.n_chunks, kTileChunks) + 1 : sg.c1 / kTileChunks;
    const int64_t cap_groups = cap_rows + 1;
    GranDesc *tdesc = (GranDesc *)m.rdesc + resolve_blocks(m.n_chunks) + 2;
    TileScanArgs ta{rows, d_n_rows, tc.ft.agg, tc.ft.tile_off, tc.ft.tile_cnt, tc.ft.excl, b.groups, cap_groups, &st->n_groups, t1, bp, tdesc,
                    m.epoch, sg.scan_b0, t0, st, parity};
    if (!(g_tail_skip & 4)) hipLaunchKernelGGL(k_tile_scan, dim3((unsigned)tile_scan_blocks(sg.c0, sg.c1, sg.final)), dim3(kScanBlock), 0, s, ta);
    ScanDesc<3> *desc3 = (ScanDesc<3> *)((char *)ss.desc + (((size_t)(scan_blocks(cap_desc) + 1) * sizeof(ScanDesc<4>) + 255) & ~size_t(255)));
    GroupLoad gl{b.groups, &st->n_groups, nullptr, sg.final ? 1 : 0, bp.write_pos, sg.final ? 0 : 1};
    const int has_pos = (bp.write_pos && o.pos) ? 1 : 0;
    const int64_t caps[5] = {cap_rows, o.cap_msg, o.cap_bits, o.cap_pos, cap_rows};
    BlobLayout L = blob_layout(caps, cap_rows, o.cap_bits, o.cap_msg, o.cap_pos, has_pos);
    const bool split = dst && dst->host && dst->split;
    if (split) {
        if (!sg.final || sg.c0 != 0) return URHGPU_ERR_ARG;
        const StagedLayout SL = staged_layout(cap_rows, o.cap_bits, o.cap_msg, o.cap_pos, has_pos);
        L.off_row_state = SL.off_row_state; L.off_row_len = SL.off_row_len; L.off_pos32 = SL.off_pos32;
    }
    const bool pos_direct = dst && dst->host && has_pos && sg.final && sg.c0 == 0 && dst->pos_direct;
    uint32_t *h_pos = pos_direct ? (uint32_t *)((char *)dst->host + L.off_pos32) : nullptr;
    GroupStore gs{gl, b.gout, o.msg_off, o.pauses, o.pos_off, o.pos, o.cap_msg, o.cap_pos, h_pos};
    SegGroupLoad sl{gl, st, parity};
    SegGroupStore sst{gs, st, parity};
    SegFinal fin{sl, st, d_n_rows, parity, sg.final ? 1 : 0, BitsCountsFinal{d_n_rows, o.msg_off, o.pos_off, o.counts, b.huge_count, &st->rows_needed, o.h_counts}};
    if (!(g_tail_skip & 8))
        hipLaunchKernelGGL((k_scan_lookback<3, SegGroupLoad, SegGroupStore, SegFinal, kGroupItems>), dim3((unsigned)std::min<int64_t>(scan_grid(b.nbg), 32)),
                           dim3(kScanBlock), 0, s, &st->n_groups_local, sl, desc3, b.nbg, sst, fin, ++*ss.epoch, ss.tickets + 2, 0);
    ExpandTileArgs ea{rows, d_n_rows, tc.ft.agg, tc.ft.excl, tc.ft.tile_off, tc.ft.tile_cnt, b.gout, &st->n_groups, o.bits, o.cap_bits, o.pos, o.cap_pos,
                      bp, tc.huge, m.huge_count, kTileHugeCap, m.parity, t1, t0, h_pos};
    const unsigned tile_blocks = (unsigned)expand_tile_blocks(t1 - t0, kTileChunks);
    if (g_tail_skip & 2048) ea.cap_bits = 0;
    if (!(g_tail_skip & 16)) hipLaunchKernelGGL(k_expand_tiles<kTileChunks>, dim3(tile_blocks + kHugeBlocksX * kHugeBlocksY), dim3(64 * kEmitWaves), 0, s, ea);
    if (dst && dst->host) {
        if (((uintptr_t)o.bits & 7) || ((uintptr_t)dst->host & 15)) return URHGPU_ERR_ARG;
        SegPack pk{o.bits, o.msg_off, o.pauses, o.pos_off, o.pos, o.counts, cap_rows, o.cap_bits, o.cap_msg, o.cap_pos, has_pos, (char *)dst->host,
                   L, st, d_n_rows, parity, sg.final ? 1 : 0, sg.final ? dst->progress_reset : nullptr, pos_direct ? 1 : 0, split ? 1 : 0,
                   (split && dst->host_head) ? (char *)dst->host_head : (char *)dst->host, split ? dst->esc : nullptr, dst->esc_cap,
                   (split && dst->esc) ? dst->row16_esc_off : 0};
        if (dst->cap_host < pk.L.total) return URHGPU_ERR_CAPACITY;
        if (!(g_tail_skip & 32)) hipLaunchKernelGGL(k_pack_seg, dim3(dst->blocks > 0 ? dst->blocks : 32), dim3(256), 0, s, pk);
    }
    return URHGPU_OK;
}

__global__ void k_merge_summary(const int64_t *rows, const int64_t *d_n_rows, int64_t *out5) {
    const int64_t n = *d_n_rows;
    out5[0] = n;
    out5[1] = n ? rows[0] : 0; out5[2] = n ? rows[1] : 0;
    out5[3] = n ? rows[2 * (n - 1)] : 0; out5[4] = n ? rows[2 * (n - 1) + 1] : 0;
}
void launch_merge_summary(const int64_t *rows, const int64_t *d_n_rows, int64_t *d_out5, hipStream_t s) {
    hipLaunchKernelGGL(k_merge_summary, dim3(1), dim3(1), 0, s, rows, d_n_rows, d_out5);
}

__global__ void k_merge_fix(int64_t *rows, const int64_t *d_n_rows, const int64_t *all, int rank, int world, int64_t *d_absorbed) {
    const int64_t n = *d_n_rows;
    *d_absorbed = -1;
    if (n == 0) return;
    auto M = [&](int q, int k) { return all[5 * q + k]; };
    int prev = -1;
    for (int q = rank - 1; q >= 0; --q) if (M(q, 0) > 0) { prev = q; break; }
    const bool absorbed = prev >= 0 && M(prev, 3) == rows[0];
    if (!(absorbed && n == 1)) {
        const int64_t last_state = rows[2 * (n - 1)];
        for (int q = rank + 1; q < world; ++q) {
            if (M(q, 0) == 0) continue;
            if (M(q, 1) != last_state) break;
            rows[2 * (n - 1) + 1] += M(q, 2);
            if (M(q, 0) > 1) break;
        }
    }
    if (absorbed) {
        if (n == 1 && rows[0] == -1) {
            int64_t tot = rows[1];
            for (int q = rank + 1; q < world; ++q) tot += (M(q, 0) > 0) ? M(q, 2) : 0;
            for (int q = rank - 1; q >= 0; --q) {
                if (M(q, 0) == 0) continue;
                tot += M(q, 4);
                if (M(q, 0) > 1) break;
                int pq = -1;
                for (int u = q - 1; u >= 0; --u) if (M(u, 0) > 0) { pq = u; break; }
                if (!(pq >= 0 && M(pq, 3) == M(q, 1))) break;
            }
            *d_absorbed = tot;
        }
        rows[0] = kRowAbsorbed;
    }
}
void launch_merge_fix(int64_t *rows, const int64_t *d_n_rows, const int64_t *d_all, int rank, int world,
                      int64_t *d_absorbed, hipStream_t s) {
    hipLaunchKernelGGL(k_merge_fix, dim3(1), dim3(1), 0, s, rows, d_n_rows, d_all, rank, world, d_absorbed);
}

__global__ void k_bits_extra(const int64_t *all, int rank, int world, int32_t *extra) {
    int head = 0, tail = 0;
    for (int q = rank - 1; q >= 0; --q) { head |= (int)all[3 * q + 2]; if (all[3 * q]) break; }
    for (int q = rank + 1; q < world; ++q) { tail |= (int)all[3 * q + 1]; if (all[3 * q]) break; }
    extra[0] = head; extra[1] = tail;
}
void launch_bits_extra(const int64_t *d_all, int rank, int world, int32_t *d_extra, hipStream_t s) {
    hipLaunchKernelGGL(k_bits_extra, dim3(1), dim3(1), 0, s, d_all, rank, world, d_extra);
}

}
```

urh_amd/csrc/stream_pass.hip:

```cpp
#include "pass.hpp"

namespace urh {

static int segment_bounds(int64_t n_chunks, int wanted, int shape, int last_units, int64_t *bound ) {
    const int64_t blocks = n_chunks / kSegAlign;
    int S = wanted;
    if (S > kMaxSegments) S = kMaxSegments;
    if (S > blocks) S = (int)blocks;
    if (S < 1) S = 1;
    bound[0] = 0;
    if (shape == 1 && S > 2) {
        int64_t left = blocks, at = 0;
        for (int k = 0; k < S - 1; ++k) {
            int64_t take = left / 2;
            const int64_t must_leave = S - 1 - k;
            if (take < 1) take = 1;
            if (left - take < must_leave) take = left - must_leave;
            at += take; left -= take;
            bound[k + 1] = at * kSegAlign;
        }
    } else if (shape == 2 && S > 1) {
        int64_t last = last_units < 1 ? 1 : last_units;
        if (last > blocks - (S - 1)) last = blocks - (S - 1);
        const int64_t rest = blocks - last;
// ... 1 lines not shown
    } else {
        for (int k = 1; k < S; ++k) bound[k] = (blocks * k / S) * kSegAlign;
    }
    bound[S] = n_chunks;
    for (int k = 0; k < S; ++k)
        if (bound[k + 1] <= bound[k]) return 0;
    return S;
}

namespace {
struct StreamPass {
    urhgpu_ctx *ctx; const void *d_iq; int64_t n; const urhgpu_params *p; const urhgpu_outputs *out;
    const void *h_iq;
    void *host_blob; int64_t cap_host;
    void *real_host_blob;
    Plan pl; RunArgs a;
    int S; int64_t bound[kMaxSegments + 1]; uint32_t target[kMaxSegments];
    bool direct, to_stage;
    BitsParams bp; int has_pos; BlobLayout host_layout;
    int slot; uint32_t *progress; SegState *st;
    hipStream_t s; hipEvent_t hot_done;
    ChunkInfo *chunks; uint64_t *slab; void *rs_mem, *scratch; TileTailMem tm; ScanState ss;
    int policy(void *stage_blob);
    int begin();
    int hot();
    int tail(hipEvent_t ev_ready, hipEvent_t ev_rows, int len16);
};
}

int StreamPass::policy(void *stage_blob) {
    S = 0;
    int segs = runs_streamable(a) ? segment_bounds(pl.n_chunks, h_iq ? ctx->tune_upload_pieces : ctx->tune_stream_segments, h_iq ? 2 : 0, 1, bound) : 0;
    int policy = ctx->tune_stream_policy;
    if (policy == 5) policy = (p->write_bit_sample_pos && out->pos && !ctx->tune_stream_pos_direct) ? 0 : (ctx->tune_stream_latency ? 4 : (stage_blob ? 6 : 3));
    if (policy == 6 && !stage_blob) policy = 3;
    direct = to_stage = false;
    if (!h_iq && runs_streamable(a) && host_blob && (policy == 3 || policy == 6)) { direct = true; to_stage = (policy == 6); }
    if (segs < 2 && !direct) return URHGPU_OK;
    if (policy == 2 && !h_iq) return URHGPU_OK;
    if ((policy == 0 || policy == 4) && ctx->passes_begun > 0 && !h_iq) {
        const hipError_t q = hipEventQuery(ctx->ev_tail[(ctx->flip + 2) % 3]);
        if (q == hipErrorNotReady) {
            (void)hipGetLastError();
            if (policy == 0 || !host_blob) return URHGPU_OK;
            direct = true; to_stage = (stage_blob != nullptr);
        } else if (q != hipSuccess) URH_HIP(q);
    }
    S = segs;
    if (direct) { S = 1; bound[0] = 0; bound[1] = pl.n_chunks; }
    real_host_blob = host_blob;
    if (to_stage) host_blob = stage_blob;
    return URHGPU_OK;
}

static int stream_resources(urhgpu_ctx *ctx) {
    if (ctx->d_seg) return URHGPU_OK;
    URH_HIP(hipMalloc(&ctx->d_seg, 3 * kSegBlockBytes));
    URH_HIP(hipMemset(ctx->d_seg, 0, 3 * kSegBlockBytes));
    URH_HIP(hipDeviceSynchronize());
    URH_HIP(hipStreamCreateWithFlags(&ctx->bits_stream, hipStreamNonBlocking));
    for (int k = 0; k < kMaxSegments; ++k) URH_HIP(hipEventCreateWithFlags(&ctx->ev_piece[k], hipEventDisableTiming));
    for (int k = 0; k < 3; ++k) {
        URH_HIP(hipEventCreateWithFlags(&ctx->ev_hot_done[k], hipEventDisableTiming));
        URH_HIP(hipEventCreateWithFlags(&ctx->ev_bits[k], hipEventDisableTiming));
        for (int j = 0; j < kMaxSegments; ++j) URH_HIP(hipEventCreateWithFlags(&ctx->ev_rows[k][j], hipEventDisableTiming));
    }
    return URHGPU_OK;
}

int StreamPass::begin() {
    URH_TRY(stream_resources(ctx));
    bp = bits_params(p);
    has_pos = (bp.write_pos && out->pos) ? 1 : 0;
    memset(&host_layout, 0, sizeof(host_layout));
    if (host_blob) {
        const int64_t caps[5] = {out->cap_rows, out->cap_msg, out->cap_bits, out->cap_pos, out->cap_rows};
        host_layout = blob_layout(caps, out->cap_rows, out->cap_bits, out->cap_msg, out->cap_pos, has_pos);
        if (cap_host < host_layout.total) return URHGPU_ERR_CAPACITY;
    }
    URH_TRY(begin_pipelined_pass(ctx));
    slot = ctx->flip;
    progress = (uint32_t *)((char *)ctx->d_seg + (size_t)slot * kSegBlockBytes);
    st = (SegState *)((char *)progress + kMaxSegments * kProgressStride * 4);
    static_assert(kMaxSegments * kProgressStride * 4 + sizeof(SegState) <= kSegBlockBytes && kMaxSegments <= 16, "segment block");
    if (ctx->seg_dirty[slot]) {
        URH_HIP(hipDeviceSynchronize());
        URH_HIP(hipMemset(progress, 0, kSegBlockBytes));
        URH_HIP(hipDeviceSynchronize());
        ctx->seg_dirty[slot] = false;
    }
    URH_TRY(ctx->arena.reserve(digitize_scratch_bytes(pl, out->cap_rows, false, true)));
    ctx->arena.reset();
    ctx->seg_dirty[slot] = true;
    s = ctx->stream;
    URH_TRY(hot_stream_begin(ctx, &s));
    chunks = (ChunkInfo *)ctx->arena.take((size_t)pl.n_chunks * sizeof(ChunkInfo));
    slab = (uint64_t *)ctx->arena.take((size_t)pl.n_chunks * pl.slab_stride * 8);
    rs_mem = ctx->arena.take(resolve_scratch_bytes(pl.n_chunks));
    if (!chunks || !slab || !rs_mem) return URHGPU_ERR_ARG;
    a.chunks = chunks; a.slab = slab;
    URH_TRY(tile_tail_mem(ctx, pl.n_chunks, true, &tm));
    const int64_t cap = std::max<int64_t>(out->cap_rows, 1);
    scratch = ctx->arena.take(bits_scratch_bytes(cap));
    if (!scratch) return URHGPU_ERR_ARG;
    URH_TRY(scan_state(ctx, tile_desc_cap(cap, pl.n_chunks), &ss));
    a.progress = progress; a.n_seg = S;
    for (int k = 0; k < S; ++k) {
        const int64_t hi = (k < S - 1) ? bound[k + 1] + 1 : pl.n_chunks, lo = (k == 0) ? 0 : bound[k] + 1;
        a.seg_end[k] = (int32_t)hi;
        target[k] = (uint32_t)(hi - lo);
    }
    return URHGPU_OK;
}

int StreamPass::hot() {
    if (h_iq) {
        a.progress = nullptr; a.n_seg = 0;
        const size_t bps = (size_t)dtype_bytes(p->dtype);
        int64_t piece_lo[kMaxSegments], piece_hi[kMaxSegments];
        for (int k = 0; k < S; ++k) {
            piece_lo[k] = k == 0 ? 0 : piece_hi[k - 1];
            piece_hi[k] = (k < S - 1) ? std::min<int64_t>(bound[k + 1] + 1, pl.n_chunks) : pl.n_chunks;
        }
        hipStream_t up = s;
        for (int k = 0; k < S; ++k) {
            {
                const int64_t s0 = piece_lo[k] * pl.chunk_len, s1 = std::min<int64_t>(piece_hi[k] * pl.chunk_len, n);
                URH_HIP(hipMemcpyAsync((char *)const_cast<void *>(d_iq) + (size_t)s0 * bps, (const char *)h_iq + (size_t)s0 * bps, (size_t)(s1 - s0) * bps,
                                       hipMemcpyHostToDevice, up));
            }
            a.launch_lo = piece_lo[k]; a.launch_hi = piece_hi[k];
            const int stl = launch_demod_runs_iq(a, p->dtype, p->mod, out->qad != nullptr, s);
            if (stl != URHGPU_OK) return stl;
            URH_HIP(hipEventRecord(ctx->ev_piece[k], s));
        }
        a.launch_lo = 0; a.launch_hi = 0;
        URH_HIP(hipEventRecord(ctx->ev_hot_done[slot], s));
        hot_done = ctx->ev_hot_done[slot];
        return URHGPU_OK;
    }
    if (direct) { a.progress = nullptr; a.n_seg = 0; }
    return hot_launch(ctx, a, p, true, s, true, ctx->ev_hot_done[slot], nullptr, &hot_done);
}

int StreamPass::tail(hipEvent_t ev_ready, hipEvent_t ev_rows, int len16) {
    const bool event_start = (h_iq != nullptr) || direct;
    hipStream_t ts = ctx->tail_stream, tb = ctx->bits_stream;
    ResolveArgs r;
    EmitArgs e;
    table_args(ctx, p, pl, n, chunks, slab, rs_mem, out->rows, out->cap_rows, &st->n_acc, &st->rows_at[S - 1], &st->rows_needed, false, &r, &e);
    int8_t *h_state = nullptr; int32_t *h_len = nullptr;
    BitsOut bo{out->bits, out->cap_bits, out->msg_off, out->pauses, out->cap_msg, out->pos, out->cap_pos, out->pos_off, out->counts, out->h_counts};
    if (host_blob) { h_state = (int8_t *)((char *)host_blob + host_layout.off_row_state); h_len = (int32_t *)((char *)host_blob + host_layout.off_row_len); }
    if (to_stage) {
        const StagedLayout SL = staged_layout(out->cap_rows, out->cap_bits, out->cap_msg, out->cap_pos, has_pos);
        h_state = (int8_t *)((char *)host_blob + SL.off_row_state); h_len = (int32_t *)((char *)host_blob + SL.off_row_len);
    }
    const bool l16 = to_stage && len16 != 0;
    const bool row16 = l16 && len16 == 2;
    int64_t row16_esc_off = 0;
    if (row16) row16_esc_off = staged_layout(out->cap_rows, out->cap_bits, out->cap_msg, out->cap_pos, has_pos).total;
    int64_t *esc = l16 ? (int64_t *)((char *)host_blob + (row16 ? row16_esc_off : (int64_t)URHGPU_BLOB_HEADER_BYTES)) : nullptr;
    const int64_t esc_cap = row16 ? n / 8191 + 2 : n / 65535 + 2;
    SegPackDst dst{host_blob, cap_host, progress, 0, (direct && ctx->tune_stream_pos_direct) ? 1 : 0, to_stage ? 1 : 0, to_stage ? real_host_blob : nullptr,
                   esc, esc_cap, row16_esc_off};
    int Sb = h_iq ? S : 1;
    int bits_end_at[kMaxSegments];
    for (int j = 0; j < Sb - 1; ++j) bits_end_at[j] = (int)((int64_t)(S - 1) * (j + 1) / (Sb - 1)) - 1;
    bits_end_at[Sb - 1] = S - 1;
    int jb = 0;
    int64_t bits_from = 0, scan_b0 = 0;
    for (int k = 0; k < S; ++k) {
        if (h_iq) URH_HIP(hipStreamWaitEvent(ts, ctx->ev_piece[k], 0));
        else if (direct) URH_HIP(hipStreamWaitEvent(ts, hot_done, 0));
        RowsSegment sg{k, k == S - 1 ? 1 : 0, bound[k], bound[k + 1], SegGate{event_start ? nullptr : progress, k, target[k], k == 0 ? 1 : 0, st, (long long)200000000, 0},
                       h_state, h_len, 1, l16 ? (row16 ? 2 : 1) : 0, esc, esc_cap};
        URH_TRY(launch_rows_segment(r, e, tm, bp, st, sg, ts));
        if (to_stage && ev_rows) URH_HIP(hipEventRecord(ev_rows, ts));
        while (jb < Sb && bits_end_at[jb] < k) ++jb;
        if (jb < Sb && bits_end_at[jb] == k) {
            const bool last = (jb == Sb - 1);
            BitsSegment bs{jb, last ? 1 : 0, bits_from, bound[k + 1], k, st, scan_b0};
            scan_b0 += tile_scan_blocks(bits_from, bound[k + 1], last ? 1 : 0);
            if (last) {
                if (jb > 0) {
                    URH_HIP(hipEventRecord(ctx->ev_bits[slot], tb));
                    URH_HIP(hipStreamWaitEvent(ts, ctx->ev_bits[slot], 0));
                }
                URH_TRY(launch_bits_segment(tm, bp, bo, scratch, ss, out->rows, out->cap_rows, bs, &dst, ts));
            } else {
                URH_HIP(hipEventRecord(ctx->ev_rows[slot][jb], ts));
                URH_HIP(hipStreamWaitEvent(tb, ctx->ev_rows[slot][jb], 0));
                URH_TRY(launch_bits_segment(tm, bp, bo, scratch, ss, out->rows, out->cap_rows, bs, &dst, tb));
            }
            bits_from = bound[k + 1];
            ++jb;
        }
    }
    URH_HIP(hipGetLastError());
    if (!host_blob) URH_HIP(hipMemsetAsync(progress, 0, kMaxSegments * kProgressStride * 4, ts));
    ctx->seg_dirty[slot] = false;
    if (ev_ready) URH_HIP(hipEventRecord(ev_ready, ts));
    URH_HIP(hipStreamWaitEvent(ts, hot_done, 0));
    if (s != ctx->stream && ctx->stream != nullptr) URH_HIP(hipStreamWaitEvent(ctx->stream, hot_done, 0));
    URH_TRY(end_pipelined_pass(ctx));
    return URHGPU_OK;
}

int iq_to_bits_streamed(urhgpu_ctx *ctx, const void *d_iq, int64_t n, const urhgpu_params *p, const urhgpu_outputs *out, void *host_blob,
                        int64_t cap_host, hipEvent_t ev_ready, bool *streamed, const void *h_iq, void *stage_blob, bool *staged, hipEvent_t ev_rows, int len16) {
    *streamed = false;
    if (staged) *staged = false;
    if (!ctx || !p || !out || n <= 0 || !d_iq || !out->rows || !out->counts) return URHGPU_ERR_ARG;
    if (dtype_bytes(p->dtype) == 0) return URHGPU_ERR_DTYPE;
    const bool want_bits = out->bits && out->msg_off && out->pauses && out->pos_off;
    if (!ctx->pipelined || !ctx->tail_stream || n <= 2 || p->mod == URHGPU_MOD_PSK || p->mod == URHGPU_MOD_ASK || !g_tile_tail || !want_bits ||
        (ctx->tune_stream_segments < 2 && !h_iq) || out->cap_rows < 1)
        return URHGPU_OK;
    URH_TRY(check_params(p, true));
    if (((uintptr_t)d_iq & 15) || (out->qad && ((uintptr_t)out->qad & 7))) return URHGPU_ERR_ARG;
    URH_HIP(hipSetDevice(ctx->device));
    StreamPass sp;
    sp.ctx = ctx; sp.d_iq = d_iq; sp.n = n; sp.p = p; sp.out = out; sp.h_iq = h_iq; sp.host_blob = host_blob; sp.cap_host = cap_host;
    sp.pl = make_plan(ctx, n, p->tolerance);
    URH_TRY(hot_run_args(ctx, p, sp.pl, n, 0, true, &sp.a));
    sp.a.in = d_iq; sp.a.qad = out->qad;
    sp.a.lds_pad = ctx->hot_lds_pad;
    if (ctx->wide_int_next) sp.a.wide_int = 1;
    URH_TRY(sp.policy(stage_blob));
    if (sp.S == 0) return URHGPU_OK;
    if (sp.to_stage && staged) *staged = true;
    URH_TRY(sp.begin());
    URH_TRY(sp.hot());
    URH_TRY(sp.tail(ev_ready, ev_rows, len16));
    *streamed = true;
    return URHGPU_OK;
}

}
```

Baseline: 492,100.

## Fuse bit expansion into row emission with decoupled look-back tile scan

For single-segment streamed passes that do not write positions, the row-emission kernel now computes a per-tile bit-offset summary, runs a decoupled look-back scan across blocks, and writes the expanded bits directly. Tiles it cannot finish (look-back gave up, or ambiguous run boundaries) go onto a defer list. A small completion kernel then expands only those deferred tiles plus the last one, instead of running the full expand-tiles pass. The aim is to avoid a second pass over all rows and the separate scan, at the cost of more complex emit kernels, extra registers, and more descriptor and stat memory.

```diff
diff --git a/include/urhgpu.h b/include/urhgpu.h
--- a/include/urhgpu.h
+++ b/include/urhgpu.h
@@ -296,6 +296,7 @@
                           int load_kind);
 int urhgpu_test_hot_stamps(int on);
 int urhgpu_test_tail_skip(int mask);
+int urhgpu_test_fused_expand_stats(urhgpu_ctx *ctx, int64_t out[3]);
 int urhgpu_test_fetch_chunk_tables(urhgpu_ctx *ctx, void *host_dst, int64_t n_chunks);
 int urhgpu_memcpy_to_host(urhgpu_ctx *ctx, const void *d_src, void *host_dst, int64_t bytes);
 int urhgpu_memcpy_dtod(urhgpu_ctx *ctx, void *d_dst, const void *d_src, int64_t bytes);
diff --git a/urh_amd/_lib.py b/urh_amd/_lib.py
--- a/urh_amd/_lib.py
+++ b/urh_amd/_lib.py
@@ -186,6 +186,7 @@
     "urhgpu_test_hot_probe": (_i, [_vp, _vp, _i64, C.POINTER(Params), _vp, _i, _i, _i, _i, _i, _vp, C.POINTER(_i64), _vp, _vp, _i, _i]),
     "urhgpu_test_hot_stamps": (_i, [_i]),
     "urhgpu_test_tail_skip": (_i, [_i]),
+    "urhgpu_test_fused_expand_stats": (_i, [_vp, _vp]),
     "urhgpu_test_fetch_chunk_tables": (_i, [_vp, _vp, _i64]),
     "urhgpu_test_fast_division_dev": (_i, [_vp, C.c_uint64, _i, C.POINTER(C.c_uint64)]),
     "urhgpu_test_sincosf_fast_dev": (_i, [_vp, C.POINTER(C.c_uint64)]),
diff --git a/urh_amd/csrc/common.hpp b/urh_amd/csrc/common.hpp
--- a/urh_amd/csrc/common.hpp
+++ b/urh_amd/csrc/common.hpp
@@ -131,6 +131,9 @@
     int tune_stream_policy = 5;
     long long passes_begun = 0;
     bool tune_stream_latency = false;
+    bool tune_stream_fused_expand = true;
+    int32_t *fused_stats_last = nullptr;
+    int64_t fused_tiles_last = 0;
     bool tune_stream_pos_direct = true;
     int tune_upload_pieces = 4;
     hipEvent_t ev_piece[16] = {};
@@ -154,6 +157,7 @@
     int64_t dc_shard_n = -1;
     urh::Arena batch_dc_mean;
 };
+constexpr size_t kSegFusedStatsOffset = 512;
 constexpr size_t kSegBlockBytes = 4096;
 
 namespace urh {
diff --git a/urh_amd/csrc/ctx.hip b/urh_amd/csrc/ctx.hip
--- a/urh_amd/csrc/ctx.hip
+++ b/urh_amd/csrc/ctx.hip
@@ -224,6 +224,7 @@
     else if (!strcmp(key, "stream_policy")) { if (value < 0 || value > 6) return URHGPU_ERR_ARG; ctx->tune_stream_policy = value; }
     else if (!strcmp(key, "stream_latency")) { ctx->tune_stream_latency = value != 0; }
     else if (!strcmp(key, "stream_pos_direct")) { ctx->tune_stream_pos_direct = value != 0; }
+    else if (!strcmp(key, "stream_fused_expand")) { ctx->tune_stream_fused_expand = value != 0; }
     else if (!strcmp(key, "spin_wait")) { ctx->tune_spin_wait = value != 0; }
     else if (!strcmp(key, "shard_summary_generic")) { ctx->tune_shard_summary_generic = value != 0; }
     else if (!strcmp(key, "wide_int")) { ctx->tune_wide_int = value != 0; }
diff --git a/urh_amd/csrc/launchers.hpp b/urh_amd/csrc/launchers.hpp
--- a/urh_amd/csrc/launchers.hpp
+++ b/urh_amd/csrc/launchers.hpp
@@ -261,7 +261,13 @@
     void *rdesc;
     unsigned long long epoch;
     int64_t *d_row_base = nullptr;
-};
+    int fused_expand = 0;
+    uint8_t *fused_bits = nullptr;
+    int64_t fused_cap_bits = 0;
+    int32_t *fused_stats = nullptr;
+};
+bool fused_expand_fits(int64_t n, int64_t sps, int tolerance, int bps);
+int64_t fused_tile_count(int64_t n_chunks);
 size_t tile_rdesc_bytes(int64_t n_chunks);
 size_t tile_tail_bytes(int64_t n_chunks);
 int64_t tile_desc_cap(int64_t cap_rows, int64_t n_chunks);
diff --git a/urh_amd/csrc/probes.hip b/urh_amd/csrc/probes.hip
--- a/urh_amd/csrc/probes.hip
+++ b/urh_amd/csrc/probes.hip
@@ -92,6 +92,18 @@
 
 int urhgpu_test_hot_stamps(int on) { urh::g_stamp_probe = (on != 0); return URHGPU_OK; }
 int urhgpu_test_tail_skip(int mask) { urh::g_tail_skip = mask; return URHGPU_OK; }
+int urhgpu_test_fused_expand_stats(urhgpu_ctx *ctx, int64_t out[3]) {
+    if (!ctx || !out) return URHGPU_ERR_ARG;
+    out[0] = out[1] = out[2] = 0;
+    if (!ctx->fused_stats_last) return URHGPU_OK;
+    URH_HIP(hipSetDevice(ctx->device));
+    URH_TRY(urhgpu_ctx_sync(ctx));
+    int32_t st[4] = {0, 0, 0, 0};
+    URH_HIP(hipMemcpy(st, ctx->fused_stats_last, sizeof(st), hipMemcpyDeviceToHost));
+    out[1] = st[0]; out[2] = st[1];
+    out[0] = ctx->fused_tiles_last - out[1];
+    return URHGPU_OK;
+}
 
 int urhgpu_test_fetch_chunk_tables(urhgpu_ctx *ctx, void *host_dst, int64_t n_chunks) {
     if (!ctx || !host_dst || n_chunks < 1) return URHGPU_ERR_ARG;
diff --git a/urh_amd/csrc/pulse_table.hip b/urh_amd/csrc/pulse_table.hip
--- a/urh_amd/csrc/pulse_table.hip
+++ b/urh_amd/csrc/pulse_table.hip
@@ -674,7 +674,13 @@
     unsigned long long epoch;
     int64_t *d_row_base;
     int64_t *esc;
-};
+    int32_t *fstats;
+    int32_t *defer_list;
+    GranDesc *fdesc;
+    uint8_t *fbits;
+    int64_t fcap_bits;
+};
+constexpr int kFusedDeferred = 0, kFusedGaveUp = 1;
 
 __global__ __launch_bounds__(kResolveBlock) void k_resolve_one(const ResolveArgs a, const TileTail ft, const int64_t blk0, const SegGate gate) {
     URH_TAIL_PRIO();
@@ -701,6 +707,7 @@
     }
     if (blockIdx.x == 0 && t == 0 && ft.want_bits) ft.huge_count[ft.parity] = 0;
     if (blockIdx.x == 0 && t == 0 && ft.esc) ft.esc[0] = 0;
+    if (blockIdx.x == 0 && t == 0 && ft.fstats) { ft.fstats[kFusedDeferred] = 0; ft.fstats[kFusedGaveUp] = 0; }
     ResElem e = res_identity();
     if (c < a.n_chunks) {
         ChunkInfo *ch = a.chunks + c;
@@ -953,13 +960,119 @@
     }
 }
 
-template <int TC>
-__global__ __launch_bounds__(64 * kEmitWaves) URH_EMIT_OCC void k_emit_rows_tiles(const EmitTileArgs g) {
-    URH_TAIL_PRIO();
+struct TileElem {
+    uint32_t nl;
+    uint32_t ts;
+    uint32_t lb, ld;
+    uint32_t kb;
+    uint32_t tb, td;
+    uint32_t pad;
+};
+static_assert(sizeof(TileElem) == 32, "a tile element is one granule payload");
+__device__ __forceinline__ TileElem te_identity() { TileElem e; e.nl = 0; e.ts = 0; e.lb = 0; e.ld = 0; e.kb = 0; e.tb = 0; e.td = 0; e.pad = 0; return e; }
+__device__ __forceinline__ TileElem te_combine(const TileElem &a, const TileElem &b) {
+    const bool al = a.nl != 0, bl = b.nl != 0;
+    const uint32_t closed = (a.td + b.ld > 0) ? a.tb + b.lb : 0;
+    TileElem r;
+    r.nl = a.nl + b.nl; r.ts = a.ts + b.ts;
+    r.lb = al ? a.lb : a.lb + b.lb;
+    r.ld = al ? a.ld : a.ld + b.ld;
+    r.kb = (al && bl) ? a.kb + b.kb + closed : (al ? a.kb : b.kb);
+    r.tb = bl ? b.tb : a.tb + b.lb;
+    r.td = bl ? b.td : a.td + b.ld;
+    r.pad = 0;
+    return r;
+}
+__device__ __forceinline__ TileElem te_shfl_down(const TileElem &x, int o) {
+    TileElem r;
+    r.nl = (uint32_t)__shfl_down((int)x.nl, o); r.ts = (uint32_t)__shfl_down((int)x.ts, o); r.lb = (uint32_t)__shfl_down((int)x.lb, o);
+    r.ld = (uint32_t)__shfl_down((int)x.ld, o); r.kb = (uint32_t)__shfl_down((int)x.kb, o); r.tb = (uint32_t)__shfl_down((int)x.tb, o);
+    r.td = (uint32_t)__shfl_down((int)x.td, o); r.pad = 0;
+    return r;
+}
+__device__ __forceinline__ TileElem te_shfl0(const TileElem &x) {
+    TileElem r;
+    r.nl = (uint32_t)__shfl((int)x.nl, 0); r.ts = (uint32_t)__shfl((int)x.ts, 0); r.lb = (uint32_t)__shfl((int)x.lb, 0);
+    r.ld = (uint32_t)__shfl((int)x.ld, 0); r.kb = (uint32_t)__shfl((int)x.kb, 0); r.tb = (uint32_t)__shfl((int)x.tb, 0);
+    r.td = (uint32_t)__shfl((int)x.td, 0); r.pad = 0;
+    return r;
+}
+
+__device__ __forceinline__ uint64_t fused_pack(const VecK<4> &v, int64_t state, bool in_cap) {
+    return (uint64_t)(uint32_t)v.v[0] | ((uint64_t)((uint32_t)(state + 1) & 0xFFFFu) << 32) | ((uint64_t)(v.v[1] ? 1 : 0) << 48) |
+           ((uint64_t)(v.v[3] ? 1 : 0) << 49) | ((uint64_t)(in_cap ? 1 : 0) << 50) | (1ull << 51);
+}
+struct FusedKeep {
+    uint64_t k0, k1, k2, k3;
+    bool kept;
+    int64_t t_off, t_total;
+    int64_t t_samples;
+    int n_mine;
+};
+
+struct TileRun {
+    uint32_t B, D, nl;
+    uint32_t Bl, Dl;
+    uint32_t lb, ld;
+    uint32_t K;
+    bool u_first, u_later;
+};
+__device__ __forceinline__ TileRun tr_start() { TileRun r; r.B = 0; r.D = 0; r.nl = 0; r.Bl = 0; r.Dl = 0; r.lb = 0; r.ld = 0; r.K = 0; r.u_first = false; r.u_later = false; return r; }
+__device__ __forceinline__ TileElem tr_elem(const TileRun &r, uint32_t samples) {
+    TileElem e;
+    e.nl = r.nl; e.ts = samples; e.kb = r.K; e.pad = 0;
+    e.lb = r.nl ? r.lb : r.B; e.ld = r.nl ? r.ld : r.D;
+    e.tb = r.nl ? r.B - r.Bl : r.B; e.td = r.nl ? r.D - r.Dl : r.D;
+    return e;
+}
+struct RowPlace { uint32_t rel; bool first; };
+__device__ __forceinline__ uint32_t lane_get(uint32_t v, int src) { return (uint32_t)__builtin_amdgcn_readlane((int)v, __builtin_amdgcn_readfirstlane(src)); }
+__device__ __forceinline__ RowPlace tile_batch(TileRun &r, uint32_t kb, bool is_l, bool is_d, int lane) {
+    uint32_t b_in = kb, c_in = (is_l ? 1u : 0u) | (is_d ? 0x10000u : 0u);
+#pragma unroll
+    for (int o = 1; o < 64; o <<= 1) {
+        const uint32_t ub = (uint32_t)__shfl_up((int)b_in, o), uc = (uint32_t)__shfl_up((int)c_in, o);
+        if (lane >= o) { b_in += ub; c_in += uc; }
+    }
+    const uint32_t Bb = r.B + b_in - kb;
+    const uint32_t Lb = r.nl + (c_in & 0xFFFFu) - (is_l ? 1u : 0u);
+    const uint32_t Db = r.D + (c_in >> 16) - (is_d ? 1u : 0u);
+    uint32_t Bl = r.Bl, Dl = r.Dl, Kb = r.K;
+    const unsigned long long m_l = __ballot(is_l);
+    if (m_l) {
+        const unsigned long long below = m_l & ((1ull << lane) - 1ull);
+        const int src = below ? 63 - __builtin_clzll(below) : lane;
+        const uint32_t sb = (uint32_t)__shfl((int)Bb, src), sd = (uint32_t)__shfl((int)Db, src);
+        if (below) { Bl = sb; Dl = sd; }
+        const uint32_t c = (is_l && Lb > 0 && Db - Dl > 0) ? Bb - Bl : 0u;
+        uint32_t c_incl = c;
+#pragma unroll
+        for (int o = 1; o < 64; o <<= 1) {
+            const uint32_t u = (uint32_t)__shfl_up((int)c_incl, o);
+            if (lane >= o) c_incl += u;
+        }
+        Kb = r.K + c_incl - c;
+        if (r.nl == 0) { const int f = __builtin_ctzll(m_l); r.lb = lane_get(Bb, f); r.ld = lane_get(Db, f); }
+        const int last = 63 - __builtin_clzll(m_l);
+        r.Bl = lane_get(Bb, last); r.Dl = lane_get(Db, last);
+        r.K += lane_get(c_incl, 63);
+    }
+    RowPlace p;
+    p.first = Lb == 0;
+    const bool no_data = (Db - (p.first ? 0u : Dl)) == 0;
+    const bool cand = kb > 0 && !is_d && no_data;
+    r.u_first = r.u_first || __ballot(cand && p.first) != 0ull;
+    r.u_later = r.u_later || __ballot(cand && !p.first) != 0ull;
+    p.rel = p.first ? Bb : Kb + (Bb - Bl);
+    const uint32_t c_tot = lane_get(c_in, 63);
+    r.B += lane_get(b_in, 63); r.nl += c_tot & 0xFFFFu; r.D += c_tot >> 16;
+    return p;
+}
+
+template <int TC, bool FUSED>
+__device__ __forceinline__ void emit_rows_wave(const EmitTileArgs &g, const int64_t w, const int lane, FusedKeep &fk) {
     const EmitArgs &a = g.e;
     const ResolveArgs &r = g.r;
-    const int lane = threadIdx.x & 63;
-    const int64_t w = g.w0 + (int64_t)blockIdx.x * kEmitWaves + __builtin_amdgcn_readfirstlane((int)(threadIdx.x >> 6));
     const int64_t n_cw = g.w_end;
     if (w > n_cw) return;
     const bool totals = (w == n_cw);
@@ -1094,6 +1207,10 @@
                 const VecK<4> v = row_value(state, len, gi == 0, g.bp);
                 acc_bits += v.v[0];
                 acc_ld += (uint64_t)v.v[1] | ((uint64_t)v.v[3] << 32);
+                if constexpr (FUSED) {
+                    const uint64_t pk = fused_pack(v, state, gi - row_base < a.cap_rows);
+                    fk.k0 = (jc == 0) ? pk : fk.k0; fk.k1 = (jc == 1) ? pk : fk.k1; fk.k2 = (jc == 2) ? pk : fk.k2; fk.k3 = (jc == 3) ? pk : fk.k3;
+                }
                 if (v.v[0] > kHugeBits) {
                     const int slot = atomicAdd(g.ft.huge_count + g.ft.parity, 1);
                     if (slot < g.huge_cap) { g.huge[slot].tile = c / TC; g.huge[slot].row = gi - row_base; }
@@ -1102,6 +1219,7 @@
         }
         if (g.ft.want_bits && total > 0) t_samples += lane_bcast(my_last_pos, (int)((total - 1) & 63)) - prev_pos;
         t_total += total;
+        if constexpr (FUSED) { fk.kept = fk.kept && total <= 64; fk.t_off = t_off; fk.t_total = t_total; fk.t_samples = t_samples; fk.n_mine = n_mine; }
         if (jc % TC == TC - 1 || jc == n_mine - 1) {
             VecK<4> acc; acc.zero();
             if (g.ft.want_bits && t_total > 0) {
@@ -1113,6 +1231,94 @@
             if (lane == 0) { g.ft.agg[c / TC] = acc; g.ft.tile_off[c / TC] = t_off; g.ft.tile_cnt[c / TC] = (int32_t)t_total; }
         }
         rec = rec_next;
+    }
+}
+
+__device__ __forceinline__ void expand_rows_wave(uint8_t *bits, int64_t cap_bits, int64_t *pos, int64_t cap_pos, uint32_t *h_pos, bool write_pos,
+                                                 int64_t samples_per_bit, int bps, int lane, int64_t kb, int64_t ob, int64_t op, int64_t ts, int64_t type);
+
+__device__ __forceinline__ uint64_t fused_reread(const EmitTileArgs &g, int64_t i0, int64_t end, int lane) {
+    const int64_t i = i0 + lane;
+    if (i >= end) return 0;
+    const int64_t type = (int64_t)__hip_atomic_load((const unsigned long long *)g.e.rows + 2 * i, __ATOMIC_RELAXED, __HIP_MEMORY_SCOPE_AGENT);
+    const int64_t len = (int64_t)__hip_atomic_load((const unsigned long long *)g.e.rows + 2 * i + 1, __ATOMIC_RELAXED, __HIP_MEMORY_SCOPE_AGENT);
+    return fused_pack(row_value(type, len, i == 0, g.bp), type, true);
+}
+
+template <int TC, bool FUSED>
+__global__ __launch_bounds__(64 * kEmitWaves) URH_EMIT_OCC void k_emit_rows_tiles(const EmitTileArgs g) {
+    URH_TAIL_PRIO();
+    const int lane = threadIdx.x & 63;
+    const int wave = __builtin_amdgcn_readfirstlane((int)(threadIdx.x >> 6));
+    const int64_t w = g.w0 + (int64_t)blockIdx.x * kEmitWaves + wave;
+    FusedKeep fk;
+    fk.k0 = 0; fk.k1 = 0; fk.k2 = 0; fk.k3 = 0;
+    fk.kept = true; fk.t_off = 0; fk.t_total = 0; fk.t_samples = 0; fk.n_mine = 0;
+    emit_rows_wave<TC, FUSED>(g, w, lane, fk);
+    if constexpr (FUSED) {
+        static_assert(!FUSED || (TC == kTailCPW && kTailCPW <= 4), "the fused expansion takes one tile of at most four chunks per wavefront");
+        __shared__ TileElem s_el[kEmitWaves];
+        __shared__ TileElem s_pre;
+        __shared__ int s_ok;
+        const bool has_tile = w < g.w_end && fk.t_total > 0;
+        const int64_t row_end = (fk.t_off + fk.t_total < g.e.cap_rows) ? fk.t_off + fk.t_total : g.e.cap_rows;
+        const int n_batches = !has_tile ? 0 : (fk.kept ? fk.n_mine : (int)((row_end - fk.t_off + 63) / 64));
+        if (has_tile && !fk.kept) __builtin_amdgcn_fence(__ATOMIC_RELEASE, "workgroup");
+        auto batch = [&](int q) -> uint64_t {
+            if (!fk.kept) return fused_reread(g, fk.t_off + 64 * (int64_t)q, row_end, lane);
+            return (q == 0) ? fk.k0 : ((q == 1) ? fk.k1 : ((q == 2) ? fk.k2 : fk.k3));
+        };
+        TileRun run = tr_start();
+        for (int q = 0; q < n_batches; ++q) {
+            const uint64_t pk = batch(q);
+            (void)tile_batch(run, (uint32_t)pk, (pk >> 48) & 1, (pk >> 49) & 1, lane);
+        }
+        const TileElem mine = tr_elem(run, (uint32_t)fk.t_samples);
+        if (lane == 0) s_el[wave] = mine;
+        __syncthreads();
+        if (wave == 0) {
+            TileElem total = te_identity();
+#pragma unroll
+            for (int u = 0; u < kEmitWaves; ++u) total = te_combine(total, s_el[u]);
+            const uint32_t tag = (uint32_t)g.ft.epoch;
+            const int64_t b = blockIdx.x;
+            if (lane == 0) gran_store(g.ft.fdesc[b].agg, total, tag);
+            bool ok;
+            const TileElem prefix = gran_look_back<TileElem>(g.ft.fdesc, b, tag, te_identity(),
+                                                             [](const TileElem &l, const TileElem &r) { return te_combine(l, r); },
+                                                             [](const TileElem &x, int o) { return te_shfl_down(x, o); },
+                                                             [](const TileElem &x) { return te_shfl0(x); }, lane, ok);
+            if (lane == 0) {
+                if (ok) gran_store(g.ft.fdesc[b].incl, te_combine(prefix, total), tag);
+                else atomicAdd(g.ft.fstats + kFusedGaveUp, 1);
+                s_pre = prefix; s_ok = ok ? 1 : 0;
+            }
+        }
+        __syncthreads();
+        if (!has_tile) return;
+        TileElem pre = s_pre;
+        for (int u = 0; u < wave; ++u) pre = te_combine(pre, s_el[u]);
+        const uint32_t open_off = pre.nl ? ((pre.ld > 0 ? pre.lb : 0u) + pre.kb) : 0u;
+        const uint32_t open_bits = pre.nl ? pre.tb : pre.lb, open_data = pre.nl ? pre.td : pre.ld;
+        if (!s_ok || run.u_later || (run.u_first && open_data == 0)) {
+            if (lane == 0) {
+                const int slot = atomicAdd(g.ft.fstats + kFusedDeferred, 1);
+                g.ft.defer_list[slot] = (int32_t)(w * kTailCPW / TC);
+            }
+            return;
+        }
+        const uint32_t second_off = open_off + ((open_data + mine.ld > 0) ? open_bits + mine.lb : 0u);
+        const int bps = (int)g.bp.bps;
+        TileRun run2 = tr_start();
+        for (int q = 0; q < n_batches; ++q) {
+            const uint64_t pk = batch(q);
+            const uint32_t kb = (uint32_t)pk;
+            const RowPlace p = tile_batch(run2, kb, (pk >> 48) & 1, (pk >> 49) & 1, lane);
+            const int64_t ob = p.first ? (int64_t)open_off + open_bits + p.rel : (int64_t)second_off + p.rel;
+            const bool mine_to_do = ((pk >> 50) & 1) && kb > 0 && kb <= (uint32_t)kHugeBits;
+            expand_rows_wave(g.ft.fbits, g.ft.fcap_bits, nullptr, 0, nullptr, false, 0, bps, lane, mine_to_do ? (int64_t)kb : 0, ob, 0, 0,
+                             (int64_t)((pk >> 32) & 0xFFFFu) - 1);
+        }
     }
 }
 
@@ -1243,6 +1449,8 @@
     int64_t n_tiles;
     int64_t t_base;
     uint32_t *h_pos;
+    const int32_t *defer_list = nullptr;
+    const int32_t *fstats = nullptr;
 };
 constexpr unsigned kHugeBlocksX = 16, kHugeBlocksY = 16;
 
@@ -1251,17 +1459,69 @@
     return ((n_tiles + tpw - 1) / tpw + kEmitWaves - 1) / kEmitWaves;
 }
 
-template <int TC>
-__global__ __launch_bounds__(64 * kEmitWaves) URH_EXPAND_OCC void k_expand_tiles(const ExpandTileArgs a) {
-    constexpr int kTPW = kTailCPW / TC;
-    URH_TAIL_PRIO();
-    const int lane = threadIdx.x & 63, wave = __builtin_amdgcn_readfirstlane((int)(threadIdx.x >> 6));
+__device__ __forceinline__ void expand_rows_wave(uint8_t *bits, int64_t cap_bits, int64_t *pos, int64_t cap_pos, uint32_t *h_pos, bool write_pos,
+                                                 int64_t samples_per_bit, int bps, int lane, int64_t kb, int64_t ob, int64_t op, int64_t ts, int64_t type) {
+    constexpr int kShort = 16;
+#if URH_EXPAND_EARLY_EXIT
+    {
+        const int kbs = (kb > 0 && kb <= kShort) ? (int)kb : 0;
+        const int nb = (ob + kbs <= cap_bits) ? kbs : (int)((cap_bits > ob) ? cap_bits - ob : 0);
+        const int np = !write_pos ? 0 : ((op + kbs <= cap_pos) ? kbs : (int)((cap_pos > op) ? cap_pos - op : 0));
+        uint8_t *bp8 = bits + ob;
+        int64_t *pp = pos + op;
+        uint32_t *hp = h_pos ? h_pos + op : nullptr;
+        int64_t tsk = ts;
+        int sh = bps - 1;
+#pragma unroll 1
+        for (int k = 0; k < kShort; ++k) {
+            if (__ballot(k < kbs) == 0ull) break;
+            const uint8_t b = (type < 0) ? 0 : (uint8_t)((type >> sh) & 1);
+            sh = (sh == 0) ? bps - 1 : sh - 1;
+            if (k < nb) bp8[k] = b;
+            if (k < np) { pp[k] = tsk; if (hp) hp[k] = (uint32_t)tsk; }
+            tsk += samples_per_bit;
+        }
+    }
+#else
+    if (kb > 0 && kb <= kShort) {
+        const int nb = (ob + kb <= cap_bits) ? (int)kb : (int)((cap_bits > ob) ? cap_bits - ob : 0);
+        const int np = !write_pos ? 0 : ((op + kb <= cap_pos) ? (int)kb : (int)((cap_pos > op) ? cap_pos - op : 0));
+        uint8_t *bp8 = bits + ob;
+        int64_t *pp = pos + op;
+        uint32_t *hp = h_pos ? h_pos + op : nullptr;
+        int64_t tsk = ts;
+        int sh = bps - 1;
+        for (int k = 0; k < (int)kb; ++k) {
+            const uint8_t b = (type < 0) ? 0 : (uint8_t)((type >> sh) & 1);
+            sh = (sh == 0) ? bps - 1 : sh - 1;
+            if (k < nb) bp8[k] = b;
+            if (k < np) { pp[k] = tsk; if (hp) hp[k] = (uint32_t)tsk; }
+            tsk += samples_per_bit;
+        }
+    }
+#endif
+    unsigned long long big = __ballot(kb > kShort);
+    while (big) {
+        const int src = __builtin_ctzll(big);
+        big &= big - 1;
+        const int64_t kb_s = __shfl(kb, src), ob_s = __shfl(ob, src), op_s = __shfl(op, src), ts_s = __shfl(ts, src),
+                      ty_s = __shfl(type, src);
+        for (int64_t k = lane; k < kb_s; k += 64) {
+            const uint8_t b = symbol_bit(ty_s, k, bps);
+            if (ob_s + k < cap_bits) bits[ob_s + k] = b;
+            if (write_pos && op_s + k < cap_pos) {
+                pos[op_s + k] = ts_s + k * samples_per_bit;
+                if (h_pos) h_pos[op_s + k] = (uint32_t)(ts_s + k * samples_per_bit);
+            }
+        }
+    }
+}
+
+__device__ __forceinline__ void expand_huge_block(const ExpandTileArgs &a, const int64_t hb, const int lane, const int wave) {
     const int bps = (int)a.bp.bps;
-    const int64_t tile_blocks = expand_tile_blocks(a.n_tiles - a.t_base, TC);
-    if ((int64_t)blockIdx.x >= tile_blocks) {
+    {
         const int64_t n = *a.d_n_rows;
         const bool row0g = !a.bp.d_row_base || *a.bp.d_row_base == 0;
-        const int64_t hb = (int64_t)blockIdx.x - tile_blocks;
         const int hx = (int)(hb % kHugeBlocksX), hy = (int)(hb / kHugeBlocksX);
         if (hb == 0 && threadIdx.x == 0) a.huge_count[a.parity ^ 1] = 0;
         int cnt = a.huge_count[a.parity];
@@ -1306,11 +1566,11 @@
                 }
             }
         }
-        return;
-    }
-    const int64_t t0 = a.t_base + ((int64_t)blockIdx.x * kEmitWaves + wave) * kTPW;
-    if (t0 >= a.n_tiles) return;
-    const int n_mine = (int)((a.n_tiles - t0 < kTPW) ? a.n_tiles - t0 : kTPW);
+    }
+}
+
+__device__ __forceinline__ void expand_wave_tiles(const ExpandTileArgs &a, const int64_t t0, const int n_mine, const int lane) {
+    const int bps = (int)a.bp.bps;
     const int64_t n = *a.d_n_rows;
     const int64_t n_groups = *a.d_n_groups;
     const bool row0g = !a.bp.d_row_base || *a.bp.d_row_base == 0;
@@ -1408,63 +1668,37 @@
                     }
                 }
             }
-            constexpr int kShort = 16;
-#if URH_EXPAND_EARLY_EXIT
-            {
-                const int kbs = (kb > 0 && kb <= kShort) ? (int)kb : 0;
-                const int nb = (ob + kbs <= a.cap_bits) ? kbs : (int)((a.cap_bits > ob) ? a.cap_bits - ob : 0);
-                const int np = !a.bp.write_pos ? 0 : ((op + kbs <= a.cap_pos) ? kbs : (int)((a.cap_pos > op) ? a.cap_pos - op : 0));
-                uint8_t *bp8 = a.bits + ob;
-                int64_t *pp = a.pos + op;
-                uint32_t *hp = a.h_pos ? a.h_pos + op : nullptr;
-                int64_t tsk = ts;
-                int sh = bps - 1;
-#pragma unroll 1
-                for (int k = 0; k < kShort; ++k) {
-                    if (__ballot(k < kbs) == 0ull) break;
-                    const uint8_t b = (type < 0) ? 0 : (uint8_t)((type >> sh) & 1);
-                    sh = (sh == 0) ? bps - 1 : sh - 1;
-                    if (k < nb) bp8[k] = b;
-                    if (k < np) { pp[k] = tsk; if (hp) hp[k] = (uint32_t)tsk; }
-                    tsk += a.bp.samples_per_bit;
-                }
-            }
-#else
-            if (kb > 0 && kb <= kShort) {
-                const int nb = (ob + kb <= a.cap_bits) ? (int)kb : (int)((a.cap_bits > ob) ? a.cap_bits - ob : 0);
-                const int np = !a.bp.write_pos ? 0 : ((op + kb <= a.cap_pos) ? (int)kb : (int)((a.cap_pos > op) ? a.cap_pos - op : 0));
-                uint8_t *bp8 = a.bits + ob;
-                int64_t *pp = a.pos + op;
-                uint32_t *hp = a.h_pos ? a.h_pos + op : nullptr;
-                int64_t tsk = ts;
-                int sh = bps - 1;
-                for (int k = 0; k < (int)kb; ++k) {
-                    const uint8_t b = (type < 0) ? 0 : (uint8_t)((type >> sh) & 1);
-                    sh = (sh == 0) ? bps - 1 : sh - 1;
-                    if (k < nb) bp8[k] = b;
-                    if (k < np) { pp[k] = tsk; if (hp) hp[k] = (uint32_t)tsk; }
-                    tsk += a.bp.samples_per_bit;
-                }
-            }
-#endif
-            unsigned long long big = __ballot(kb > kShort);
-            while (big) {
-                const int src = __builtin_ctzll(big);
-                big &= big - 1;
-                const int64_t kb_s = __shfl(kb, src), ob_s = __shfl(ob, src), op_s = __shfl(op, src), ts_s = __shfl(ts, src),
-                              ty_s = __shfl(type, src);
-                for (int64_t k = lane; k < kb_s; k += 64) {
-                    const uint8_t b = symbol_bit(ty_s, k, bps);
-                    if (ob_s + k < a.cap_bits) a.bits[ob_s + k] = b;
-                    if (a.bp.write_pos && op_s + k < a.cap_pos) {
-                        a.pos[op_s + k] = ts_s + k * a.bp.samples_per_bit;
-                        if (a.h_pos) a.h_pos[op_s + k] = (uint32_t)(ts_s + k * a.bp.samples_per_bit);
-                    }
-                }
-            }
+            expand_rows_wave(a.bits, a.cap_bits, a.pos, a.cap_pos, a.h_pos, a.bp.write_pos != 0, a.bp.samples_per_bit, bps, lane, kb, ob, op, ts, type);
             run.v[0] += lane_bcast(in_bits, 63); run.v[1] += lane_bcast(in_l, 63); run.v[2] += lane_bcast(in_ts, 63);
         }
         row0 = row_next;
+    }
+}
+
+template <int TC>
+__global__ __launch_bounds__(64 * kEmitWaves) URH_EXPAND_OCC void k_expand_tiles(const ExpandTileArgs a) {
+    constexpr int kTPW = kTailCPW / TC;
+    URH_TAIL_PRIO();
+    const int lane = threadIdx.x & 63, wave = __builtin_amdgcn_readfirstlane((int)(threadIdx.x >> 6));
+    const int64_t tile_blocks = expand_tile_blocks(a.n_tiles - a.t_base, TC);
+    if ((int64_t)blockIdx.x >= tile_blocks) { expand_huge_block(a, (int64_t)blockIdx.x - tile_blocks, lane, wave); return; }
+    const int64_t t0 = a.t_base + ((int64_t)blockIdx.x * kEmitWaves + wave) * kTPW;
+    if (t0 >= a.n_tiles) return;
+    expand_wave_tiles(a, t0, (int)((a.n_tiles - t0 < kTPW) ? a.n_tiles - t0 : kTPW), lane);
+}
+
+constexpr unsigned kCompleteBlocks = 16;
+__global__ __launch_bounds__(64 * kEmitWaves) URH_EXPAND_OCC void k_expand_complete(const ExpandTileArgs a) {
+    URH_TAIL_PRIO();
+    const int lane = threadIdx.x & 63, wave = __builtin_amdgcn_readfirstlane((int)(threadIdx.x >> 6));
+    if (blockIdx.x >= kCompleteBlocks) { expand_huge_block(a, (int64_t)blockIdx.x - kCompleteBlocks, lane, wave); return; }
+    const bool all = a.huge_count[a.parity] > a.huge_cap;
+    int64_t n_def = a.fstats[kFusedDeferred];
+    if (n_def > a.n_tiles - 1) n_def = a.n_tiles - 1;
+    const int64_t n_work = all ? a.n_tiles : n_def + 1;
+    for (int64_t i = (int64_t)blockIdx.x * kEmitWaves + wave; i < n_work; i += (int64_t)kCompleteBlocks * kEmitWaves) {
+        const int64_t t = all ? i : (i < n_def ? (int64_t)a.defer_list[i] : a.n_tiles - 1);
+        if (t >= 0 && t < a.n_tiles) expand_wave_tiles(a, t, 1, lane);
     }
 }
 
@@ -1652,6 +1886,7 @@
     tc.ft.epoch = m.epoch;
     tc.ft.d_row_base = m.d_row_base;
     tc.ft.esc = nullptr;
+    tc.ft.fstats = nullptr; tc.ft.defer_list = (int32_t *)take((size_t)nt * 4); tc.ft.fdesc = nullptr; tc.ft.fbits = nullptr; tc.ft.fcap_bits = 0;
     return tc;
 }
 }
@@ -1666,14 +1901,16 @@
 }
 int64_t tile_scan_blocks(int64_t c0, int64_t c1, int final) { return tile_scan_blocks_tc(c0, c1, final, kTileChunks); }
 
+static inline int64_t emit_blocks(int64_t n_chunks) { return (tail_waves(n_chunks) + 1 + kEmitWaves - 1) / kEmitWaves; }
+static inline int64_t fused_desc_first(int64_t n_chunks) { return resolve_blocks(n_chunks) + 2 + (n_chunks + 1 + kScanBlock - 1) / kScanBlock + kMaxSegments + 2; }
 size_t tile_rdesc_bytes(int64_t n_chunks) {
-    return (size_t)(resolve_blocks(n_chunks) + 2 + (n_chunks + 1 + kScanBlock - 1) / kScanBlock + kMaxSegments + 2) * sizeof(GranDesc);
+    return (size_t)(fused_desc_first(n_chunks) + emit_blocks(n_chunks) + 2) * sizeof(GranDesc);
 }
 
 size_t tile_tail_bytes(int64_t n_chunks) {
     const int64_t nt = n_chunks + 1;
     return (size_t)n_chunks * sizeof(ResElem) + (size_t)(resolve_blocks(n_chunks) + 1) * sizeof(ResElem) + (size_t)nt * (2 * sizeof(VecK<4>) + 12) +
-           64 + (size_t)kTileHugeCap * sizeof(HugeRef) + 10 * 256;
+           64 + (size_t)kTileHugeCap * sizeof(HugeRef) + (size_t)nt * 4 + 11 * 256;
 }
 
 int launch_tile_rows(const ResolveArgs &r, const EmitArgs &e, const TileTailMem &m, const BitsParams *bp, hipStream_t s) {
@@ -1693,8 +1930,8 @@
     if (!(g_tail_skip & 1)) hipLaunchKernelGGL(k_resolve_one, dim3(gb), dim3(kResolveBlock), 0, s, r, g.ft, (int64_t)0, no_gate);
     const dim3 grid((unsigned)((tail_waves(r.n_chunks) + 1 + kEmitWaves - 1) / kEmitWaves));
     if (!(g_tail_skip & 2)) {
-        if (tile_chunks_of(m) == 1) hipLaunchKernelGGL(k_emit_rows_tiles<1>, grid, dim3(64 * kEmitWaves), 0, s, g);
-        else hipLaunchKernelGGL(k_emit_rows_tiles<kTileChunks>, grid, dim3(64 * kEmitWaves), 0, s, g);
+        if (tile_chunks_of(m) == 1) hipLaunchKernelGGL((k_emit_rows_tiles<1, false>), grid, dim3(64 * kEmitWaves), 0, s, g);
+        else hipLaunchKernelGGL((k_emit_rows_tiles<kTileChunks, false>), grid, dim3(64 * kEmitWaves), 0, s, g);
     }
     return URHGPU_OK;
 }
@@ -1923,6 +2160,16 @@
         hdr[0] = URHGPU_BLOB_MAGIC;
     }
     if (a.final && a.progress && gtid < kMaxSegments) a.progress[gtid * kProgressStride] = 0;
+}
+
+bool fused_expand_fits(int64_t n, int64_t sps, int tolerance, int bps) {
+    if (sps < 1 || tolerance < 0 || bps < 1) return false;
+    return n < (int64_t(1) << 31) && (n / sps + n / ((int64_t)tolerance + 1) + 4) * bps < (int64_t(1) << 31);
+}
+int64_t fused_tile_count(int64_t n_chunks) { return chunk_tiles(n_chunks, kTileChunks); }
+constexpr bool kFusedBuild = kTileChunks == kTailCPW && kTailCPW <= 4;
+static inline bool fused_segment(const TileTailMem &m, const BitsParams &bp, int final, int64_t c0) {
+    return kFusedBuild && m.fused_expand && m.fused_stats && m.fused_bits && final && c0 == 0 && !bp.write_pos && !m.d_row_base;
 }
 
 int launch_rows_segment(const ResolveArgs &r, const EmitArgs &e, const TileTailMem &m, const BitsParams &bp, SegState *state, const RowsSegment &sg,
@@ -1950,8 +2197,18 @@
     SegGate gate = sg.gate;
     gate.fused = (sg.fuse_gate && gate.progress && !gate.init && resolve_blocks(sg.c1 - sg.c0) == 1) ? 1 : 0;
     if (!gate.fused && gate.progress) hipLaunchKernelGGL(k_seg_gate, dim3(1), dim3(64), 0, s, gate);
+    const dim3 rows_grid((unsigned)((g.w_end - g.w0 + 1 + kEmitWaves - 1) / kEmitWaves));
+    if (fused_segment(m, bp, sg.final, sg.c0) && g.e.rows && !(g_tail_skip & 2)) {
+        g.ft.fstats = m.fused_stats; g.ft.fdesc = (GranDesc *)m.rdesc + fused_desc_first(m.n_chunks); g.ft.fbits = m.fused_bits; g.ft.fcap_bits = m.fused_cap_bits;
+        ft_resolve.fstats = m.fused_stats;
+    }
     if (!(g_tail_skip & 1)) hipLaunchKernelGGL(k_resolve_one, dim3((unsigned)resolve_blocks(sg.c1 - sg.c0)), dim3(kResolveBlock), 0, s, r, ft_resolve, sg.c0 / kResolveBlock, gate);
-    if (!(g_tail_skip & 2)) hipLaunchKernelGGL(k_emit_rows_tiles<kTileChunks>, dim3((unsigned)((g.w_end - g.w0 + 1 + kEmitWaves - 1) / kEmitWaves)), dim3(64 * kEmitWaves), 0, s, g);
+    if (!(g_tail_skip & 2)) {
+        if constexpr (kFusedBuild) {
+            if (g.ft.fstats) { hipLaunchKernelGGL((k_emit_rows_tiles<kTileChunks, kFusedBuild>), rows_grid, dim3(64 * kEmitWaves), 0, s, g); return URHGPU_OK; }
+        }
+        hipLaunchKernelGGL((k_emit_rows_tiles<kTileChunks, false>), rows_grid, dim3(64 * kEmitWaves), 0, s, g);
+    }
     return URHGPU_OK;
 }
 
@@ -1999,7 +2256,10 @@
                       bp, tc.huge, m.huge_count, kTileHugeCap, m.parity, t1, t0, h_pos};
     const unsigned tile_blocks = (unsigned)expand_tile_blocks(t1 - t0, kTileChunks);
     if (g_tail_skip & 2048) ea.cap_bits = 0;
-    if (!(g_tail_skip & 16)) hipLaunchKernelGGL(k_expand_tiles<kTileChunks>, dim3(tile_blocks + kHugeBlocksX * kHugeBlocksY), dim3(64 * kEmitWaves), 0, s, ea);
+    if (fused_segment(m, bp, sg.final, sg.c0) && rows && !has_pos && !(g_tail_skip & (2 | 128))) {
+        ea.defer_list = tc.ft.defer_list; ea.fstats = m.fused_stats;
+        if (!(g_tail_skip & 16)) hipLaunchKernelGGL(k_expand_complete, dim3(kCompleteBlocks + kHugeBlocksX * kHugeBlocksY), dim3(64 * kEmitWaves), 0, s, ea);
+    } else if (!(g_tail_skip & 16)) hipLaunchKernelGGL(k_expand_tiles<kTileChunks>, dim3(tile_blocks + kHugeBlocksX * kHugeBlocksY), dim3(64 * kEmitWaves), 0, s, ea);
     if (dst && dst->host) {
         if (((uintptr_t)o.bits & 7) || ((uintptr_t)dst->host & 15)) return URHGPU_ERR_ARG;
         SegPack pk{o.bits, o.msg_off, o.pauses, o.pos_off, o.pos, o.counts, cap_rows, o.cap_bits, o.cap_msg, o.cap_pos, has_pos, (char *)dst->host,
diff --git a/urh_amd/csrc/stream_pass.hip b/urh_amd/csrc/stream_pass.hip
--- a/urh_amd/csrc/stream_pass.hip
+++ b/urh_amd/csrc/stream_pass.hip
@@ -107,7 +107,7 @@
     slot = ctx->flip;
     progress = (uint32_t *)((char *)ctx->d_seg + (size_t)slot * kSegBlockBytes);
     st = (SegState *)((char *)progress + kMaxSegments * kProgressStride * 4);
-    static_assert(kMaxSegments * kProgressStride * 4 + sizeof(SegState) <= kSegBlockBytes && kMaxSegments <= 16, "segment block");
+    static_assert(kMaxSegments * kProgressStride * 4 + kSegFusedStatsOffset + 16 <= kSegBlockBytes && sizeof(SegState) <= kSegFusedStatsOffset && kMaxSegments <= 16, "segment block");
     if (ctx->seg_dirty[slot]) {
         URH_HIP(hipDeviceSynchronize());
         URH_HIP(hipMemset(progress, 0, kSegBlockBytes));
@@ -125,6 +125,12 @@
     if (!chunks || !slab || !rs_mem) return URHGPU_ERR_ARG;
     a.chunks = chunks; a.slab = slab;
     URH_TRY(tile_tail_mem(ctx, pl.n_chunks, true, &tm));
+    tm.fused_stats = (int32_t *)((char *)st + kSegFusedStatsOffset);
+    tm.fused_bits = out->bits; tm.fused_cap_bits = out->cap_bits;
+    tm.fused_expand = (ctx->tune_stream_fused_expand && S == 1 && !has_pos && !bp.write_pos &&
+                       fused_expand_fits(n, p->samples_per_symbol, p->tolerance, p->bits_per_symbol)) ? 1 : 0;
+    ctx->fused_stats_last = tm.fused_expand ? tm.fused_stats : nullptr;
+    ctx->fused_tiles_last = tm.fused_expand ? fused_tile_count(pl.n_chunks) : 0;
     const int64_t cap = std::max<int64_t>(out->cap_rows, 1);
     scratch = ctx->arena.take(bits_scratch_bytes(cap));
     if (!scratch) return URHGPU_ERR_ARG;
@@ -236,6 +242,7 @@
                         int64_t cap_host, hipEvent_t ev_ready, bool *streamed, const void *h_iq, void *stage_blob, bool *staged, hipEvent_t ev_rows, int len16) {
     *streamed = false;
     if (staged) *staged = false;
+    if (ctx) { ctx->fused_stats_last = nullptr; ctx->fused_tiles_last = 0; }
     if (!ctx || !p || !out || n <= 0 || !d_iq || !out->rows || !out->counts) return URHGPU_ERR_ARG;
     if (dtype_bytes(p->dtype) == 0) return URHGPU_ERR_DTYPE;
     const bool want_bits = out->bits && out->msg_off && out->pauses && out->pos_off;
```

Result: slower. 461,100 (-6.3%).
